# fr34za/multilinear

Hardware: AMD Instinct MI355X
Metric: NTT 2^24 field-elems/sec + FRI commit ms; % HBM roofline at 1/2/4/8 GPUs (higher is better)
Workload: dtype u128 mod M (F_M, M = 2^128 - 45*2^40 + 1)

## Files before the change

include/mlhip.h:

```cpp
#ifndef MLHIP_H
#define MLHIP_H

#include <stddef.h>
#include <stdint.h>

#ifdef __cplusplus
extern "C" {
#endif

typedef enum mlh_status {
  MLH_OK = 0,
  MLH_ERR_INVALID = 1,
  MLH_ERR_NOT_POW2 = 2,
  MLH_ERR_BAD_GENERATOR = 3,
  MLH_ERR_HIP = 4,
  MLH_ERR_OOM = 5,
  MLH_ERR_NOT_RS_CODE = 6,
  MLH_ERR_VERIFY = 7,
  MLH_ERR_VERIFY_INDEX = 8,
  MLH_ERR_COMM = 9,
  MLH_ERR_DEVICE = 10
} mlh_status;

typedef struct mlh_ctx mlh_ctx;
typedef struct mlh_transcript mlh_transcript;
typedef struct mlh_fri_prover mlh_fri_prover;

#define MLH_LOG_BLOWUP 1
#define MLH_NUM_QUERIES 128

const char* mlh_version(void);
mlh_status mlh_context_create(int device, void* hip_stream, mlh_ctx** out);
void mlh_context_destroy(mlh_ctx* ctx);
mlh_status mlh_set_table_cache_limit(mlh_ctx* ctx, uint64_t bytes);
uint64_t mlh_table_cache_bytes(const mlh_ctx* ctx);
mlh_status mlh_set_ntt_plan(mlh_ctx* ctx, const uint32_t* logr, uint32_t count);
mlh_status mlh_set_coop_spin_limit(mlh_ctx* ctx, uint32_t sleeps);
mlh_status mlh_set_pcs_fused_max(mlh_ctx* ctx, uint32_t max_vars);
mlh_status mlh_set_stream(mlh_ctx* ctx, void* hip_stream);
mlh_status mlh_synchronize(mlh_ctx* ctx);
const char* mlh_last_error(const mlh_ctx* ctx);
mlh_status mlh_malloc(mlh_ctx* ctx, size_t bytes, void** dev);
mlh_status mlh_free(mlh_ctx* ctx, void* dev);
mlh_status mlh_memcpy_h2d(mlh_ctx* ctx, void* dev, const void* host, size_t bytes);
mlh_status mlh_memcpy_d2h(mlh_ctx* ctx, void* host, const void* dev, size_t bytes);
mlh_status mlh_memcpy_d2d(mlh_ctx* ctx, void* dst, const void* src, size_t bytes);

mlh_status mlh_pow_2_generator(uint32_t log_size, uint8_t gen_out[16]);
mlh_status mlh_pow_2_generator_powers(mlh_ctx* ctx, uint32_t log_size, void* dev_out);

mlh_status mlh_field_add(mlh_ctx* ctx, const void* dev_a, const void* dev_b, void* dev_out, uint64_t n);
mlh_status mlh_field_sub(mlh_ctx* ctx, const void* dev_a, const void* dev_b, void* dev_out, uint64_t n);
mlh_status mlh_field_mul(mlh_ctx* ctx, const void* dev_a, const void* dev_b, void* dev_out, uint64_t n);
mlh_status mlh_field_neg(mlh_ctx* ctx, const void* dev_a, void* dev_out, uint64_t n);
mlh_status mlh_field_scale(mlh_ctx* ctx, const void* dev_a, const uint8_t c[16], void* dev_out,
                           uint64_t n);
mlh_status mlh_field_inv(mlh_ctx* ctx, const void* dev_a, void* dev_out, uint64_t n);

mlh_status mlh_ntt(mlh_ctx* ctx, const void* dev_coeffs, void* dev_evals, uint32_t log_n,
                   const uint8_t gen[16]);
mlh_status mlh_intt(mlh_ctx* ctx, const void* dev_evals, void* dev_coeffs, uint32_t log_n,
                    const uint8_t gen[16]);
mlh_status mlh_bit_reverse_permutation(mlh_ctx* ctx, const void* dev_in, void* dev_out,
                                       uint32_t log_n);
mlh_status mlh_ntt_host(mlh_ctx* ctx, const uint8_t* host_in, uint8_t* host_out, uint32_t log_n,
                        const uint8_t gen[16], int inverse);

mlh_status mlh_reed_solomon(mlh_ctx* ctx, const void* dev_coeffs, uint32_t log_n,
                            const uint8_t gen[16], void* dev_code);
mlh_status mlh_reed_solomon_brev(mlh_ctx* ctx, const void* dev_coeffs, uint32_t log_n,
                                 const uint8_t gen[16], void* dev_code);
uint64_t mlh_merkle_layers_bytes(uint64_t leaves);
mlh_status mlh_merkle_commit_pairs(mlh_ctx* ctx, const void* dev_code, uint32_t log_code,
                                   void* dev_layers, uint8_t root_out[32]);
mlh_status mlh_merkle_commit(mlh_ctx* ctx, const void* dev_items, uint64_t item_len,
                             uint64_t count, void* dev_layers, uint8_t root_out[32]);
mlh_status mlh_merkle_batch_commit(mlh_ctx* ctx, const void* dev_items, uint64_t item_len,
                                   uint32_t m, uint64_t count, void* dev_layers,
                                   uint8_t root_out[32]);
mlh_status mlh_fri_fold(mlh_ctx* ctx, const void* dev_layer, uint32_t log_layer, uint32_t k,
                        uint32_t log_domain, const uint8_t r[16], void* dev_next);

mlh_status mlh_gen_pows_params(const uint8_t* gen_pows, uint64_t len, uint8_t gen_out[16],
                               uint32_t* log_len_out);
mlh_status mlh_gen_pows_verify(mlh_ctx* ctx, const uint8_t* gen_pows, uint64_t len,
                               uint8_t gen_out[16], uint32_t* log_len_out);
mlh_status mlh_fri_prover_init(mlh_ctx* ctx, const void* dev_code, uint32_t log_code,
                               mlh_transcript* tr, mlh_fri_prover** out);
mlh_status mlh_fri_prover_init_gp(mlh_ctx* ctx, const void* dev_code, uint32_t log_code,
                                  const uint8_t gen_pows_1[16], uint32_t log_gen_pows,
                                  mlh_transcript* tr, mlh_fri_prover** out);
mlh_status mlh_fri_prover_fold_step(mlh_ctx* ctx, mlh_fri_prover* p, uint32_t k,
                                    const uint8_t r[16], mlh_transcript* tr);
mlh_status mlh_fri_prover_fold_step_gp(mlh_ctx* ctx, mlh_fri_prover* p, const uint8_t gen_pows_1[16],
                                       uint32_t log_gen_pows, uint32_t k, const uint8_t r[16],
                                       mlh_transcript* tr);
mlh_status mlh_fri_prover_fold(mlh_ctx* ctx, const void* dev_code, uint32_t log_code,
                               mlh_transcript* tr, mlh_fri_prover** out);
mlh_status mlh_fri_prover_fold_gp(mlh_ctx* ctx, const void* dev_code, uint32_t log_code,
                                  const uint8_t gen_pows_1[16], uint32_t log_gen_pows,
                                  mlh_transcript* tr, mlh_fri_prover** out);
uint32_t mlh_fri_prover_num_trees(const mlh_fri_prover* p);
mlh_status mlh_fri_prover_roots(const mlh_fri_prover* p, uint8_t* roots_out );
mlh_status mlh_fri_prover_last_element(const mlh_fri_prover* p, uint8_t out[16]);
mlh_status mlh_fri_prover_open_query(mlh_ctx* ctx, const mlh_fri_prover* p, uint64_t index,
                                     uint8_t* out);
void mlh_fri_prover_destroy(mlh_fri_prover* p);

typedef struct mlh_fri_proof {
  uint32_t log_code;
  uint32_t num_trees;
  uint32_t num_queries;
  uint8_t* commitments;
  uint8_t last_elem[16];
  uint8_t last_random[32];
  uint64_t* query_indices;
  uint8_t* queries;
} mlh_fri_proof;
uint64_t mlh_fri_query_bytes(uint32_t log_code);
mlh_status mlh_fri_prove(mlh_ctx* ctx, const void* dev_code, uint32_t log_code, mlh_transcript* tr,
                         mlh_fri_proof* proof);
mlh_status mlh_fri_prove_gp(mlh_ctx* ctx, const void* dev_code, uint32_t log_code,
                            const uint8_t gen_pows_1[16], uint32_t log_gen_pows, mlh_transcript* tr,
                            mlh_fri_proof* proof);
uint64_t mlh_fri_proof_encoded_size(const mlh_fri_proof* proof);
mlh_status mlh_fri_proof_encode(const mlh_fri_proof* proof, uint8_t* out, uint64_t cap);
mlh_status mlh_fri_proof_decode_header(const uint8_t* in, uint64_t len, uint32_t* log_code,
                                       uint32_t* num_queries);
mlh_status mlh_fri_proof_decode(const uint8_t* in, uint64_t len, mlh_fri_proof* proof);
mlh_status mlh_fri_verify(const mlh_fri_proof* proof);

mlh_status mlh_fri_prover_open_queries(mlh_ctx* ctx, const mlh_fri_prover* p,
                                       const uint64_t* idx, uint32_t nq, uint8_t* out);

mlh_status mlh_shard_ntt_cross(mlh_ctx* ctx, const void* dev_in, void* dev_out, uint32_t log_n,
                               uint32_t log_p, uint32_t rank, const uint8_t gen[16], int inverse);
mlh_status mlh_shard_fri_fold(mlh_ctx* ctx, const void* dev_layer, uint32_t log_local, uint32_t k,
                              uint32_t log_domain, const uint8_t r[16], void* dev_next,
                              uint32_t log_s, uint32_t log_p, uint32_t rank);
mlh_status mlh_shard_fri_fold_commit(mlh_ctx* ctx, const void* dev_layer, uint32_t log_local,
                                     uint32_t k, uint32_t log_domain, const uint8_t r[16],
                                     void* dev_next, void* dev_tree, uint32_t log_s,
                                     uint32_t log_p, uint32_t rank);
mlh_status mlh_merkle_open(mlh_ctx* ctx, const void* dev_layers, uint64_t leaves,
                           const uint64_t* host_idx, uint32_t nq, uint8_t* out);
mlh_status mlh_merkle_verify(const uint8_t* value, uint64_t value_len, const uint8_t* sibs,
                             uint32_t depth, uint64_t dirs, const uint8_t root[32], uint64_t index);
mlh_status mlh_merkle_open_pairs(mlh_ctx* ctx, const void* dev_values, uint32_t log_n,
                                 const void* dev_tree, uint32_t levels, const uint64_t* idx,
                                 uint32_t nq, uint8_t* out);

uint64_t mlh_device_transcript_bytes(void);
mlh_status mlh_transcript_to_device(mlh_ctx* ctx, const mlh_transcript* tr, void* dev_state);
mlh_status mlh_transcript_from_device(mlh_ctx* ctx, const void* dev_state, mlh_transcript* tr);
mlh_status mlh_device_transcript_absorb(mlh_ctx* ctx, void* dev_state, const void* dev_src,
                                        uint32_t n, void* dev_challenge);
mlh_status mlh_device_fri_last(mlh_ctx* ctx, const void* dev_vals2, void* dev_state,
                               void* dev_flag, void* dev_last);
mlh_status mlh_shard_fri_fold_dr(mlh_ctx* ctx, const void* dev_layer, uint32_t log_local,
                                 uint32_t k, uint32_t log_domain, const void* dev_r,
                                 void* dev_next, uint32_t log_s, uint32_t log_p, uint32_t rank);
mlh_status mlh_shard_fri_fold_commit_dr(mlh_ctx* ctx, const void* dev_layer, uint32_t log_local,
                                        uint32_t k, uint32_t log_domain, const void* dev_r,
                                        void* dev_next, void* dev_tree, uint32_t log_s,
                                        uint32_t log_p, uint32_t rank);
mlh_status mlh_merkle_top(mlh_ctx* ctx, const void* dev_gathered, uint32_t P, uint64_t per_rank,
                          void* dev_levels);

mlh_status mlh_sumcheck_sums_dev(mlh_ctx* ctx, const void* dev_matrix, const void* dev_delta,
                                 uint32_t log_height, void* dev_sums);
mlh_status mlh_sumcheck_fold_sums_dr(mlh_ctx* ctx, void* dev_matrix, void* dev_delta,
                                     uint32_t log_height, const void* dev_r, void* dev_sums);
mlh_status mlh_sumcheck_fold_dr(mlh_ctx* ctx, void* dev_matrix, void* dev_delta,
                                uint32_t log_height, const void* dev_r);
mlh_status mlh_device_sumcheck_round(mlh_ctx* ctx, const void* dev_sum_pairs, uint32_t npairs,
                                     void* dev_prev, void* dev_state, void* dev_poly_out,
                                     void* dev_r_out);

typedef struct mlh_batched_fri_proof {
  uint32_t log_code;
  uint32_t num_codes;
  uint32_t num_trees;
  uint32_t num_queries;
  uint8_t batch_commitment[32];
  uint8_t* commitments;
  uint8_t last_elem[16];
  uint8_t last_random[32];
  uint64_t* query_indices;
  uint8_t* queries;
} mlh_batched_fri_proof;
uint64_t mlh_batched_fri_query_bytes(uint32_t log_code, uint32_t num_codes);
mlh_status mlh_batched_fri_prove(mlh_ctx* ctx, const void* dev_codes, uint32_t num_codes,
                                 uint32_t log_code, mlh_transcript* tr,
                                 mlh_batched_fri_proof* proof);
mlh_status mlh_batched_fri_verify(const mlh_batched_fri_proof* proof);
typedef struct mlh_batched_fri_prover mlh_batched_fri_prover;
mlh_status mlh_batched_fri_prover_init(mlh_ctx* ctx, const void* dev_codes, uint32_t num_codes,
                                       uint32_t log_code, mlh_transcript* tr,
                                       mlh_batched_fri_prover** out);
mlh_status mlh_batched_fri_prover_fold_step_gp(mlh_ctx* ctx, mlh_batched_fri_prover* bp,
                                               const uint8_t gen_pows_1[16], uint32_t log_gen_pows,
                                               const uint8_t r[16], mlh_transcript* tr);
mlh_fri_prover* mlh_batched_fri_prover_inner(mlh_batched_fri_prover* bp);
mlh_status mlh_batched_fri_prover_batch_root(const mlh_batched_fri_prover* bp, uint8_t out[32]);
mlh_status mlh_batched_fri_prover_fingerprint_r(const mlh_batched_fri_prover* bp, uint8_t out[16]);
mlh_status mlh_batched_fri_prover_open_query(mlh_ctx* ctx, const mlh_batched_fri_prover* bp,
                                             uint64_t index, uint8_t* out);
void mlh_batched_fri_prover_destroy(mlh_batched_fri_prover* bp);
typedef struct mlh_batched_pcs_proof {
  mlh_batched_fri_proof fri;
  uint8_t* sumcheck_polys;
} mlh_batched_pcs_proof;
mlh_status mlh_batched_pcs_prove(mlh_ctx* ctx, const void* dev_evals, uint32_t num_polys,
                                 uint32_t n_vars, const uint8_t* inputs, const uint8_t* outputs,
                                 mlh_transcript* tr, mlh_batched_pcs_proof* proof);
mlh_status mlh_batched_pcs_verify(const mlh_batched_pcs_proof* proof, uint32_t n_vars,
                                  const uint8_t* inputs, const uint8_t* outputs,
                                  mlh_transcript* tr);

mlh_status mlh_transcript_create(mlh_transcript** out);
mlh_status mlh_transcript_clone(const mlh_transcript* t, mlh_transcript** out);
void mlh_transcript_destroy(mlh_transcript* t);
mlh_status mlh_transcript_absorb(mlh_transcript* t, const uint8_t* bytes, uint64_t len);
mlh_status mlh_transcript_random(const mlh_transcript* t, uint8_t out[32]);
mlh_status mlh_transcript_next_challenge(mlh_transcript* t, uint8_t out[16]);

mlh_status mlh_mle_to_coefficient(mlh_ctx* ctx, void* dev_evals, uint32_t log_n);
mlh_status mlh_mle_to_evaluation(mlh_ctx* ctx, void* dev_coeffs, uint32_t log_n);
mlh_status mlh_eq_table(mlh_ctx* ctx, const uint8_t* host_points, uint32_t n, void* dev_out);
mlh_status mlh_mle_evaluate(mlh_ctx* ctx, const void* dev_evals, uint32_t n,
                            const uint8_t* host_args, uint8_t out[16]);
mlh_status mlh_mle_coeffs_evaluate(mlh_ctx* ctx, const void* dev_coeffs, uint32_t n,
                                   const uint8_t* host_args, uint8_t out[16]);
mlh_status mlh_poly_evaluate(mlh_ctx* ctx, const void* dev_coeffs, uint64_t n, const uint8_t x[16],
                             uint8_t out[16]);
mlh_status mlh_trace_evaluate(mlh_ctx* ctx, const void* dev_matrix, uint32_t log_height,
                              uint32_t width, const uint8_t* host_points, uint8_t* out);
mlh_status mlh_sumcheck_partial_sums(mlh_ctx* ctx, const void* dev_matrix, const void* dev_delta,
                                     uint32_t log_height, uint8_t out[32]);
mlh_status mlh_sumcheck_fold(mlh_ctx* ctx, void* dev_matrix, void* dev_delta, uint32_t log_height,
                             const uint8_t r[16]);
mlh_status mlh_sumcheck_fold_and_sums(mlh_ctx* ctx, void* dev_matrix, void* dev_delta,
                                      uint32_t log_height, const uint8_t r[16], uint8_t out[32]);
mlh_status mlh_sumcheck_prove(mlh_ctx* ctx, void* dev_matrix, void* dev_delta, uint32_t log_height,
                              const uint8_t sum[16], mlh_transcript* tr, uint8_t* polys_out,
                              uint8_t* rs_out);
mlh_status mlh_sumcheck_prove_eq(mlh_ctx* ctx, const void* dev_evals, void* dev_work,
                                 uint32_t log_height, const uint8_t* host_points,
                                 const uint8_t sum[16], mlh_transcript* tr, uint8_t* polys_out,
                                 uint8_t* rs_out, uint8_t* delta_out);

typedef struct mlh_cs_program mlh_cs_program;
#define MLH_CS_MAX_LOG_HEIGHT 32
mlh_status mlh_cs_program_create(const uint8_t* bytes, uint64_t len, mlh_cs_program** out);
void mlh_cs_program_destroy(mlh_cs_program* prog);
uint32_t mlh_cs_program_width(const mlh_cs_program* prog);
uint32_t mlh_cs_program_degree(const mlh_cs_program* prog);
uint32_t mlh_cs_program_n_constraints(const mlh_cs_program* prog);
uint32_t mlh_cs_program_n_randoms(const mlh_cs_program* prog);
mlh_status mlh_cs_program_evaluate(const mlh_cs_program* prog, const uint8_t* host_values,
                                   const uint8_t* host_randoms, const uint8_t* host_mask,
                                   uint8_t out[16]);
mlh_status mlh_cs_launch_info(const mlh_cs_program* prog, uint32_t log_height, uint32_t* threads,
                              uint32_t* blocks);
mlh_status mlh_system_challenges(mlh_transcript* tr, uint32_t log_rows, uint32_t n_randoms,
                                 uint32_t n_constraints, uint8_t* row_out, uint8_t* trace_out,
                                 uint8_t* constraint_out, uint8_t* mask_out);
mlh_status mlh_cs_partial_sums(mlh_ctx* ctx, const mlh_cs_program* prog, uint32_t width,
                               const void* dev_matrix, const void* dev_delta, uint32_t log_height,
                               const uint8_t* host_randoms, const uint8_t* host_mask,
                               uint8_t* out);
mlh_status mlh_cs_fold(mlh_ctx* ctx, uint32_t width, void* dev_matrix, void* dev_delta,
                       uint32_t log_height, const uint8_t r[16]);
mlh_status mlh_cs_fold_and_sums(mlh_ctx* ctx, const mlh_cs_program* prog, uint32_t width,
                                void* dev_matrix, void* dev_delta, uint32_t log_height,
                                const uint8_t* host_randoms, const uint8_t* host_mask,
                                const uint8_t r[16], uint8_t* out);
mlh_status mlh_cs_sumcheck_prove(mlh_ctx* ctx, const mlh_cs_program* prog, uint32_t width,
                                 void* dev_matrix, void* dev_delta, uint32_t log_height,
                                 const uint8_t* host_randoms, const uint8_t* host_mask,
                                 const uint8_t sum[16], mlh_transcript* tr, uint8_t* polys_out,
                                 uint8_t* rs_out);
mlh_status mlh_cs_sumcheck_verify(const mlh_cs_program* prog, uint32_t log_height,
                                  const uint8_t* host_row_points, const uint8_t* host_randoms,
                                  const uint8_t* host_mask, const uint8_t sum[16],
                                  const uint8_t* polys, const uint8_t* host_output,
                                  mlh_transcript* tr);

mlh_status mlh_cs_sumcheck_prove_sums(mlh_ctx* ctx, const mlh_cs_program* prog, uint32_t width,
                                      void* dev_matrix, void* dev_delta, uint32_t log_height,
                                      const uint8_t* host_randoms, const uint8_t* host_mask,
                                      uint32_t sum_column_mask, const uint8_t* beta,
                                      const uint8_t claim[16], mlh_transcript* tr,
                                      uint8_t* polys_out, uint8_t* rs_out);
mlh_status mlh_cs_sumcheck_verify_sums(const mlh_cs_program* prog, uint32_t log_height,
                                       const uint8_t* host_row_points, const uint8_t* host_randoms,
                                       const uint8_t* host_mask, uint32_t sum_column_mask,
                                       const uint8_t* beta, const uint8_t claim[16],
                                       const uint8_t* polys, const uint8_t* host_output,
                                       mlh_transcript* tr);

mlh_status mlh_trace_columns(mlh_ctx* ctx, const void* dev_matrix, uint32_t log_height,
                             uint32_t width, void* dev_out);
mlh_status mlh_trace_columns_launch_info(uint32_t log_height, uint32_t width, uint32_t* tile_rows,
                                         uint32_t* blocks);
typedef struct mlh_trace_commitment mlh_trace_commitment;
mlh_status mlh_trace_commit(mlh_ctx* ctx, const void* dev_matrix, uint32_t log_height,
                            uint32_t width, mlh_trace_commitment** out);
mlh_status mlh_trace_columns_range(mlh_ctx* ctx, const void* dev_matrix, uint32_t log_height,
                                   uint32_t width, uint32_t col0, uint32_t ncols, void* dev_out);
mlh_status mlh_trace_columns_range_launch_info(uint32_t log_height, uint32_t width, uint32_t col0,
                                               uint32_t ncols, uint32_t* tile_rows,
                                               uint32_t* blocks);
mlh_status mlh_trace_commit_range(mlh_ctx* ctx, const void* dev_matrix, uint32_t log_height,
                                  uint32_t width, uint32_t col0, uint32_t ncols,
                                  mlh_trace_commitment** out);
mlh_status mlh_trace_commitment_root(const mlh_trace_commitment* c, uint8_t out[32]);
uint32_t mlh_trace_commitment_width(const mlh_trace_commitment* c);
uint32_t mlh_trace_commitment_log_height(const mlh_trace_commitment* c);
void mlh_trace_commitment_destroy(mlh_trace_commitment* c);
typedef struct mlh_system_proof {
  uint32_t log_height, width, degree;
  uint8_t* sumcheck_polys;
  uint8_t* output;
  mlh_batched_pcs_proof pcs;
} mlh_system_proof;
mlh_status mlh_system_prove(mlh_ctx* ctx, const mlh_cs_program* prog,
                            const mlh_trace_commitment* commitment, void* dev_matrix,
                            const uint8_t sum[16], mlh_transcript* tr, mlh_system_proof* proof);
mlh_status mlh_system_verify(const mlh_cs_program* prog, uint32_t log_height, const uint8_t sum[16],
                             const mlh_system_proof* proof, mlh_transcript* tr);

mlh_status mlh_system_trace_randoms(const mlh_transcript* tr, const uint8_t root1[32],
                                    uint32_t n_randoms, uint8_t* out);
typedef struct mlh_phased_proof {
  uint32_t log_height, width, degree;
  uint32_t pre_random_columns;
  uint32_t sum_column_mask;
  uint8_t* sumcheck_polys;
  uint8_t* output;
  mlh_batched_pcs_proof pcs[2];
} mlh_phased_proof;
mlh_status mlh_system_prove_phased(mlh_ctx* ctx, const mlh_cs_program* prog,
                                   const mlh_trace_commitment* commitment1,
                                   const mlh_trace_commitment* commitment2,
                                   uint32_t sum_column_mask, void* dev_matrix,
                                   const uint8_t sum[16], const uint8_t column_sum[16],
                                   mlh_transcript* tr, mlh_phased_proof* proof);
mlh_status mlh_system_verify_phased(const mlh_cs_program* prog, uint32_t log_height,
                                    uint32_t pre_random_columns, uint32_t sum_column_mask,
                                    const uint8_t sum[16], const uint8_t column_sum[16],
                                    const mlh_phased_proof* proof, mlh_transcript* tr);

typedef struct mlh_fill_program mlh_fill_program;
mlh_status mlh_fill_program_create(const uint8_t* bytes, uint64_t len, mlh_fill_program** out);
void mlh_fill_program_destroy(mlh_fill_program* prog);
uint32_t mlh_fill_program_width(const mlh_fill_program* prog);
uint32_t mlh_fill_program_n_randoms(const mlh_fill_program* prog);
uint32_t mlh_fill_program_n_outputs(const mlh_fill_program* prog);
uint32_t mlh_fill_program_n_inverses(const mlh_fill_program* prog);
uint32_t mlh_fill_program_output_mask(const mlh_fill_program* prog);
mlh_status mlh_fill_program_evaluate(const mlh_fill_program* prog, const uint8_t* host_row,
                                     const uint8_t* host_randoms, uint8_t* out_row);
mlh_status mlh_trace_fill(mlh_ctx* ctx, const mlh_fill_program* prog, void* dev_matrix,
                          uint32_t log_height, uint32_t width, const uint8_t* host_randoms);
mlh_status mlh_trace_fill_launch_info(const mlh_fill_program* prog, uint32_t log_height,
                                      uint32_t* threads, uint32_t* rows_per_thread,
                                      uint32_t* blocks);
mlh_status mlh_trace_fill_shaped(mlh_ctx* ctx, const mlh_fill_program* prog, void* dev_matrix,
                                 uint32_t log_height, uint32_t width, const uint8_t* host_randoms,
                                 uint32_t threads, uint32_t rows_per_thread);
mlh_status mlh_trace_column_sum(mlh_ctx* ctx, const void* dev_matrix, uint32_t log_height,
                                uint32_t width, uint32_t column_mask, uint8_t out[16]);

typedef struct mlh_pcs_proof {
  mlh_fri_proof fri;
  uint8_t* sumcheck_polys;
} mlh_pcs_proof;
mlh_status mlh_pcs_prove(mlh_ctx* ctx, const void* dev_evals, uint32_t n_vars,
                         const uint8_t* host_inputs, const uint8_t output[16], mlh_transcript* tr,
                         mlh_pcs_proof* proof);
mlh_status mlh_pcs_verify(const mlh_pcs_proof* proof, uint32_t n_vars, const uint8_t* host_inputs,
                          const uint8_t output[16], mlh_transcript* tr);

typedef int (*mlh_all_to_all_fn)(void* user, const void* dev_send, void* dev_recv,
                                 uint64_t bytes_per_rank, void* hip_stream);
typedef int (*mlh_all_gather_fn)(void* user, const void* dev_send, void* dev_recv, uint64_t bytes,
                                 void* hip_stream);
typedef struct mlh_transport {
  uint32_t world;
  uint32_t rank;
  uint32_t host_side;
  void* user;
  mlh_all_to_all_fn all_to_all;
  mlh_all_gather_fn all_gather;
} mlh_transport;
typedef struct mlh_comm mlh_comm;
mlh_status mlh_comm_unique_id(uint8_t out[128]);
mlh_status mlh_comm_create(mlh_ctx* ctx, uint32_t world, uint32_t rank, const uint8_t id[128],
                           mlh_comm** out);
void mlh_comm_destroy(mlh_comm* comm);
mlh_status mlh_comm_transport(mlh_comm* comm, mlh_transport* out);
mlh_status mlh_comm_info(mlh_comm* comm, uint32_t* count, uint32_t* rank, int* device);
mlh_status mlh_comm_preflight(mlh_ctx* ctx, const mlh_transport* tp, uint64_t bytes_per_rank,
                              uint64_t* mismatches, float* ms);
mlh_status mlh_sharded_ntt(mlh_ctx* ctx, const mlh_transport* tp, const void* dev_in, void* dev_out,
                           uint32_t log_n, const uint8_t gen[16], int inverse);
mlh_status mlh_sharded_ntt_batch(mlh_ctx* ctx, const mlh_transport* tp, const void* const* dev_in,
                                 void* const* dev_out, uint32_t count, uint32_t log_n,
                                 const uint8_t gen[16], int inverse);
mlh_status mlh_sharded_ntt_fused_batch(mlh_ctx* ctx, const mlh_transport* tp, const void* const* dev_in,
                                       void* const* dev_out, uint32_t count, uint32_t log_n,
                                       const uint8_t gen[16], uint32_t* log_s_out);
mlh_status mlh_sharded_reed_solomon(mlh_ctx* ctx, const mlh_transport* tp, const void* dev_coeffs,
                                    uint32_t log_n, const uint8_t gen[16], void* dev_code);
mlh_status mlh_sharded_commit_rs_code(mlh_ctx* ctx, const mlh_transport* tp, const void* dev_code,
                                      uint32_t log_code, uint8_t root_out[32]);
mlh_status mlh_sharded_fri_prove(mlh_ctx* ctx, const mlh_transport* tp, const void* dev_code,
                                 uint32_t log_code, uint32_t gather_log, mlh_transcript* tr,
                                 mlh_fri_proof* proof);
mlh_status mlh_sharded_eq_table(mlh_ctx* ctx, const mlh_transport* tp, const uint8_t* points,
                                uint32_t n, void* dev_out);
mlh_status mlh_sharded_sumcheck_prove(mlh_ctx* ctx, const mlh_transport* tp, void* dev_m, void* dev_d,
                                      uint32_t n, const uint8_t sum[16], mlh_transcript* tr,
                                      uint8_t* polys_out, uint8_t* rs_out);

mlh_status mlh_profile_enable(mlh_ctx* ctx, int on);
mlh_status mlh_profile_reset(mlh_ctx* ctx);
mlh_status mlh_profile_get(mlh_ctx* ctx, const char* label, uint64_t* count, double* total_ms);
mlh_status mlh_bench_ntt(mlh_ctx* ctx, void* dev_buf, uint32_t log_n, uint32_t iters,
                         float* ms_out);

#ifdef __cplusplus
}
#endif
#endif
```

multilinear_amd/_lib.py:

```python
import ctypes
import os

_HERE = os.path.dirname(os.path.abspath(__file__))
LIB_PATH = os.path.join(_HERE, "libmlhip.so")

MLH_OK = 0
STATUS_NAMES = {
    0: "MLH_OK",
    1: "MLH_ERR_INVALID",
    2: "MLH_ERR_NOT_POW2",
    3: "MLH_ERR_BAD_GENERATOR",
    4: "MLH_ERR_HIP",
    5: "MLH_ERR_OOM",
    6: "MLH_ERR_NOT_RS_CODE",
    7: "MLH_ERR_VERIFY",
    8: "MLH_ERR_VERIFY_INDEX",
    9: "MLH_ERR_COMM",
    10: "MLH_ERR_DEVICE",
}
STATUS_CODES = {v: k for k, v in STATUS_NAMES.items()}
globals().update(STATUS_CODES)
LOG_BLOWUP = 1
NUM_QUERIES = 128


class MlhError(RuntimeError):
    def __init__(self, status, msg=""):
        self.status = status
        super().__init__("%s: %s" % (STATUS_NAMES.get(status, status), msg))


class FriProofC(ctypes.Structure):
    _fields_ = [
        ("log_code", ctypes.c_uint32),
        ("num_trees", ctypes.c_uint32),
        ("num_queries", ctypes.c_uint32),
        ("commitments", ctypes.c_void_p),
        ("last_elem", ctypes.c_uint8 * 16),
        ("last_random", ctypes.c_uint8 * 32),
        ("query_indices", ctypes.c_void_p),
        ("queries", ctypes.c_void_p),
    ]


class PcsProofC(ctypes.Structure):
    _fields_ = [("fri", FriProofC), ("sumcheck_polys", ctypes.c_void_p)]


class BatchedFriProofC(ctypes.Structure):
    _fields_ = [
        ("log_code", ctypes.c_uint32),
        ("num_codes", ctypes.c_uint32),
        ("num_trees", ctypes.c_uint32),
        ("num_queries", ctypes.c_uint32),
        ("batch_commitment", ctypes.c_uint8 * 32),
        ("commitments", ctypes.c_void_p),
        ("last_elem", ctypes.c_uint8 * 16),
        ("last_random", ctypes.c_uint8 * 32),
        ("query_indices", ctypes.c_void_p),
        ("queries", ctypes.c_void_p),
    ]


class BatchedPcsProofC(ctypes.Structure):
    _fields_ = [("fri", BatchedFriProofC), ("sumcheck_polys", ctypes.c_void_p)]


class SystemProofC(ctypes.Structure):
    _fields_ = [
        ("log_height", ctypes.c_uint32),
        ("width", ctypes.c_uint32),
        ("degree", ctypes.c_uint32),
        ("sumcheck_polys", ctypes.c_void_p),
        ("output", ctypes.c_void_p),
        ("pcs", BatchedPcsProofC),
    ]


class PhasedProofC(ctypes.Structure):
    _fields_ = [
        ("log_height", ctypes.c_uint32),
        ("width", ctypes.c_uint32),
        ("degree", ctypes.c_uint32),
        ("pre_random_columns", ctypes.c_uint32),
        ("sum_column_mask", ctypes.c_uint32),
        ("sumcheck_polys", ctypes.c_void_p),
        ("output", ctypes.c_void_p),
        ("pcs", BatchedPcsProofC * 2),
    ]


ALL_TO_ALL_FN = ctypes.CFUNCTYPE(ctypes.c_int, ctypes.c_void_p, ctypes.c_void_p, ctypes.c_void_p,
                                 ctypes.c_uint64, ctypes.c_void_p)
ALL_GATHER_FN = ctypes.CFUNCTYPE(ctypes.c_int, ctypes.c_void_p, ctypes.c_void_p, ctypes.c_void_p,
                                 ctypes.c_uint64, ctypes.c_void_p)


class TransportC(ctypes.Structure):
    _fields_ = [
        ("world", ctypes.c_uint32),
        ("rank", ctypes.c_uint32),
        ("host_side", ctypes.c_uint32),
        ("user", ctypes.c_void_p),
        ("all_to_all", ALL_TO_ALL_FN),
        ("all_gather", ALL_GATHER_FN),
    ]


_P = ctypes.c_void_p
_U32 = ctypes.c_uint32
_U64 = ctypes.c_uint64
_I = ctypes.c_int
_S = ctypes.c_size_t

SIGNATURES = {
    "mlh_version": (ctypes.c_char_p, []),
    "mlh_context_create": (_I, [_I, _P, ctypes.POINTER(_P)]),
    "mlh_context_destroy": (None, [_P]),
    "mlh_set_stream": (_I, [_P, _P]),
    "mlh_set_ntt_plan": (_I, [_P, ctypes.POINTER(ctypes.c_uint32), _U32]),
    "mlh_set_coop_spin_limit": (_I, [_P, _U32]),
    "mlh_set_pcs_fused_max": (_I, [_P, _U32]),
    "mlh_set_table_cache_limit": (_I, [_P, ctypes.c_uint64]),
    "mlh_table_cache_bytes": (ctypes.c_uint64, [_P]),
    "mlh_synchronize": (_I, [_P]),
    "mlh_last_error": (ctypes.c_char_p, [_P]),
    "mlh_malloc": (_I, [_P, _S, ctypes.POINTER(_P)]),
    "mlh_free": (_I, [_P, _P]),
    "mlh_memcpy_h2d": (_I, [_P, _P, _P, _S]),
    "mlh_memcpy_d2h": (_I, [_P, _P, _P, _S]),
    "mlh_memcpy_d2d": (_I, [_P, _P, _P, _S]),
    "mlh_pow_2_generator": (_I, [_U32, _P]),
    "mlh_pow_2_generator_powers": (_I, [_P, _U32, _P]),
    "mlh_field_add": (_I, [_P, _P, _P, _P, _U64]),
    "mlh_field_sub": (_I, [_P, _P, _P, _P, _U64]),
    "mlh_field_mul": (_I, [_P, _P, _P, _P, _U64]),
    "mlh_field_neg": (_I, [_P, _P, _P, _U64]),
    "mlh_field_scale": (_I, [_P, _P, _P, _P, _U64]),
    "mlh_field_inv": (_I, [_P, _P, _P, _U64]),
    "mlh_ntt": (_I, [_P, _P, _P, _U32, _P]),
    "mlh_intt": (_I, [_P, _P, _P, _U32, _P]),
    "mlh_bit_reverse_permutation": (_I, [_P, _P, _P, _U32]),
    "mlh_ntt_host": (_I, [_P, _P, _P, _U32, _P, _I]),
    "mlh_reed_solomon": (_I, [_P, _P, _U32, _P, _P]),
    "mlh_reed_solomon_brev": (_I, [_P, _P, _U32, _P, _P]),
    "mlh_merkle_layers_bytes": (_U64, [_U64]),
    "mlh_merkle_commit_pairs": (_I, [_P, _P, _U32, _P, _P]),
    "mlh_merkle_commit": (_I, [_P, _P, _U64, _U64, _P, _P]),
    "mlh_merkle_batch_commit": (_I, [_P, _P, _U64, _U32, _U64, _P, _P]),
    "mlh_fri_fold": (_I, [_P, _P, _U32, _U32, _U32, _P, _P]),
    "mlh_fri_prover_init": (_I, [_P, _P, _U32, _P, ctypes.POINTER(_P)]),
    "mlh_fri_prover_fold_step": (_I, [_P, _P, _U32, _P, _P]),
    "mlh_fri_prover_fold_step_gp": (_I, [_P, _P, _P, _U32, _U32, _P, _P]),
    "mlh_fri_prover_fold": (_I, [_P, _P, _U32, _P, ctypes.POINTER(_P)]),
    "mlh_fri_prover_init_gp": (_I, [_P, _P, _U32, _P, _U32, _P, ctypes.POINTER(_P)]),
    "mlh_fri_prover_fold_gp": (_I, [_P, _P, _U32, _P, _U32, _P, ctypes.POINTER(_P)]),
    "mlh_fri_prover_num_trees": (_U32, [_P]),
    "mlh_fri_prover_roots": (_I, [_P, _P]),
    "mlh_fri_prover_last_element": (_I, [_P, _P]),
    "mlh_fri_prover_open_query": (_I, [_P, _P, _U64, _P]),
    "mlh_fri_prover_open_queries": (_I, [_P, _P, _P, _U32, _P]),
    "mlh_fri_prover_destroy": (None, [_P]),
    "mlh_fri_query_bytes": (_U64, [_U32]),
    "mlh_fri_prove": (_I, [_P, _P, _U32, _P, ctypes.POINTER(FriProofC)]),
    "mlh_fri_prove_gp": (_I, [_P, _P, _U32, _P, _U32, _P, ctypes.POINTER(FriProofC)]),
    "mlh_fri_verify": (_I, [ctypes.POINTER(FriProofC)]),
    "mlh_fri_proof_encoded_size": (_U64, [ctypes.POINTER(FriProofC)]),
    "mlh_fri_proof_encode": (_I, [ctypes.POINTER(FriProofC), _P, _U64]),
    "mlh_fri_proof_decode_header": (_I, [_P, _U64, ctypes.POINTER(_U32), ctypes.POINTER(_U32)]),
    "mlh_fri_proof_decode": (_I, [_P, _U64, ctypes.POINTER(FriProofC)]),
    "mlh_shard_ntt_cross": (_I, [_P, _P, _P, _U32, _U32, _U32, _P, _I]),
    "mlh_shard_fri_fold": (_I, [_P, _P, _U32, _U32, _U32, _P, _P, _U32, _U32, _U32]),
    "mlh_shard_fri_fold_commit": (_I, [_P, _P, _U32, _U32, _U32, _P, _P, _P, _U32, _U32, _U32]),
    "mlh_merkle_open_pairs": (_I, [_P, _P, _U32, _P, _U32, _P, _U32, _P]),
    "mlh_merkle_open": (_I, [_P, _P, _U64, _P, _U32, _P]),
    "mlh_merkle_verify": (_I, [_P, _U64, _P, _U32, _U64, _P, _U64]),
    "mlh_batched_fri_query_bytes": (_U64, [_U32, _U32]),
    "mlh_batched_fri_prove": (_I, [_P, _P, _U32, _U32, _P, ctypes.POINTER(BatchedFriProofC)]),
    "mlh_batched_fri_prover_init": (_I, [_P, _P, _U32, _U32, _P, ctypes.POINTER(_P)]),
    "mlh_batched_fri_prover_fold_step_gp": (_I, [_P, _P, _P, _U32, _P, _P]),
    "mlh_batched_fri_prover_inner": (_P, [_P]),
    "mlh_batched_fri_prover_batch_root": (_I, [_P, _P]),
    "mlh_batched_fri_prover_fingerprint_r": (_I, [_P, _P]),
    "mlh_batched_fri_prover_open_query": (_I, [_P, _P, ctypes.c_uint64, _P]),
    "mlh_batched_fri_prover_destroy": (None, [_P]),
    "mlh_batched_fri_verify": (_I, [ctypes.POINTER(BatchedFriProofC)]),
    "mlh_batched_pcs_prove": (_I, [_P, _P, _U32, _U32, _P, _P, _P,
                                   ctypes.POINTER(BatchedPcsProofC)]),
    "mlh_batched_pcs_verify": (_I, [ctypes.POINTER(BatchedPcsProofC), _U32, _P, _P, _P]),
    "mlh_device_transcript_bytes": (_U64, []),
    "mlh_transcript_to_device": (_I, [_P, _P, _P]),
    "mlh_transcript_from_device": (_I, [_P, _P, _P]),
    "mlh_device_transcript_absorb": (_I, [_P, _P, _P, _U32, _P]),
    "mlh_device_fri_last": (_I, [_P, _P, _P, _P, _P]),
    "mlh_shard_fri_fold_dr": (_I, [_P, _P, _U32, _U32, _U32, _P, _P, _U32, _U32, _U32]),
    "mlh_shard_fri_fold_commit_dr": (_I, [_P, _P, _U32, _U32, _U32, _P, _P, _P, _U32, _U32, _U32]),
    "mlh_merkle_top": (_I, [_P, _P, _U32, _U64, _P]),
    "mlh_sumcheck_sums_dev": (_I, [_P, _P, _P, _U32, _P]),
    "mlh_sumcheck_fold_sums_dr": (_I, [_P, _P, _P, _U32, _P, _P]),
    "mlh_sumcheck_fold_dr": (_I, [_P, _P, _P, _U32, _P]),
    "mlh_device_sumcheck_round": (_I, [_P, _P, _U32, _P, _P, _P, _P]),
    "mlh_transcript_create": (_I, [ctypes.POINTER(_P)]),
    "mlh_transcript_clone": (_I, [_P, ctypes.POINTER(_P)]),
    "mlh_transcript_destroy": (None, [_P]),
    "mlh_transcript_absorb": (_I, [_P, _P, _U64]),
    "mlh_transcript_random": (_I, [_P, _P]),
    "mlh_transcript_next_challenge": (_I, [_P, _P]),
    "mlh_mle_to_coefficient": (_I, [_P, _P, _U32]),
    "mlh_mle_to_evaluation": (_I, [_P, _P, _U32]),
    "mlh_eq_table": (_I, [_P, _P, _U32, _P]),
    "mlh_mle_coeffs_evaluate": (_I, [_P, _P, _U32, _P, _P]),
    "mlh_poly_evaluate": (_I, [_P, _P, _U64, _P, _P]),
    "mlh_trace_evaluate": (_I, [_P, _P, _U32, _U32, _P, _P]),
    "mlh_mle_evaluate": (_I, [_P, _P, _U32, _P, _P]),
    "mlh_sumcheck_partial_sums": (_I, [_P, _P, _P, _U32, _P]),
    "mlh_sumcheck_fold": (_I, [_P, _P, _P, _U32, _P]),
    "mlh_sumcheck_fold_and_sums": (_I, [_P, _P, _P, _U32, _P, _P]),
    "mlh_sumcheck_prove": (_I, [_P, _P, _P, _U32, _P, _P, _P, _P]),
    "mlh_sumcheck_prove_eq": (_I, [_P, _P, _P, _U32, _P, _P, _P, _P, _P, _P]),
    "mlh_cs_program_create": (_I, [_P, _U64, ctypes.POINTER(_P)]),
    "mlh_cs_program_destroy": (None, [_P]),
    "mlh_cs_program_width": (_U32, [_P]),
    "mlh_cs_program_degree": (_U32, [_P]),
    "mlh_cs_program_n_constraints": (_U32, [_P]),
    "mlh_cs_program_n_randoms": (_U32, [_P]),
    "mlh_cs_program_evaluate": (_I, [_P, _P, _P, _P, _P]),
    "mlh_cs_launch_info": (_I, [_P, _U32, ctypes.POINTER(_U32), ctypes.POINTER(_U32)]),
    "mlh_system_challenges": (_I, [_P, _U32, _U32, _U32, _P, _P, _P, _P]),
    "mlh_cs_partial_sums": (_I, [_P, _P, _U32, _P, _P, _U32, _P, _P, _P]),
    "mlh_cs_fold": (_I, [_P, _U32, _P, _P, _U32, _P]),
    "mlh_cs_fold_and_sums": (_I, [_P, _P, _U32, _P, _P, _U32, _P, _P, _P, _P]),
    "mlh_cs_sumcheck_prove": (_I, [_P, _P, _U32, _P, _P, _U32, _P, _P, _P, _P, _P, _P]),
    "mlh_cs_sumcheck_verify": (_I, [_P, _U32, _P, _P, _P, _P, _P, _P, _P]),
    "mlh_cs_sumcheck_prove_sums": (_I, [_P, _P, _U32, _P, _P, _U32, _P, _P, _U32, _P, _P, _P, _P, _P]),
    "mlh_cs_sumcheck_verify_sums": (_I, [_P, _U32, _P, _P, _P, _U32, _P, _P, _P, _P, _P]),
    "mlh_trace_columns": (_I, [_P, _P, _U32, _U32, _P]),
    "mlh_trace_columns_range": (_I, [_P, _P, _U32, _U32, _U32, _U32, _P]),
    "mlh_trace_columns_range_launch_info": (_I, [_U32, _U32, _U32, _U32, ctypes.POINTER(_U32),
                                                 ctypes.POINTER(_U32)]),
    "mlh_trace_commit_range": (_I, [_P, _P, _U32, _U32, _U32, _U32, ctypes.POINTER(_P)]),
    "mlh_system_trace_randoms": (_I, [_P, _P, _U32, _P]),
    "mlh_system_prove_phased": (_I, [_P, _P, _P, _P, _U32, _P, _P, _P, _P,
                                     ctypes.POINTER(PhasedProofC)]),
    "mlh_system_verify_phased": (_I, [_P, _U32, _U32, _U32, _P, _P, ctypes.POINTER(PhasedProofC), _P]),
    "mlh_fill_program_create": (_I, [_P, _U64, ctypes.POINTER(_P)]),
    "mlh_fill_program_destroy": (None, [_P]),
    "mlh_fill_program_width": (_U32, [_P]),
    "mlh_fill_program_n_randoms": (_U32, [_P]),
    "mlh_fill_program_n_outputs": (_U32, [_P]),
    "mlh_fill_program_n_inverses": (_U32, [_P]),
    "mlh_fill_program_output_mask": (_U32, [_P]),
    "mlh_fill_program_evaluate": (_I, [_P, _P, _P, _P]),
    "mlh_trace_fill": (_I, [_P, _P, _P, _U32, _U32, _P]),
    "mlh_trace_fill_launch_info": (_I, [_P, _U32, ctypes.POINTER(_U32), ctypes.POINTER(_U32),
                                        ctypes.POINTER(_U32)]),
    "mlh_trace_fill_shaped": (_I, [_P, _P, _P, _U32, _U32, _P, _U32, _U32]),
    "mlh_trace_column_sum": (_I, [_P, _P, _U32, _U32, _U32, _P]),
    "mlh_trace_columns_launch_info": (_I, [_U32, _U32, ctypes.POINTER(_U32), ctypes.POINTER(_U32)]),
    "mlh_trace_commit": (_I, [_P, _P, _U32, _U32, ctypes.POINTER(_P)]),
    "mlh_trace_commitment_root": (_I, [_P, _P]),
    "mlh_trace_commitment_width": (_U32, [_P]),
    "mlh_trace_commitment_log_height": (_U32, [_P]),
    "mlh_trace_commitment_destroy": (None, [_P]),
    "mlh_system_prove": (_I, [_P, _P, _P, _P, _P, _P, ctypes.POINTER(SystemProofC)]),
    "mlh_system_verify": (_I, [_P, _U32, _P, ctypes.POINTER(SystemProofC), _P]),
    "mlh_pcs_prove": (_I, [_P, _P, _U32, _P, _P, _P, ctypes.POINTER(PcsProofC)]),
    "mlh_pcs_verify": (_I, [ctypes.POINTER(PcsProofC), _U32, _P, _P, _P]),
    "mlh_bench_ntt": (_I, [_P, _P, _U32, _U32, ctypes.POINTER(ctypes.c_float)]),
    "mlh_profile_enable": (_I, [_P, _I]),
    "mlh_profile_reset": (_I, [_P]),
    "mlh_profile_get": (_I, [_P, ctypes.c_char_p, ctypes.POINTER(_U64), ctypes.POINTER(ctypes.c_double)]),
    "mlh_comm_unique_id": (_I, [_P]),
    "mlh_comm_create": (_I, [_P, _U32, _U32, _P, ctypes.POINTER(_P)]),
    "mlh_comm_destroy": (None, [_P]),
    "mlh_comm_transport": (_I, [_P, ctypes.POINTER(TransportC)]),
    "mlh_comm_info": (_I, [_P, ctypes.POINTER(_U32), ctypes.POINTER(_U32), ctypes.POINTER(ctypes.c_int)]),
    "mlh_comm_preflight": (_I, [_P, ctypes.POINTER(TransportC), ctypes.c_uint64,
                                ctypes.POINTER(ctypes.c_uint64), ctypes.POINTER(ctypes.c_float)]),
    "mlh_sharded_ntt": (_I, [_P, ctypes.POINTER(TransportC), _P, _P, _U32, _P, _I]),
    "mlh_gen_pows_params": (_I, [_P, _U64, _P, ctypes.POINTER(_U32)]),
    "mlh_gen_pows_verify": (_I, [_P, _P, _U64, _P, ctypes.POINTER(_U32)]),
    "mlh_sharded_ntt_batch": (_I, [_P, ctypes.POINTER(TransportC), ctypes.POINTER(_P),
                                   ctypes.POINTER(_P), _U32, _U32, _P, _I]),
    "mlh_sharded_ntt_fused_batch": (_I, [_P, ctypes.POINTER(TransportC), ctypes.POINTER(_P),
                                         ctypes.POINTER(_P), _U32, _U32, _P, ctypes.POINTER(_U32)]),
    "mlh_sharded_reed_solomon": (_I, [_P, ctypes.POINTER(TransportC), _P, _U32, _P, _P]),
    "mlh_sharded_commit_rs_code": (_I, [_P, ctypes.POINTER(TransportC), _P, _U32, _P]),
    "mlh_sharded_fri_prove": (_I, [_P, ctypes.POINTER(TransportC), _P, _U32, _U32, _P,
                                   ctypes.POINTER(FriProofC)]),
    "mlh_sharded_eq_table": (_I, [_P, ctypes.POINTER(TransportC), _P, _U32, _P]),
    "mlh_sharded_sumcheck_prove": (_I, [_P, ctypes.POINTER(TransportC), _P, _P, _U32, _P, _P, _P, _P]),
}

_lib = None


def load():
    global _lib
    if _lib is not None:
        return _lib
    if not os.path.exists(LIB_PATH):
        raise ImportError(
            "libmlhip.so not built at %s -- run `python -c 'import __graft_entry__ as g; g.build()'`"
            % LIB_PATH
        )
    import torch

    lib = ctypes.CDLL(LIB_PATH)
    for name, (res, args) in SIGNATURES.items():
        fn = getattr(lib, name)
        fn.restype = res
        fn.argtypes = args
    _lib = lib
    return lib
```

multilinear_amd/csrc/capi.hip:

```cpp
#include <hip/hip_runtime.h>
#include <stdint.h>
#include <stdio.h>
#include <string.h>

#include <algorithm>
#include <map>
#include <memory>
#include <string>
#include <tuple>
#include <vector>

#include "../../include/mlhip.h"
#include "field.hpp"
#include "dist.hpp"
#include "fieldops.hpp"
#include "host_field.hpp"
#include "host_sha256.hpp"
#include "host_transcript.hpp"
#include "context.hpp"
#include "cs_program.hpp"
#include "cs_sumcheck.hpp"
#include "fri_prover.hpp"
#include "fused_ntt.hpp"
#include "merkle.hpp"
#include "ntt.hpp"
#include "pcs_prover.hpp"
#include "sha256.hpp"
#include "sumcheck.hpp"
#include "system_head.hpp"
#include "tables.hpp"
#include "trace_commit.hpp"
#include "trace_fill.hpp"
#include "transcript_dev.hpp"

using namespace mlh;


constexpr uint64_t kTablePin = 24;

static bool ranges_overlap(const void* a, const void* b, uint64_t bytes) {
  const uintptr_t x = (uintptr_t)a, y = (uintptr_t)b;
  return x < y ? y - x < bytes : x - y < bytes;
}

static mlh_status table_make_room(mlh_ctx* ctx, size_t need) {
  if (ctx->table_bytes + need <= ctx->table_limit) return MLH_OK;
  std::vector<std::pair<uint64_t, TableKey>> order;
  for (auto& kv : ctx->tables)
    if (kv.second.stamp + kTablePin <= ctx->table_stamp) order.push_back({kv.second.stamp, kv.first});
  std::sort(order.begin(), order.end(),
            [](const std::pair<uint64_t, TableKey>& a, const std::pair<uint64_t, TableKey>& b) {
              return a.first < b.first;
            });
  bool synced = false;
  for (auto& o : order) {
    if (ctx->table_bytes + need <= ctx->table_limit) break;
    if (!synced) {
      HIP_TRY(ctx, hipStreamSynchronize(ctx->stream));
      synced = true;
    }
    auto it = ctx->tables.find(o.second);
    HIP_TRY(ctx, hipFree(it->second.d));
    ctx->table_bytes -= it->second.bytes;
    ctx->tables.erase(it);
  }
  return MLH_OK;
}

static bool table_hit(mlh_ctx* ctx, const TableKey& k, const fe** out) {
  auto it = ctx->tables.find(k);
  if (it == ctx->tables.end()) return false;
  it->second.stamp = ++ctx->table_stamp;
  *out = it->second.d;
  return true;
}

static mlh_status table_alloc(mlh_ctx* ctx, const TableKey& k, size_t bytes, fe** d) {
  MLH_TRY(table_make_room(ctx, bytes));
  HIP_TRY(ctx, hipMalloc(d, bytes));
  ctx->tables[k] = CachedTable{*d, bytes, ++ctx->table_stamp};
  ctx->table_bytes += bytes;
  return MLH_OK;
}

mlh_status mlh::get_table(mlh_ctx* ctx, u128 base, uint64_t count, u128 scale, const fe** out,
                          bool expand) {
  TableKey k{base, count, scale, expand ? 1 : 0};
  if (table_hit(ctx, k, out)) return MLH_OK;
  fe* d = nullptr;
  MLH_TRY(table_alloc(ctx, k, count * sizeof(fe) * (expand ? 4 : 1), &d));
  HIP_TRY(ctx, launch_pow_table(d, to_fe(base), to_fe(scale), count, ctx->stream, expand));
  *out = d;
  return MLH_OK;
}

static mlh_status get_table2d(mlh_ctx* ctx, u128 base, uint64_t rows, uint64_t cols,
                              uint64_t mult, u128 scale, const fe** out, bool expand = false) {
  TableKey k{base, rows, scale, expand ? 1 : 0, cols, mult};
  if (table_hit(ctx, k, out)) return MLH_OK;
  fe* d = nullptr;
  MLH_TRY(table_alloc(ctx, k, rows * cols * sizeof(fe) * (expand ? 4 : 1), &d));
  HIP_TRY(ctx, launch_pow_table2d(d, to_fe(base), to_fe(scale), rows, cols, mult, ctx->stream,
                                  expand));
  *out = d;
  return MLH_OK;
}

uint64_t mlh::hi_count(uint32_t log_n) {
  const uint64_t N = 1ull << log_n;
  return N <= 4096 ? 1 : N / 4096;
}

#ifndef MLH_P0_GEO
#define MLH_P0_GEO 1
#endif
#ifndef MLH_P0_GEO_MAXLOGW
#define MLH_P0_GEO_MAXLOGW 16
#endif
static mlh_status get_ntt_tables(mlh_ctx* ctx, u128 gen, uint32_t log_n, bool inverse,
                                 NttTables* tb, const uint32_t* plan = nullptr, uint32_t nplan = 0) {
  const uint64_t N = 1ull << log_n;
  const u128 w = inverse ? h_inv(gen) : gen;
  const u128 scale = inverse ? h_inv((u128)N) : (u128)1;
  tb->log_n = log_n;
  tb->inverse = inverse;
  tb->scale = to_fe(scale);
  if (log_n <= 10) {
    MLH_TRY(get_table(ctx, w, N / 2 ? N / 2 : 1, 1, &tb->tw_small));
    return MLH_OK;
  }
  tb->debug_sync = ctx->debug_sync;
  if (plan)
    ntt_plan_radices(log_n, &tb->nradix, tb->logr, plan, nplan);
  else
    ntt_plan_radices(log_n, &tb->nradix, tb->logr, ctx->forced_plan, ctx->forced_plan_len);
  for (uint32_t p = 0; p < tb->nradix; ++p) {
    const uint64_t R = 1ull << tb->logr[p];
    MLH_TRY(get_table(ctx, h_pow(w, N / R), R / 2, 1, &tb->tw[p], true));
  }
  uint64_t S = 1;
  for (uint32_t p = 0; p + 1 < tb->nradix; ++p) {
    const uint64_t R = 1ull << tb->logr[p];
    const uint32_t logw = log_n - (uint32_t)__builtin_ctzll(S) - tb->logr[p];
    const uint32_t loga =
        tb->logr[p] + logw <= kFullTwLog ? logw : (logw < kTwLogA ? logw : kTwLogA);
    const u128 ws = h_pow(w, S);
    tb->loga[p] = loga;
    MLH_TRY(get_table2d(ctx, ws, R, 1ull << loga, 1, p == 0 ? scale : (u128)1, &tb->ta[p]));
    tb->tb[p] = nullptr;
    if (logw > loga)
      MLH_TRY(get_table2d(ctx, ws, R, 1ull << (logw - loga), 1ull << loga, 1, &tb->tb[p], true));
    if (MLH_P0_GEO && p == 0 && logw > loga && (tb->logr[0] == 7 || tb->logr[0] == 8) &&
        logw <= MLH_P0_GEO_MAXLOGW) {
      MLH_TRY(get_table2d(ctx, ws, 64, 1ull << logw, 1, scale, &tb->gp[0]));
      MLH_TRY(get_table(ctx, h_pow(ws, 64), 1ull << logw, 1, &tb->gc[0], true));
    }
    S <<= tb->logr[p];
  }
  return MLH_OK;
}

bool mlh::check_generator(u128 gen, uint32_t log_n) {
  if (gen >= kModulus) return false;
  if (log_n == 0) return gen == 1;
  const u128 half = h_pow(gen, (u128)1 << (log_n - 1));
  return half == kModulus - 1;
}

mlh_status mlh::read_root(mlh_ctx* ctx, const uint8_t* layers, uint64_t leaves, uint8_t out[32]) {
  if (!out) return MLH_OK;
  HIP_TRY(ctx, hipMemcpyAsync(ctx->pinned, layers + (2 * leaves - 2) * 32, 32,
                              hipMemcpyDeviceToHost, ctx->stream));
  HIP_TRY(ctx, hipStreamSynchronize(ctx->stream));
  memcpy(out, ctx->pinned, 32);
  return MLH_OK;
}

mlh_status mlh::fold_tables_g(mlh_ctx* ctx, u128 g, uint32_t log_len, const fe** tlo,
                              const fe** thi) {
  const u128 ginv = h_inv(g);
  MLH_TRY(get_table(ctx, ginv, 4096, 1, tlo));
  MLH_TRY(get_table(ctx, h_pow(ginv, 4096), hi_count(log_len), 1, thi));
  return MLH_OK;
}
mlh_status mlh::fold_tables(mlh_ctx* ctx, uint32_t log_domain, const fe** tlo, const fe** thi) {
  return fold_tables_g(ctx, h_pow2_generator(log_domain), log_domain, tlo, thi);
}

#ifndef MLH_FOLD_TABLE_MAX_LOG
#define MLH_FOLD_TABLE_MAX_LOG 25
#endif
mlh_status mlh::fold_layer_table(mlh_ctx* ctx, u128 g, uint32_t L, const fe** out) {
  *out = nullptr;
  if (L < 2 || L > MLH_FOLD_TABLE_MAX_LOG) return MLH_OK;
  const TableKey key{h_inv(g), (1ull << L) - 1, 0, 2};
  if (table_hit(ctx, key, out)) return MLH_OK;
  fe* d = nullptr;
  MLH_TRY(table_alloc(ctx, key, ((1ull << L) - 1) * sizeof(fe), &d));
  const fe *tlo, *thi;
  MLH_TRY(fold_tables_g(ctx, g, L, &tlo, &thi));
  HIP_TRY(ctx, launch_fold_layer_table(d, tlo, thi, L, ctx->stream));
  *out = d;
  return MLH_OK;
}

static mlh_status ensure_ntt_scratch(mlh_ctx* ctx, uint32_t log_n) {
  const size_t need = (size_t)16 << log_n;
  if (ctx->ntt_scratch_bytes < need) {
    if (ctx->ntt_scratch) {
      HIP_TRY(ctx, hipStreamSynchronize(ctx->stream));
      HIP_TRY(ctx, hipFree(ctx->ntt_scratch));
      ctx->ntt_scratch = nullptr;
      ctx->ntt_scratch_bytes = 0;
    }
    HIP_TRY(ctx, hipMalloc(&ctx->ntt_scratch, need));
    ctx->ntt_scratch_bytes = need;
  }
  return MLH_OK;
}

static mlh_status ntt_network_core(mlh_ctx* ctx, const fe* in, fe* out, uint32_t log_n, u128 gen,
                                   bool inverse, int zero_top) {
  const u128 w = inverse ? h_inv(gen) : gen;
  const fe *tlo, *thi;
  MLH_TRY(get_table(ctx, w, 4096, 1, &tlo));
  MLH_TRY(get_table(ctx, h_pow(w, 4096), hi_count(log_n - 1), 1, &thi));
  fe* scratch = nullptr;
  if (in == out && log_n > 11) {
    MLH_TRY(ensure_ntt_scratch(ctx, log_n));
    scratch = ctx->ntt_scratch;
  }
  const u128 scale = inverse ? h_inv((u128)1 << log_n) : (u128)1;
  HIP_TRY(ctx, launch_ntt_network(in, out, scratch, tlo, thi, log_n, zero_top, to_fe(scale), inverse,
                                  ctx->stream));
  return MLH_OK;
}

FusedNtt::~FusedNtt() {
  for (void* q : scaled) pool_free(ctx, q);
}

mlh_status FusedNtt::prepare(mlh_ctx* c, u128 gen, uint32_t log_n, uint32_t log_p, uint32_t rank_) {
  ctx = c;
  L = log_n;
  p = log_p;
  rank = rank_;
  const uint32_t Lloc = L - p;
  const uint32_t cl = 9 - p;
  if (p < 1 || p > 4 || cl < 4 || Lloc < cl + 4 || Lloc > 40) return fail(ctx, MLH_ERR_INVALID, "fused plan");
  uint32_t npre = 0, pre[kMaxPasses];
  ntt_plan_radices(Lloc - cl, &npre, pre);
  if (npre + 1 > (uint32_t)kMaxPasses || pre[0] < p + 3) return fail(ctx, MLH_ERR_INVALID, "fused plan");
  uint32_t plan[kMaxPasses];
  for (uint32_t i = 0; i < npre; ++i) plan[i] = pre[i];
  plan[npre] = cl;
  for (uint32_t i = 0; i <= npre; ++i)
    if (plan[i] < 4 || plan[i] > 9) return fail(ctx, MLH_ERR_INVALID, "fused plan");
  const u128 gl = h_pow(gen, (u128)1 << p);
  MLH_TRY(get_ntt_tables(ctx, gl, Lloc, false, &loc, plan, npre + 1));
  if (loc.nradix != npre + 1) return fail(ctx, MLH_ERR_INVALID, "fused plan");
  nglob = npre + 1;
  for (uint32_t i = 0; i < npre; ++i) logr[i] = plan[i];
  logr[npre] = cl + p;
  uint64_t S = 1;
  for (uint32_t i = 0; i < npre; ++i) {
    const uint64_t R = 1ull << plan[i];
    void* q;
    MLH_TRY(pool_alloc(ctx, (R << loc.loga[i]) * sizeof(fe), &q));
    scaled.push_back(q);
    const u128 rb = h_pow(gen, (u128)S * rank);
    HIP_TRY(ctx, launch_scale_rows(loc.ta[i], reinterpret_cast<fe*>(q), R, loc.loga[i], to_fe(rb), ctx->stream));
    loc.ta[i] = reinterpret_cast<const fe*>(q);
    S <<= plan[i];
  }
  const uint64_t Rl = 1ull << logr[npre];
  MLH_TRY(get_table(ctx, h_pow(gen, (u128)(1ull << (L - logr[npre]))), Rl / 2, 1, &tw_last, true));
  return MLH_OK;
}

mlh_status FusedNtt::run_pre(const void* in, void* out) {
  ProfScope ps(ctx, "ntt_fused_pre");
  HIP_TRY(ctx, launch_ntt_passes_pre(reinterpret_cast<const fe*>(in), reinterpret_cast<fe*>(out), loc, L - p,
                                     nglob - 1, ctx->stream));
  ps.end();
  return MLH_OK;
}

mlh_status FusedNtt::run_last(const void* recv, void* out) {
  ProfScope ps(ctx, "ntt_fused_last");
  HIP_TRY(ctx, launch_ntt_shard_last(reinterpret_cast<const fe*>(recv), reinterpret_cast<fe*>(out), tw_last,
                                     logr, nglob, L, p, rank, ctx->stream));
  ps.end();
  return MLH_OK;
}

static mlh_status ntt_core(mlh_ctx* ctx, const fe* in, fe* out, uint32_t log_n, u128 gen,
                           bool inverse, int zero_top) {
  NttTables tb;
  MLH_TRY(get_ntt_tables(ctx, gen, log_n, inverse, &tb));
  if (log_n <= 10) {
    const uint64_t N = 1ull << log_n;
    HIP_TRY(ctx, launch_ntt_small(in, out, tb.tw_small, log_n, zero_top ? N / 2 : N, tb.scale,
                                  inverse, ctx->stream, 1, zero_top == 2));
    return MLH_OK;
  }
  MLH_TRY(ensure_ntt_scratch(ctx, log_n));
  char lab0[64];
  if (ctx->prof_on) ntt_pass_label(tb, 0, zero_top, lab0, sizeof lab0);
  if (ctx->prof_on && prof_sample(ctx, lab0)) {
    std::vector<hipEvent_t> ev(tb.nradix + 1);
    for (auto& e : ev) e = take_event(ctx);
    HIP_TRY(ctx, launch_ntt_passes(in, out, ctx->ntt_scratch, tb, log_n, zero_top, ctx->stream,
                                   ev.data()));
    for (uint32_t p = 0; p < tb.nradix; ++p) {
      char lab[64];
      ntt_pass_label(tb, p, zero_top, lab, sizeof lab);
      ctx->pending.push_back(mlh_ctx::Pending{lab, ev[p], ev[p + 1]});
    }
    return MLH_OK;
  }
  HIP_TRY(ctx, launch_ntt_passes(in, out, ctx->ntt_scratch, tb, log_n, zero_top, ctx->stream));
  return MLH_OK;
}

extern "C" {

const char* mlh_version(void) { return "mlhip 0.1 (gfx950)"; }

static thread_local char g_create_err[160] = "null context";

mlh_status mlh_context_create(int device, void* hip_stream, mlh_ctx** out) {
  if (!out) return MLH_ERR_INVALID;
  *out = nullptr;
  int n = 0;
  hipError_t e = hipGetDeviceCount(&n);
  if (e != hipSuccess || n <= device || device < 0) {
    snprintf(g_create_err, sizeof g_create_err, "mlh_context_create: hipGetDeviceCount -> %s, %d devices, device %d",
             hipGetErrorString(e), n, device);
    return MLH_ERR_HIP;
  }
  e = hipSetDevice(device);
  if (e != hipSuccess) {
    snprintf(g_create_err, sizeof g_create_err, "mlh_context_create: hipSetDevice(%d) -> %s", device,
             hipGetErrorString(e));
    return MLH_ERR_HIP;
  }
  std::unique_ptr<mlh_ctx> c(new mlh_ctx());
  c->device = device;
  c->stream = reinterpret_cast<hipStream_t>(hip_stream);
  const char* dbg = getenv("MLH_DEBUG_SYNC");
  c->debug_sync = dbg && *dbg && strcmp(dbg, "0") != 0;
  void* st = nullptr;
  const bool ok = hipMalloc(&c->partials, 2 * kMaxRedBlocks * sizeof(fe)) == hipSuccess &&
                  hipMalloc(&c->small, 64 * sizeof(fe)) == hipSuccess &&
                  hipHostMalloc(&c->pinned, kPinnedBytes, 0) == hipSuccess &&
                  hipHostMalloc(&st, 64, hipHostMallocCoherent) == hipSuccess;
  if (!ok) {
    snprintf(g_create_err, sizeof g_create_err, "mlh_context_create: allocation failed (%s)",
             hipGetErrorString(hipGetLastError()));
    (void)hipFree(c->partials);
    (void)hipFree(c->small);
    (void)hipHostFree(c->pinned);
    (void)hipHostFree(st);
    return MLH_ERR_OOM;
  }
  c->dev_status = reinterpret_cast<volatile uint32_t*>(st);
  *c->dev_status = 0;
  *out = c.release();
  return MLH_OK;
}

void mlh_context_destroy(mlh_ctx* ctx) {
  if (!ctx) return;
  (void)hipSetDevice(ctx->device);
  (void)hipStreamSynchronize(ctx->stream);
  if (ctx->side) (void)hipStreamSynchronize(ctx->side);
  if (ctx->side2) (void)hipStreamSynchronize(ctx->side2);
  resolve_profile(ctx);
  for (auto e : ctx->ev_free) (void)hipEventDestroy(e);
  for (auto& kv : ctx->tables) (void)hipFree(kv.second.d);
  for (auto& kv : ctx->pool) (void)hipFree(kv.second);
  for (auto& kv : ctx->live) (void)hipFree(kv.first);
  (void)hipFree(ctx->ntt_scratch);
  if (ctx->side) (void)hipStreamDestroy(ctx->side);
  if (ctx->side2) (void)hipStreamDestroy(ctx->side2);
  (void)hipFree(ctx->partials);
  (void)hipFree(ctx->small);
  (void)hipHostFree(ctx->pinned);
  (void)hipHostFree(const_cast<uint32_t*>(ctx->dev_status));
  if (ctx->qstage) (void)hipHostFree(ctx->qstage);
  delete ctx;
}

mlh_status mlh_set_table_cache_limit(mlh_ctx* ctx, uint64_t bytes) {
  if (!ctx) return MLH_ERR_INVALID;
  ctx->table_limit = (size_t)bytes;
  return table_make_room(ctx, 0);
}

uint64_t mlh_table_cache_bytes(const mlh_ctx* ctx) { return ctx ? ctx->table_bytes : 0; }

mlh_status mlh_set_ntt_plan(mlh_ctx* ctx, const uint32_t* logr, uint32_t count) {
  if (!ctx || (count && !logr) || count > (uint32_t)kMaxPasses)
    return fail(ctx, MLH_ERR_INVALID, "plan: at most kMaxPasses digits");
  for (uint32_t i = 0; i < count; ++i)
    if (logr[i] < 4 || logr[i] > 9) return fail(ctx, MLH_ERR_INVALID, "plan digits must be 4..9");
  ctx->forced_plan_len = count;
  for (uint32_t i = 0; i < count; ++i) ctx->forced_plan[i] = logr[i];
  return MLH_OK;
}

mlh_status mlh_set_coop_spin_limit(mlh_ctx* ctx, uint32_t sleeps) {
  if (!ctx) return MLH_ERR_INVALID;
  ctx->coop_spin = sleeps;
  return MLH_OK;
}

mlh_status mlh_set_pcs_fused_max(mlh_ctx* ctx, uint32_t max_vars) {
  if (!ctx) return MLH_ERR_INVALID;
  ctx->pcs_fused_max = max_vars < 24 ? max_vars : 24;
  return MLH_OK;
}

mlh_status mlh_set_stream(mlh_ctx* ctx, void* hip_stream) {
  if (!ctx) return MLH_ERR_INVALID;
  ctx->stream = reinterpret_cast<hipStream_t>(hip_stream);
  return MLH_OK;
}

mlh_status mlh_synchronize(mlh_ctx* ctx) {
  if (!ctx) return MLH_ERR_INVALID;
  HIP_TRY(ctx, hipStreamSynchronize(ctx->stream));
  return MLH_OK;
}

const char* mlh_last_error(const mlh_ctx* ctx) { return ctx ? ctx->err.c_str() : g_create_err; }

mlh_status mlh_malloc(mlh_ctx* ctx, size_t bytes, void** dev) {
  if (!ctx || !dev) return MLH_ERR_INVALID;
  HIP_TRY(ctx, hipMalloc(dev, bytes ? bytes : 16));
  return MLH_OK;
}
mlh_status mlh_free(mlh_ctx* ctx, void* dev) {
  if (!ctx) return MLH_ERR_INVALID;
  HIP_TRY(ctx, hipFree(dev));
  return MLH_OK;
}
mlh_status mlh_memcpy_h2d(mlh_ctx* ctx, void* dev, const void* host, size_t bytes) {
  if (!ctx) return MLH_ERR_INVALID;
  HIP_TRY(ctx, hipMemcpyAsync(dev, host, bytes, hipMemcpyHostToDevice, ctx->stream));
  HIP_TRY(ctx, hipStreamSynchronize(ctx->stream));
  return MLH_OK;
}
mlh_status mlh_memcpy_d2h(mlh_ctx* ctx, void* host, const void* dev, size_t bytes) {
  if (!ctx) return MLH_ERR_INVALID;
  HIP_TRY(ctx, hipMemcpyAsync(host, dev, bytes, hipMemcpyDeviceToHost, ctx->stream));
  HIP_TRY(ctx, hipStreamSynchronize(ctx->stream));
  return MLH_OK;
}
mlh_status mlh_memcpy_d2d(mlh_ctx* ctx, void* dst, const void* src, size_t bytes) {
  if (!ctx) return MLH_ERR_INVALID;
  HIP_TRY(ctx, hipMemcpyAsync(dst, src, bytes, hipMemcpyDeviceToDevice, ctx->stream));
  return MLH_OK;
}

mlh_status mlh_pow_2_generator(uint32_t log_size, uint8_t gen_out[16]) {
  if (!gen_out || log_size > 40) return MLH_ERR_INVALID;
  h_store(gen_out, h_pow2_generator(log_size));
  return MLH_OK;
}

mlh_status mlh_gen_pows_params(const uint8_t* gen_pows, uint64_t len, uint8_t gen_out[16],
                               uint32_t* log_len_out) {
  if (!gen_pows || !gen_out || !log_len_out) return MLH_ERR_INVALID;
  if (len < 2 || (len & (len - 1)) || len > (1ull << 40)) return MLH_ERR_INVALID;
  const uint32_t lg = 63 - __builtin_clzll(len);
  auto at = [&](uint64_t i) { return h_load(gen_pows + 16 * i); };
  const u128 g = at(1);
  if (at(0) != 1 || !check_generator(g, lg)) return MLH_ERR_INVALID;
  u128 p = g;
  for (uint32_t j = 0; j < lg; ++j, p = h_mul(p, p))
    if (at(1ull << j) != p) return MLH_ERR_INVALID;
  if (at(len / 2) != kModulus - 1 || h_mul(at(len - 1), g) != 1) return MLH_ERR_INVALID;
  p = 1;
  for (uint64_t i = 0; i < len && i < 4096; ++i, p = h_mul(p, g))
    if (at(i) != p) return MLH_ERR_INVALID;
  uint64_t x = len ^ 0x9E3779B97F4A7C15ull;
  for (int q = 0; q < 16; ++q) {
    x += 0x9E3779B97F4A7C15ull;
    uint64_t z = x;
    z = (z ^ (z >> 30)) * 0xBF58476D1CE4E5B9ull;
    z = (z ^ (z >> 27)) * 0x94D049BB133111EBull;
    z ^= z >> 31;
    const uint64_t i = z & (len - 1);
    if (at(i) != h_pow(g, (u128)i)) return MLH_ERR_INVALID;
  }
  h_store(gen_out, g);
  *log_len_out = lg;
  return MLH_OK;
}

mlh_status mlh_gen_pows_verify(mlh_ctx* ctx, const uint8_t* gen_pows, uint64_t len,
                               uint8_t gen_out[16], uint32_t* log_len_out) {
  if (!ctx || !gen_pows) return fail(ctx, MLH_ERR_INVALID, "null argument");
  uint8_t gb[16];
  uint32_t lg = 0;
  if (mlh_gen_pows_params(gen_pows, len, gb, &lg) != MLH_OK)
    return fail(ctx, MLH_ERR_INVALID, "gen_pows is not the power series of an element of order len");
  const u128 g = h_load(gb);
  const fe *tlo, *thi;
  MLH_TRY(get_table(ctx, g, 4096, 1, &tlo));
  MLH_TRY(get_table(ctx, h_pow(g, 4096), hi_count(lg), 1, &thi));
  const uint64_t chunk = len < (1ull << 20) ? len : (1ull << 20);
  PoolBuf buf(ctx), badb(ctx);
  MLH_TRY(buf.alloc(chunk * 16));
  MLH_TRY(badb.alloc(8));
  unsigned long long* bad = badb.as<unsigned long long>();
  HIP_TRY(ctx, hipMemsetAsync(bad, 0xFF, 8, ctx->stream));
  for (uint64_t base = 0; base < len; base += chunk) {
    const uint64_t cnt = len - base < chunk ? len - base : chunk;
    HIP_TRY(ctx, hipMemcpyAsync(buf.p, gen_pows + 16 * base, cnt * 16, hipMemcpyHostToDevice,
                                ctx->stream));
    HIP_TRY(ctx, launch_pow_series_check(buf.as<fe>(), base, cnt, tlo, thi, bad, ctx->stream));
  }
  HIP_TRY(ctx, hipMemcpyAsync(ctx->pinned + kPinSlotB, bad, 8, hipMemcpyDeviceToHost, ctx->stream));
  HIP_TRY(ctx, hipStreamSynchronize(ctx->stream));
  uint64_t first;
  memcpy(&first, ctx->pinned + kPinSlotB, 8);
  if (first != ~0ull)
    return fail(ctx, MLH_ERR_INVALID,
                "gen_pows[" + std::to_string(first) + "] is not gen_pows[1]^" + std::to_string(first));
  if (gen_out) memcpy(gen_out, gb, 16);
  if (log_len_out) *log_len_out = lg;
  return MLH_OK;
}

mlh_status mlh_pow_2_generator_powers(mlh_ctx* ctx, uint32_t log_size, void* dev_out) {
  if (!ctx || !dev_out || log_size > 40) return fail(ctx, MLH_ERR_INVALID, "bad argument");
  const u128 g = h_pow2_generator(log_size);
  const fe *tlo, *thi;
  MLH_TRY(get_table(ctx, g, 4096, 1, &tlo));
  MLH_TRY(get_table(ctx, h_pow(g, 4096), hi_count(log_size), 1, &thi));
  HIP_TRY(ctx, launch_pow_series(reinterpret_cast<fe*>(dev_out), tlo, thi, 1ull << log_size,
                                 ctx->stream));
  return MLH_OK;
}

static mlh_status ntt_entry(mlh_ctx* ctx, const void* in, void* out, uint32_t log_n,
                            const uint8_t gen[16], bool inverse) {
  if (!ctx || !in || !out || !gen) return fail(ctx, MLH_ERR_INVALID, "null argument");
  if (log_n < 1 || log_n > 32) return fail(ctx, MLH_ERR_NOT_POW2, "The number of coeffs must be a power of 2 (n >= 2)");
  const u128 g = h_load(gen);
  if (g >= kModulus) return fail(ctx, MLH_ERR_BAD_GENERATOR, "generator not canonical");
  if (!check_generator(g, log_n))
    return ntt_network_core(ctx, reinterpret_cast<const fe*>(in), reinterpret_cast<fe*>(out),
                            log_n, g, inverse, 0);
  return ntt_core(ctx, reinterpret_cast<const fe*>(in), reinterpret_cast<fe*>(out), log_n, g,
                  inverse, false);
}

mlh_status mlh_ntt(mlh_ctx* ctx, const void* dev_coeffs, void* dev_evals, uint32_t log_n,
                   const uint8_t gen[16]) {
  return ntt_entry(ctx, dev_coeffs, dev_evals, log_n, gen, false);
}

mlh_status mlh_intt(mlh_ctx* ctx, const void* dev_evals, void* dev_coeffs, uint32_t log_n,
                    const uint8_t gen[16]) {
  return ntt_entry(ctx, dev_evals, dev_coeffs, log_n, gen, true);
}

static mlh_status vec_op(mlh_ctx* ctx, int op, const void* a, const void* b, void* out, uint64_t n) {
  if (!ctx || !a || !out || (op < 3 && !b)) return fail(ctx, MLH_ERR_INVALID, "null argument");
  HIP_TRY(ctx, launch_vec_op(op, reinterpret_cast<const fe*>(a), reinterpret_cast<const fe*>(b),
                             reinterpret_cast<fe*>(out), n, ctx->stream));
  return MLH_OK;
}
mlh_status mlh_field_add(mlh_ctx* ctx, const void* a, const void* b, void* out, uint64_t n) {
  return vec_op(ctx, 0, a, b, out, n);
}
mlh_status mlh_field_sub(mlh_ctx* ctx, const void* a, const void* b, void* out, uint64_t n) {
  return vec_op(ctx, 1, a, b, out, n);
}
mlh_status mlh_field_mul(mlh_ctx* ctx, const void* a, const void* b, void* out, uint64_t n) {
  return vec_op(ctx, 2, a, b, out, n);
}
mlh_status mlh_field_neg(mlh_ctx* ctx, const void* a, void* out, uint64_t n) {
  return vec_op(ctx, 3, a, nullptr, out, n);
}
mlh_status mlh_field_scale(mlh_ctx* ctx, const void* a, const uint8_t c[16], void* out,
                           uint64_t n) {
  if (!ctx || !a || !out || !c) return fail(ctx, MLH_ERR_INVALID, "null argument");
  if (h_load(c) >= kModulus) return fail(ctx, MLH_ERR_INVALID, "scalar not canonical");
  HIP_TRY(ctx, launch_vec_op(4, reinterpret_cast<const fe*>(a), nullptr, reinterpret_cast<fe*>(out),
                             n, ctx->stream, to_fe(h_load(c))));
  return MLH_OK;
}
mlh_status mlh_field_inv(mlh_ctx* ctx, const void* a, void* out, uint64_t n) {
  if (!ctx) return fail(ctx, MLH_ERR_INVALID, "null argument");
  if (n == 0) return MLH_OK;
  if (!a || !out) return fail(ctx, MLH_ERR_INVALID, "null argument");
  if (a != out && ranges_overlap(a, out, n * 16))
    return fail(ctx, MLH_ERR_INVALID, "mlh_field_inv: in place or disjoint buffers only");
  ProfScope ps(ctx, "field_inv");
  HIP_TRY(ctx, launch_field_inv(reinterpret_cast<const fe*>(a), reinterpret_cast<fe*>(out), n,
                                ctx->stream));
  ps.end();
  return MLH_OK;
}

mlh_status mlh_bit_reverse_permutation(mlh_ctx* ctx, const void* dev_in, void* dev_out,
                                       uint32_t log_n) {
  if (!ctx || !dev_in || !dev_out || dev_in == dev_out)
    return fail(ctx, MLH_ERR_INVALID, "bit_reverse_permutation is out of place");
  if (log_n > 40) return fail(ctx, MLH_ERR_INVALID, "log_n too large");
  if (log_n == 0) return fail(ctx, MLH_ERR_NOT_POW2, "bit_reverse_permutation needs n >= 2");
  HIP_TRY(ctx, launch_bitrev(reinterpret_cast<const fe*>(dev_in), reinterpret_cast<fe*>(dev_out),
                             log_n, ctx->stream));
  return MLH_OK;
}

mlh_status mlh_ntt_host(mlh_ctx* ctx, const uint8_t* host_in, uint8_t* host_out, uint32_t log_n,
                        const uint8_t gen[16], int inverse) {
  if (!ctx || !host_in || !host_out) return fail(ctx, MLH_ERR_INVALID, "null argument");
  const size_t bytes = (size_t)16 << log_n;
  PoolBuf buf(ctx);
  MLH_TRY(buf.alloc(bytes));
  HIP_TRY(ctx, hipMemcpyAsync(buf.p, host_in, bytes, hipMemcpyHostToDevice, ctx->stream));
  MLH_TRY(ntt_entry(ctx, buf.p, buf.p, log_n, gen, inverse != 0));
  HIP_TRY(ctx, hipMemcpyAsync(host_out, buf.p, bytes, hipMemcpyDeviceToHost, ctx->stream));
  HIP_TRY(ctx, hipStreamSynchronize(ctx->stream));
  return MLH_OK;
}

mlh_status mlh_reed_solomon(mlh_ctx* ctx, const void* dev_coeffs, uint32_t log_n,
                            const uint8_t gen[16], void* dev_code) {
  if (!ctx || !dev_coeffs || !dev_code || !gen) return fail(ctx, MLH_ERR_INVALID, "null argument");
  if (log_n > 31) return fail(ctx, MLH_ERR_INVALID, "log_n too large");
  if (dev_coeffs == dev_code) return fail(ctx, MLH_ERR_INVALID, "reed_solomon is out of place");
  const uint32_t lc = log_n + MLH_LOG_BLOWUP;
  const u128 g = h_load(gen);
  if (g >= kModulus) return fail(ctx, MLH_ERR_BAD_GENERATOR, "generator not canonical");
  if (!check_generator(g, lc))
    return ntt_network_core(ctx, reinterpret_cast<const fe*>(dev_coeffs),
                            reinterpret_cast<fe*>(dev_code), lc, g, false, 1);
  return ntt_core(ctx, reinterpret_cast<const fe*>(dev_coeffs), reinterpret_cast<fe*>(dev_code),
                  lc, g, false, 1);
}

mlh_status mlh_reed_solomon_brev(mlh_ctx* ctx, const void* dev_coeffs, uint32_t log_n,
                                 const uint8_t gen[16], void* dev_code) {
  if (!ctx || !dev_coeffs || !dev_code || !gen) return fail(ctx, MLH_ERR_INVALID, "null argument");
  if (log_n > 31) return fail(ctx, MLH_ERR_INVALID, "log_n too large");
  if (dev_coeffs == dev_code) return fail(ctx, MLH_ERR_INVALID, "reed_solomon is out of place");
  const uint32_t lc = log_n + MLH_LOG_BLOWUP;
  const u128 g = h_load(gen);
  if (g >= kModulus) return fail(ctx, MLH_ERR_BAD_GENERATOR, "generator not canonical");
  if (!check_generator(g, lc))
    return ntt_network_core(ctx, reinterpret_cast<const fe*>(dev_coeffs),
                            reinterpret_cast<fe*>(dev_code), lc, g, false, 2);
  return ntt_core(ctx, reinterpret_cast<const fe*>(dev_coeffs), reinterpret_cast<fe*>(dev_code),
                  lc, g, false, 2);
}

uint64_t mlh_merkle_layers_bytes(uint64_t leaves) { return leaves ? (2 * leaves - 1) * 32 : 0; }

static bool is_pow2(uint64_t x) { return x && !(x & (x - 1)); }

mlh_status mlh_merkle_commit_pairs(mlh_ctx* ctx, const void* dev_code, uint32_t log_code,
                                   void* dev_layers, uint8_t root_out[32]) {
  if (!ctx || !dev_code || !dev_layers) return fail(ctx, MLH_ERR_INVALID, "null argument");
  if (log_code < 1 || log_code > 40)
    return fail(ctx, MLH_ERR_NOT_POW2, "Data length must be a power of two");
  const uint64_t L = 1ull << (log_code - 1);
  uint8_t* layers = reinterpret_cast<uint8_t*>(dev_layers);
  HIP_TRY(ctx, launch_commit_pairs(reinterpret_cast<const fe*>(dev_code), L, layers, ctx->stream));
  return read_root(ctx, layers, L, root_out);
}

mlh_status mlh_merkle_commit(mlh_ctx* ctx, const void* dev_items, uint64_t item_len,
                             uint64_t count, void* dev_layers, uint8_t root_out[32]) {
  if (!ctx || !dev_items || !dev_layers) return fail(ctx, MLH_ERR_INVALID, "null argument");
  if (!is_pow2(count)) return fail(ctx, MLH_ERR_NOT_POW2, "Data length must be a power of two");
  uint8_t* layers = reinterpret_cast<uint8_t*>(dev_layers);
  HIP_TRY(ctx, launch_leaf_bytes(reinterpret_cast<const uint8_t*>(dev_items), item_len, count,
                                 layers, ctx->stream));
  HIP_TRY(ctx, launch_merkle_levels(layers, count, ctx->stream));
  return read_root(ctx, layers, count, root_out);
}

mlh_status mlh_merkle_batch_commit(mlh_ctx* ctx, const void* dev_items, uint64_t item_len,
                                   uint32_t m, uint64_t count, void* dev_layers,
                                   uint8_t root_out[32]) {
  if (!ctx || !dev_items || !dev_layers) return fail(ctx, MLH_ERR_INVALID, "null argument");
  if (m == 0) return fail(ctx, MLH_ERR_INVALID, "Data must not be empty");
  if (!is_pow2(count))
    return fail(ctx, MLH_ERR_NOT_POW2, "Each batch length must be a power of two");
  uint8_t* layers = reinterpret_cast<uint8_t*>(dev_layers);
  HIP_TRY(ctx, launch_leaf_batch(reinterpret_cast<const uint8_t*>(dev_items), item_len,
                                 item_len * count, m, count, layers, ctx->stream));
  HIP_TRY(ctx, launch_merkle_levels(layers, count, ctx->stream));
  return read_root(ctx, layers, count, root_out);
}

mlh_status mlh_fri_fold(mlh_ctx* ctx, const void* dev_layer, uint32_t log_layer, uint32_t k,
                        uint32_t log_domain, const uint8_t r[16], void* dev_next) {
  if (!ctx || !dev_layer || !dev_next || !r) return fail(ctx, MLH_ERR_INVALID, "null argument");
  if (log_layer < 1 || log_domain > 40 || log_layer + k != log_domain)
    return fail(ctx, MLH_ERR_INVALID, "layer size must be 2^(log_domain - k)");
  const fe *tlo, *thi;
  MLH_TRY(fold_tables(ctx, log_domain, &tlo, &thi));
  HIP_TRY(ctx, launch_fri_fold(reinterpret_cast<const fe*>(dev_layer), 1ull << log_layer,
                               reinterpret_cast<fe*>(dev_next), to_fe(h_load(r)), tlo, thi, k,
                               1ull << log_domain, ctx->stream));
  return MLH_OK;
}

mlh_status mlh_mle_to_coefficient(mlh_ctx* ctx, void* dev_evals, uint32_t log_n) {
  if (!ctx || !dev_evals || log_n > 40) return fail(ctx, MLH_ERR_INVALID, "bad argument");
  HIP_TRY(ctx, launch_mobius(reinterpret_cast<fe*>(dev_evals), log_n, false, ctx->stream));
  return MLH_OK;
}

mlh_status mlh_mle_to_evaluation(mlh_ctx* ctx, void* dev_coeffs, uint32_t log_n) {
  if (!ctx || !dev_coeffs || log_n > 40) return fail(ctx, MLH_ERR_INVALID, "bad argument");
  HIP_TRY(ctx, launch_mobius(reinterpret_cast<fe*>(dev_coeffs), log_n, true, ctx->stream));
  return MLH_OK;
}

static mlh_status eq_table_impl(mlh_ctx* ctx, const uint8_t* host_points, uint32_t n,
                                void* dev_out, bool mono);

mlh_status mlh_eq_table(mlh_ctx* ctx, const uint8_t* host_points, uint32_t n, void* dev_out) {
  return eq_table_impl(ctx, host_points, n, dev_out, false);
}

static mlh_status eq_table_impl(mlh_ctx* ctx, const uint8_t* host_points, uint32_t n,
                                void* dev_out, bool mono) {
  if (!ctx || !dev_out || (n && !host_points) || n > 40)
    return fail(ctx, MLH_ERR_INVALID, "bad argument");
  PoolBuf pts(ctx), scratch(ctx);
  MLH_TRY(pts.alloc((n ? n : 1) * sizeof(fe)));
  const uint32_t a = n / 2, b = n - a;
  MLH_TRY(scratch.alloc(((1ull << a) + (1ull << b)) * sizeof(fe)));
  if (n) HIP_TRY(ctx, hipMemcpyAsync(pts.p, host_points, n * 16ull, hipMemcpyHostToDevice, ctx->stream));
  HIP_TRY(ctx, launch_eq_table(pts.as<fe>(), n, scratch.as<fe>(), reinterpret_cast<fe*>(dev_out),
                               ctx->stream, mono));
  return MLH_OK;
}

static mlh_status read_pair(mlh_ctx* ctx, const fe* dev2, uint8_t out[32]) {
  HIP_TRY(ctx, hipMemcpyAsync(ctx->pinned, dev2, 32, hipMemcpyDeviceToHost, ctx->stream));
  HIP_TRY(ctx, hipStreamSynchronize(ctx->stream));
  memcpy(out, ctx->pinned, 32);
  return MLH_OK;
}

mlh_status mlh_mle_evaluate(mlh_ctx* ctx, const void* dev_evals, uint32_t n,
                            const uint8_t* host_args, uint8_t out[16]) {
  if (!ctx || !dev_evals || !out || n > 40) return fail(ctx, MLH_ERR_INVALID, "bad argument");
  PoolBuf eq(ctx);
  MLH_TRY(eq.alloc((16ull << n)));
  MLH_TRY(mlh_eq_table(ctx, host_args, n, eq.p));
  HIP_TRY(ctx, launch_dot(reinterpret_cast<const fe*>(dev_evals), eq.as<fe>(), 1ull << n,
                          ctx->partials, ctx->small, ctx->stream));
  uint8_t pair[32];
  MLH_TRY(read_pair(ctx, ctx->small, pair));
  memcpy(out, pair, 16);
  return MLH_OK;
}

mlh_status mlh_mle_coeffs_evaluate(mlh_ctx* ctx, const void* dev_coeffs, uint32_t n,
                                   const uint8_t* host_args, uint8_t out[16]) {
  if (!ctx || !dev_coeffs || !out || n > 40) return fail(ctx, MLH_ERR_INVALID, "bad argument");
  PoolBuf mono(ctx);
  MLH_TRY(mono.alloc((16ull << n)));
  MLH_TRY(eq_table_impl(ctx, host_args, n, mono.p, true));
  HIP_TRY(ctx, launch_dot(reinterpret_cast<const fe*>(dev_coeffs), mono.as<fe>(), 1ull << n,
                          ctx->partials, ctx->small, ctx->stream));
  uint8_t pair[32];
  MLH_TRY(read_pair(ctx, ctx->small, pair));
  memcpy(out, pair, 16);
  return MLH_OK;
}

mlh_status mlh_poly_evaluate(mlh_ctx* ctx, const void* dev_coeffs, uint64_t n, const uint8_t x[16],
                             uint8_t out[16]) {
  if (!ctx || (n && !dev_coeffs) || !x || !out || n > (1ull << 40))
    return fail(ctx, MLH_ERR_INVALID, "bad argument");
  if (n == 0) {
    memset(out, 0, 16);
    return MLH_OK;
  }
  const u128 xv = h_load(x);
  if (xv >= kModulus) return fail(ctx, MLH_ERR_INVALID, "x not canonical");
  const uint64_t nlo = n < 4096 ? n : 4096, nhi = (n + 4095) / 4096;
  PoolBuf tlo(ctx), thi(ctx);
  MLH_TRY(tlo.alloc(16 * nlo));
  MLH_TRY(thi.alloc(16 * nhi));
  HIP_TRY(ctx, launch_pow_table(tlo.as<fe>(), to_fe(xv), to_fe(1), nlo, ctx->stream));
  HIP_TRY(ctx, launch_pow_table(thi.as<fe>(), to_fe(h_pow(xv, 4096)), to_fe(1), nhi, ctx->stream));
  HIP_TRY(ctx, launch_poly_eval(reinterpret_cast<const fe*>(dev_coeffs), n, tlo.as<fe>(),
                                thi.as<fe>(), ctx->partials, ctx->small, ctx->stream));
  uint8_t pair[32];
  MLH_TRY(read_pair(ctx, ctx->small, pair));
  memcpy(out, pair, 16);
  return MLH_OK;
}

mlh_status mlh_trace_evaluate(mlh_ctx* ctx, const void* dev_matrix, uint32_t log_height,
                             uint32_t width, const uint8_t* host_points, uint8_t* out) {
  if (!ctx || !dev_matrix || !out || log_height > 40 || width == 0 || width > (1u << 20) ||
      (log_height && !host_points))
    return fail(ctx, MLH_ERR_INVALID, "bad argument");
  const uint64_t height = 1ull << log_height;
  const uint32_t nc = width < 256 ? width : 256;
  PoolBuf eq(ctx), partials(ctx), res(ctx);
  MLH_TRY(eq.alloc(16ull << log_height));
  MLH_TRY(partials.alloc(16ull * trace_eval_blocks(height, nc) * nc));
  MLH_TRY(res.alloc(16ull * width));
  MLH_TRY(mlh_eq_table(ctx, host_points, log_height, eq.p));
  HIP_TRY(ctx, launch_trace_eval(reinterpret_cast<const fe*>(dev_matrix), eq.as<fe>(), height, width,
                                 partials.as<fe>(), res.as<fe>(), ctx->stream));
  HIP_TRY(ctx, hipMemcpyAsync(out, res.p, 16ull * width, hipMemcpyDeviceToHost, ctx->stream));
  HIP_TRY(ctx, hipStreamSynchronize(ctx->stream));
  return MLH_OK;
}

mlh_status mlh_sumcheck_partial_sums(mlh_ctx* ctx, const void* dev_matrix, const void* dev_delta,
                                     uint32_t log_height, uint8_t out[32]) {
  if (!ctx || !dev_matrix || !dev_delta || !out || log_height < 1 || log_height > 40)
    return fail(ctx, MLH_ERR_INVALID, "bad argument");
  HIP_TRY(ctx, launch_sums(reinterpret_cast<const fe*>(dev_matrix),
                           reinterpret_cast<const fe*>(dev_delta), 1ull << (log_height - 1),
                           ctx->partials, ctx->small, ctx->stream));
  return read_pair(ctx, ctx->small, out);
}

mlh_status mlh_sumcheck_fold(mlh_ctx* ctx, void* dev_matrix, void* dev_delta, uint32_t log_height,
                             const uint8_t r[16]) {
  if (!ctx || !dev_matrix || !dev_delta || !r || log_height < 1 || log_height > 40)
    return fail(ctx, MLH_ERR_INVALID, "bad argument");
  HIP_TRY(ctx, launch_fold(reinterpret_cast<fe*>(dev_matrix), reinterpret_cast<fe*>(dev_delta),
                           1ull << log_height, to_fe(h_load(r)), ctx->stream));
  return MLH_OK;
}

mlh_status mlh_sumcheck_fold_and_sums(mlh_ctx* ctx, void* dev_matrix, void* dev_delta,
                                      uint32_t log_height, const uint8_t r[16], uint8_t out[32]) {
  if (!ctx || !dev_matrix || !dev_delta || !r || !out || log_height < 2 || log_height > 40)
    return fail(ctx, MLH_ERR_INVALID, "bad argument");
  HIP_TRY(ctx, launch_fold_sums(reinterpret_cast<fe*>(dev_matrix), reinterpret_cast<fe*>(dev_delta),
                                1ull << log_height, to_fe(h_load(r)), ctx->partials, ctx->small,
                                ctx->stream));
  return read_pair(ctx, ctx->small, out);
}

}

extern "C" {

mlh_status mlh_merkle_open(mlh_ctx* ctx, const void* dev_layers, uint64_t leaves,
                           const uint64_t* host_idx, uint32_t nq, uint8_t* out) {
  if (!ctx || !dev_layers || (nq && (!host_idx || !out)))
    return fail(ctx, MLH_ERR_INVALID, "null argument");
  if (!is_pow2(leaves)) return fail(ctx, MLH_ERR_NOT_POW2, "Data length must be a power of two");
  for (uint32_t q = 0; q < nq; ++q)
    if (host_idx[q] >= leaves) return fail(ctx, MLH_ERR_INVALID, "index out of bounds");
  const uint32_t depth = 63 - __builtin_clzll(leaves);
  if (nq == 0 || depth == 0) return MLH_OK;
  const uint64_t rec = 32ull * depth;
  PoolBuf didx(ctx), dout(ctx);
  MLH_TRY(didx.alloc(nq * sizeof(uint64_t)));
  MLH_TRY(dout.alloc(nq * rec));
  HIP_TRY(ctx, hipMemcpyAsync(didx.p, host_idx, nq * sizeof(uint64_t), hipMemcpyHostToDevice,
                              ctx->stream));
  HIP_TRY(ctx, launch_merkle_paths(reinterpret_cast<const uint8_t*>(dev_layers), leaves,
                                   didx.as<uint64_t>(), nq, dout.as<uint8_t>(), ctx->stream));
  HIP_TRY(ctx, hipMemcpyAsync(out, dout.p, nq * rec, hipMemcpyDeviceToHost, ctx->stream));
  HIP_TRY(ctx, hipStreamSynchronize(ctx->stream));
  return MLH_OK;
}

}

extern "C" {

mlh_status mlh_profile_enable(mlh_ctx* ctx, int on) {
  if (!ctx || on < 0) return MLH_ERR_INVALID;
  ctx->prof_on = on != 0;
  ctx->prof_every = on > 1 ? (uint32_t)on : 1u;
  ctx->prof_ticks.clear();
  return MLH_OK;
}

mlh_status mlh_profile_reset(mlh_ctx* ctx) {
  if (!ctx) return MLH_ERR_INVALID;
  resolve_profile(ctx);
  ctx->prof.clear();
  return MLH_OK;
}

mlh_status mlh_profile_get(mlh_ctx* ctx, const char* label, uint64_t* count, double* total_ms) {
  if (!ctx || !label || !count || !total_ms) return MLH_ERR_INVALID;
  resolve_profile(ctx);
  auto it = ctx->prof.find(label);
  *count = it == ctx->prof.end() ? 0 : it->second.first;
  *total_ms = it == ctx->prof.end() ? 0.0 : it->second.second;
  return MLH_OK;
}

mlh_status mlh_bench_ntt(mlh_ctx* ctx, void* dev_buf, uint32_t log_n, uint32_t iters,
                         float* ms_out) {
  if (!ctx || !dev_buf || !ms_out || iters == 0) return fail(ctx, MLH_ERR_INVALID, "bad argument");
  uint8_t gen[16];
  h_store(gen, h_pow2_generator(log_n));
  MLH_TRY(mlh_ntt(ctx, dev_buf, dev_buf, log_n, gen));
  hipEvent_t a, b;
  HIP_TRY(ctx, hipEventCreate(&a));
  HIP_TRY(ctx, hipEventCreate(&b));
  HIP_TRY(ctx, hipEventRecord(a, ctx->stream));
  for (uint32_t i = 0; i < iters; ++i) MLH_TRY(mlh_ntt(ctx, dev_buf, dev_buf, log_n, gen));
  HIP_TRY(ctx, hipEventRecord(b, ctx->stream));
  HIP_TRY(ctx, hipEventSynchronize(b));
  float ms = 0;
  HIP_TRY(ctx, hipEventElapsedTime(&ms, a, b));
  (void)hipEventDestroy(a);
  (void)hipEventDestroy(b);
  *ms_out = ms / iters;
  return MLH_OK;
}

}

struct mlh_trace_commitment {
  mlh_ctx* ctx;
  uint32_t log_height = 0, width = 0;
  void* evals = nullptr;
  void* codes = nullptr;
  void* tree = nullptr;
  uint8_t root[32];
  ~mlh_trace_commitment() {
    pool_free(ctx, evals);
    pool_free(ctx, codes);
    pool_free(ctx, tree);
  }
};

static bool trace_range_ok(uint32_t log_height, uint32_t width, uint32_t col0, uint32_t ncols) {
  return width >= 1 && width <= kCsMaxWidth && log_height <= kCsMaxLogHeight && ncols >= 1 &&
         col0 < width && ncols <= width - col0;
}

static mlh_status trace_columns_impl(mlh_ctx* ctx, const void* dev_matrix, uint32_t log_height,
                                     uint32_t width, uint32_t col0, uint32_t ncols, void* dev_out) {
  if (!ctx || !dev_matrix || !dev_out) return fail(ctx, MLH_ERR_INVALID, "null argument");
  if (!trace_range_ok(log_height, width, col0, ncols))
    return fail(ctx, MLH_ERR_INVALID,
                "width 1..32, log_height 0..32, a column range inside the trace");
  const uint64_t tb = ((uint64_t)width << log_height) * 16, ob = ((uint64_t)ncols << log_height) * 16;
  const uintptr_t x = (uintptr_t)dev_matrix, y = (uintptr_t)dev_out;
  if (x < y ? y - x < tb : x - y < ob)
    return fail(ctx, MLH_ERR_INVALID, "the trace transpose is out of place: the buffers overlap");
  ProfScope ps(ctx, ncols == width ? "trace_columns" : "trace_columns_range");
  HIP_TRY(ctx, launch_trace_columns(reinterpret_cast<const fe*>(dev_matrix),
                                    reinterpret_cast<fe*>(dev_out), log_height, width, col0, ncols,
                                    ctx->stream));
  ps.end();
  return MLH_OK;
}

static mlh_status trace_launch_info(uint32_t log_height, uint32_t width, uint32_t col0,
                                    uint32_t ncols, uint32_t* tile_rows, uint32_t* blocks) {
  if (!tile_rows || !blocks || !trace_range_ok(log_height, width, col0, ncols))
    return MLH_ERR_INVALID;
  *tile_rows = tc_tile_rows(ncols);
  *blocks = tc_blocks(1ull << log_height, ncols);
  return MLH_OK;
}

static mlh_status trace_commit_impl(mlh_ctx* ctx, const void* dev_matrix, uint32_t log_height,
                                    uint32_t width, uint32_t col0, uint32_t ncols,
                                    mlh_trace_commitment** out) {
  if (!ctx || !dev_matrix || !out) return fail(ctx, MLH_ERR_INVALID, "null argument");
  if (log_height < 1 || !trace_range_ok(log_height, width, col0, ncols))
    return fail(ctx, MLH_ERR_INVALID,
                "width 1..32, log_height 1..32, a column range inside the trace");
  std::unique_ptr<mlh_trace_commitment> c(new mlh_trace_commitment());
  c->ctx = ctx;
  c->log_height = log_height;
  c->width = ncols;
  const uint64_t n = 1ull << log_height;
  MLH_TRY(pool_alloc(ctx, ncols * n * 16, &c->evals));
  MLH_TRY(pool_alloc(ctx, ncols * n * 32, &c->codes));
  MLH_TRY(pool_alloc(ctx, mlh_merkle_layers_bytes(n), &c->tree));
  MLH_TRY(trace_columns_impl(ctx, dev_matrix, log_height, width, col0, ncols, c->evals));
  fe* codes = reinterpret_cast<fe*>(c->codes);
  MLH_TRY(batched_pcs_codes(ctx, c->evals, ncols, log_height, codes));
  uint8_t* bt = reinterpret_cast<uint8_t*>(c->tree);
  MLH_TRY(batch_layer_commit(ctx, codes, ncols, 2 * n, bt));
  MLH_TRY(read_root(ctx, bt, n, c->root));
  *out = c.release();
  return MLH_OK;
}

extern "C" {

mlh_status mlh_trace_columns(mlh_ctx* ctx, const void* dev_matrix, uint32_t log_height,
                             uint32_t width, void* dev_out) {
  return trace_columns_impl(ctx, dev_matrix, log_height, width, 0, width, dev_out);
}

mlh_status mlh_trace_columns_launch_info(uint32_t log_height, uint32_t width, uint32_t* tile_rows,
                                         uint32_t* blocks) {
  return trace_launch_info(log_height, width, 0, width, tile_rows, blocks);
}

mlh_status mlh_trace_columns_range(mlh_ctx* ctx, const void* dev_matrix, uint32_t log_height,
                                   uint32_t width, uint32_t col0, uint32_t ncols, void* dev_out) {
  return trace_columns_impl(ctx, dev_matrix, log_height, width, col0, ncols, dev_out);
}

mlh_status mlh_trace_columns_range_launch_info(uint32_t log_height, uint32_t width, uint32_t col0,
                                               uint32_t ncols, uint32_t* tile_rows,
                                               uint32_t* blocks) {
  return trace_launch_info(log_height, width, col0, ncols, tile_rows, blocks);
}

mlh_status mlh_trace_commit(mlh_ctx* ctx, const void* dev_matrix, uint32_t log_height,
                            uint32_t width, mlh_trace_commitment** out) {
  return trace_commit_impl(ctx, dev_matrix, log_height, width, 0, width, out);
}

mlh_status mlh_trace_commit_range(mlh_ctx* ctx, const void* dev_matrix, uint32_t log_height,
                                  uint32_t width, uint32_t col0, uint32_t ncols,
                                  mlh_trace_commitment** out) {
  return trace_commit_impl(ctx, dev_matrix, log_height, width, col0, ncols, out);
}

mlh_status mlh_trace_commitment_root(const mlh_trace_commitment* c, uint8_t out[32]) {
  if (!c || !out) return MLH_ERR_INVALID;
  memcpy(out, c->root, 32);
  return MLH_OK;
}

uint32_t mlh_trace_commitment_width(const mlh_trace_commitment* c) { return c ? c->width : 0; }

uint32_t mlh_trace_commitment_log_height(const mlh_trace_commitment* c) {
  return c ? c->log_height : 0;
}

void mlh_trace_commitment_destroy(mlh_trace_commitment* c) {
  if (c) {
    (void)hipStreamSynchronize(c->ctx->stream);
    delete c;
  }
}


mlh_status mlh_trace_fill_shaped(mlh_ctx* ctx, const mlh_fill_program* prog, void* dev_matrix,
                                 uint32_t log_height, uint32_t width, const uint8_t* host_randoms,
                                 uint32_t threads, uint32_t rows_per_thread) {
  if (!ctx || !prog || !dev_matrix || width != prog->p.width || log_height > kCsMaxLogHeight ||
      (prog->p.n_randoms && !host_randoms) || !fill_shape_ok(prog->p, threads, rows_per_thread))
    return fail(ctx, MLH_ERR_INVALID, "mlh_trace_fill: bad argument");
  const FillProgram& p = prog->p;
  std::vector<u128> rnd(p.n_randoms);
  for (uint32_t i = 0; i < p.n_randoms; ++i)
    if ((rnd[i] = h_load(host_randoms + 16ull * i)) >= kModulus)
      return fail(ctx, MLH_ERR_INVALID, "non-canonical random");
  const FillImageLayout l = fill_image_layout(p);
  const std::vector<uint8_t> img = fill_build_image(p, rnd.data());
  PoolBuf buf(ctx);
  MLH_TRY(buf.alloc(img.size()));
  HIP_TRY(ctx, hipMemcpyAsync(buf.p, img.data(), img.size(), hipMemcpyHostToDevice, ctx->stream));
  const uint8_t* b = buf.as<uint8_t>();
  FillDev dev{};
  dev.uni = reinterpret_cast<const fe*>(b);
  dev.code = reinterpret_cast<const uint32_t*>(b + l.code_off);
  dev.outs = reinterpret_cast<const uint32_t*>(b + l.outs_off);
  dev.width = p.width;
  dev.n_temps = p.n_temps;
  dev.n_instr = p.n_instr;
  dev.n_pre = p.n_pre;
  dev.n_inv = p.n_inv;
  dev.n_outputs = p.n_outputs;
  dev.K = rows_per_thread;
  const uint64_t height = 1ull << log_height;
  const uint32_t blocks = fill_blocks(p, fill_chunks(height, threads, dev.K), threads, dev.K);
  PoolBuf prefix(ctx);
  if (const uint64_t elems = blocks * fill_prefix_elems(p, threads, dev.K)) {
    MLH_TRY(prefix.alloc(16 * elems));
    dev.prefix = prefix.as<fe>();
  }
  ProfScope ps(ctx, "trace_fill");
  HIP_TRY(ctx, launch_trace_fill(dev, threads, blocks, reinterpret_cast<fe*>(dev_matrix), height,
                                 ctx->stream));
  ps.end();
  return MLH_OK;
}

mlh_status mlh_trace_fill(mlh_ctx* ctx, const mlh_fill_program* prog, void* dev_matrix,
                          uint32_t log_height, uint32_t width, const uint8_t* host_randoms) {
  uint32_t B = 0, K = 0;
  if (prog && log_height <= kCsMaxLogHeight) fill_shape(prog->p, 1ull << log_height, &B, &K);
  return mlh_trace_fill_shaped(ctx, prog, dev_matrix, log_height, width, host_randoms, B, K);
}

mlh_status mlh_trace_column_sum(mlh_ctx* ctx, const void* dev_matrix, uint32_t log_height,
                                uint32_t width, uint32_t column_mask, uint8_t out[16]) {
  if (!ctx || !dev_matrix || !out || width < 1 || width > kCsMaxWidth ||
      log_height > kCsMaxLogHeight || (width < 32 && (column_mask >> width)))
    return fail(ctx, MLH_ERR_INVALID, "mlh_trace_column_sum: bad argument");
  ProfScope ps(ctx, "trace_column_sum");
  HIP_TRY(ctx, launch_trace_column_sum(reinterpret_cast<const fe*>(dev_matrix), 1ull << log_height,
                                       width, column_mask, ctx->partials, ctx->small, ctx->stream));
  ps.end();
  HIP_TRY(ctx, hipMemcpyAsync(ctx->pinned, ctx->small, 16, hipMemcpyDeviceToHost, ctx->stream));
  HIP_TRY(ctx, hipStreamSynchronize(ctx->stream));
  memcpy(out, ctx->pinned, 16);
  return MLH_OK;
}

}

struct CsCall {
  PoolBuf buf;
  std::vector<uint8_t> img;
  CsDev dev{};
  const fe* vinv = nullptr;
  uint32_t threads = 0;
  explicit CsCall(mlh_ctx* c) : buf(c) {}
  mlh_status init(mlh_ctx* ctx, const mlh_cs_program* prog, const uint8_t* host_randoms,
                  const uint8_t* host_mask) {
    const CsProgram& p = prog->p;
    std::vector<u128> rnd(p.n_randoms), mask(p.n_constraints);
    for (uint32_t i = 0; i < p.n_randoms; ++i)
      if ((rnd[i] = h_load(host_randoms + 16ull * i)) >= kModulus)
        return fail(ctx, MLH_ERR_INVALID, "non-canonical random");
    for (uint32_t i = 0; i < p.n_constraints; ++i)
      if ((mask[i] = h_load(host_mask + 16ull * i)) >= kModulus)
        return fail(ctx, MLH_ERR_INVALID, "non-canonical mask");
    const CsImageLayout l = cs_image_layout(p);
    img = cs_build_image(p, rnd.data(), mask.data());
    MLH_TRY(buf.alloc(l.bytes));
    HIP_TRY(ctx, hipMemcpyAsync(buf.p, img.data(), l.bytes, hipMemcpyHostToDevice, ctx->stream));
    const uint8_t* b = buf.as<uint8_t>();
    dev.uni = reinterpret_cast<const fe*>(b);
    dev.code = reinterpret_cast<const uint32_t*>(b + l.code_off);
    dev.outs = reinterpret_cast<const uint32_t*>(b + l.outs_off);
    dev.width = p.width;
    dev.n_temps = p.n_temps;
    dev.n_instr = p.n_instr;
    dev.n_constraints = p.n_constraints;
    dev.D = p.points();
    vinv = dev.uni + l.vinv_off;
    threads = cs_threads(cs_slots(p));
    return MLH_OK;
  }
};

static bool cs_args_ok(const mlh_cs_program* prog, uint32_t width, const void* m, const void* d,
                       const uint8_t* randoms, const uint8_t* mask) {
  return prog && m && d && mask && width == prog->p.width && (!prog->p.n_randoms || randoms);
}

static mlh_status cs_read_sums(mlh_ctx* ctx, const CsCall& cc, uint32_t nb, uint8_t* out) {
  HIP_TRY(ctx, launch_cs_reduce(ctx->partials, nb, cc.dev.D, ctx->small, ctx->stream));
  HIP_TRY(ctx, hipMemcpyAsync(ctx->pinned, ctx->small, 16ull * cc.dev.D, hipMemcpyDeviceToHost,
                              ctx->stream));
  HIP_TRY(ctx, hipStreamSynchronize(ctx->stream));
  memcpy(out, ctx->pinned, 16ull * cc.dev.D);
  return MLH_OK;
}

extern "C" {

mlh_status mlh_cs_partial_sums(mlh_ctx* ctx, const mlh_cs_program* prog, uint32_t width,
                               const void* dev_matrix, const void* dev_delta, uint32_t log_height,
                               const uint8_t* host_randoms, const uint8_t* host_mask,
                               uint8_t* out) {
  if (!ctx || !out || !cs_args_ok(prog, width, dev_matrix, dev_delta, host_randoms, host_mask) ||
      log_height < 1 || log_height > kCsMaxLogHeight)
    return fail(ctx, MLH_ERR_INVALID, "bad argument");
  CsCall cc(ctx);
  MLH_TRY(cc.init(ctx, prog, host_randoms, host_mask));
  uint32_t nb = 0;
  HIP_TRY(ctx, launch_cs_sums(cc.dev, cc.threads, reinterpret_cast<const fe*>(dev_matrix),
                              reinterpret_cast<const fe*>(dev_delta), 1ull << (log_height - 1),
                              ctx->partials, ctx->stream, &nb));
  return cs_read_sums(ctx, cc, nb, out);
}

mlh_status mlh_cs_fold(mlh_ctx* ctx, uint32_t width, void* dev_matrix, void* dev_delta,
                       uint32_t log_height, const uint8_t r[16]) {
  if (!ctx || !dev_matrix || !dev_delta || !r || width < 1 || width > kCsMaxWidth ||
      log_height < 1 || log_height > kCsMaxLogHeight || h_load(r) >= kModulus)
    return fail(ctx, MLH_ERR_INVALID, "bad argument");
  HIP_TRY(ctx, launch_cs_fold(width, reinterpret_cast<fe*>(dev_matrix),
                              reinterpret_cast<fe*>(dev_delta), 1ull << log_height,
                              to_fe(h_load(r)), nullptr, ctx->stream));
  return MLH_OK;
}

mlh_status mlh_cs_fold_and_sums(mlh_ctx* ctx, const mlh_cs_program* prog, uint32_t width,
                                void* dev_matrix, void* dev_delta, uint32_t log_height,
                                const uint8_t* host_randoms, const uint8_t* host_mask,
                                const uint8_t r[16], uint8_t* out) {
  if (!ctx || !out || !r || !cs_args_ok(prog, width, dev_matrix, dev_delta, host_randoms, host_mask) ||
      log_height < 2 || log_height > kCsMaxLogHeight || h_load(r) >= kModulus)
    return fail(ctx, MLH_ERR_INVALID, "bad argument");
  CsCall cc(ctx);
  MLH_TRY(cc.init(ctx, prog, host_randoms, host_mask));
  uint32_t nb = 0;
  HIP_TRY(ctx, launch_cs_fold_sums(cc.dev, cc.threads, reinterpret_cast<fe*>(dev_matrix),
                                   reinterpret_cast<fe*>(dev_delta), 1ull << log_height,
                                   to_fe(h_load(r)), nullptr, ctx->partials, ctx->stream, &nb));
  return cs_read_sums(ctx, cc, nb, out);
}

mlh_status mlh_cs_sumcheck_prove(mlh_ctx* ctx, const mlh_cs_program* prog, uint32_t width,
                                 void* dev_matrix, void* dev_delta, uint32_t log_height,
                                 const uint8_t* host_randoms, const uint8_t* host_mask,
                                 const uint8_t sum[16], mlh_transcript* tr, uint8_t* polys_out,
                                 uint8_t* rs_out) {
  return mlh_cs_sumcheck_prove_sums(ctx, prog, width, dev_matrix, dev_delta, log_height, host_randoms,
                                    host_mask, 0, nullptr, sum, tr, polys_out, rs_out);
}

mlh_status mlh_cs_sumcheck_prove_sums(mlh_ctx* ctx, const mlh_cs_program* prog, uint32_t width,
                                      void* dev_matrix, void* dev_delta, uint32_t log_height,
                                      const uint8_t* host_randoms, const uint8_t* host_mask,
                                      uint32_t sum_column_mask, const uint8_t* beta,
                                      const uint8_t claim[16], mlh_transcript* tr,
                                      uint8_t* polys_out, uint8_t* rs_out) {
  if (!ctx || !claim || !tr || !cs_args_ok(prog, width, dev_matrix, dev_delta, host_randoms, host_mask) ||
      log_height > kCsMaxLogHeight || h_load(claim) >= kModulus)
    return fail(ctx, MLH_ERR_INVALID, "bad argument");
  const uint32_t smask = sum_column_mask;
  if (smask && (!beta || h_load(beta) >= kModulus || (width < 32 && (smask >> width))))
    return fail(ctx, MLH_ERR_INVALID, "sum columns: beta missing or a mask bit at or above the width");
  const uint32_t L = log_height;
  if (L == 0) return MLH_OK;
  CsCall cc(ctx);
  MLH_TRY(cc.init(ctx, prog, host_randoms, host_mask));
  const uint32_t D = cc.dev.D;
  RoundBuf rb(ctx, D, L);
  MLH_TRY(rb.alloc(smask ? 32ull * kCsMaxBlocks : 0));
  fe* lin = smask ? rb.extra() : nullptr;
  const fe fbeta = smask ? to_fe(h_load(beta)) : fe{};
  MLH_TRY(rb.seed(tr, claim));
  fe* m = reinterpret_cast<fe*>(dev_matrix);
  fe* d = reinterpret_cast<fe*>(dev_delta);
  uint32_t nb = 0;
  {
    ProfScope ps(ctx, "cs_sums");
    HIP_TRY(ctx, launch_cs_sums(cc.dev, cc.threads, m, d, 1ull << (L - 1), ctx->partials,
                                ctx->stream, &nb, smask, lin));
    ps.end();
  }
  for (uint32_t k = 0; k < L; ++k) {
    {
      ProfScope ps(ctx, "cs_round");
      HIP_TRY(ctx, launch_cs_round(ctx->partials, nb, D, cc.vinv, rb.prev(), rb.dt(), rb.poly(k),
                                   rb.r(k), ctx->stream, lin, fbeta));
      ps.end();
    }
    const uint64_t S = 1ull << (L - k);
    if (S >= 4) {
      ProfScope ps(ctx, "cs_fold_sums");
      HIP_TRY(ctx, launch_cs_fold_sums(cc.dev, cc.threads, m, d, S, fe{}, rb.r(k), ctx->partials,
                                       ctx->stream, &nb, smask, lin));
      ps.end();
    } else {
      ProfScope ps(ctx, "cs_fold");
      HIP_TRY(ctx, launch_cs_fold(width, m, d, S, fe{}, rb.r(k), ctx->stream));
      ps.end();
    }
  }
  static_assert(16ull * (kCsMaxDegree + 2) * kCsMaxLogHeight <= kPinStage, "prove staging");
  MLH_TRY(rb.read_back());
  MLH_TRY(rb.replay(tr));
  rb.copy_out(polys_out, rs_out);
  return MLH_OK;
}

}

static mlh_status system_prove_core(mlh_ctx* ctx, const mlh_cs_program* prog,
                                    const mlh_trace_commitment* com1,
                                    const mlh_trace_commitment* com2, uint32_t sum_column_mask,
                                    void* dev_matrix, const uint8_t sum[16],
                                    const uint8_t* column_sum, mlh_transcript* tr,
                                    uint8_t* polys_out, uint8_t* output_out,
                                    mlh_batched_pcs_proof* pcs1, mlh_batched_pcs_proof* pcs2) {
  const uint32_t L = com1->log_height, W = prog->p.width;
  TranscriptGuard guard(tr);
  SystemHead h(prog->p, L);
  if (system_head(tr, prog->p, L, com1->root, com2 ? com2->root : nullptr, sum_column_mask, sum,
                  column_sum, &h) != MLH_OK)
    return fail(ctx, MLH_ERR_INVALID, "challenge set");
  PoolBuf delta(ctx);
  MLH_TRY(delta.alloc(16ull << L));
  MLH_TRY(mlh_eq_table(ctx, h.row.data(), L, delta.p));
  std::vector<uint8_t> rs(16ull * L);
  {
    ProfScope ps(ctx, "system_sumcheck");
    MLH_TRY(mlh_cs_sumcheck_prove_sums(ctx, prog, W, dev_matrix, delta.p, L, h.randoms.data(),
                                       h.mask.data(), sum_column_mask, h.beta, h.claim, tr,
                                       polys_out, rs.data()));
    ps.end();
  }
  HIP_TRY(ctx, hipMemcpyAsync(ctx->pinned, dev_matrix, 16ull * W, hipMemcpyDeviceToHost, ctx->stream));
  HIP_TRY(ctx, hipStreamSynchronize(ctx->stream));
  std::vector<uint8_t> output(ctx->pinned, ctx->pinned + 16ull * W);
  {
    ProfScope ps(ctx, "system_open");
    MLH_TRY(batched_pcs_open(ctx, reinterpret_cast<const fe*>(com1->codes), com1->evals,
                             reinterpret_cast<const uint8_t*>(com1->tree), com1->width, L, rs.data(),
                             output.data(), tr, pcs1));
    ps.end();
  }
  if (com2) {
    ProfScope ps(ctx, "system_open2");
    MLH_TRY(batched_pcs_open(ctx, reinterpret_cast<const fe*>(com2->codes), com2->evals,
                             reinterpret_cast<const uint8_t*>(com2->tree), com2->width, L, rs.data(),
                             output.data() + 16ull * com1->width, tr, pcs2));
    ps.end();
  }
  memcpy(output_out, output.data(), output.size());
  guard.keep();
  return MLH_OK;
}

extern "C" {

mlh_status mlh_system_prove(mlh_ctx* ctx, const mlh_cs_program* prog,
                            const mlh_trace_commitment* com, void* dev_matrix,
                            const uint8_t sum[16], mlh_transcript* tr, mlh_system_proof* proof) {
  if (!ctx || !prog || !com || !dev_matrix || !sum || !tr || !proof || !proof->sumcheck_polys ||
      !proof->output)
    return fail(ctx, MLH_ERR_INVALID, "null argument");
  if (com->ctx != ctx) return fail(ctx, MLH_ERR_INVALID, "commitment of another context");
  if (prog->p.width != com->width)
    return fail(ctx, MLH_ERR_INVALID, "program width differs from the commitment's");
  if (h_load(sum) >= kModulus) return fail(ctx, MLH_ERR_INVALID, "non-canonical sum");
  MLH_TRY(system_prove_core(ctx, prog, com, nullptr, 0, dev_matrix, sum, nullptr, tr,
                            proof->sumcheck_polys, proof->output, &proof->pcs, nullptr));
  proof->log_height = com->log_height;
  proof->width = com->width;
  proof->degree = prog->p.degree;
  return MLH_OK;
}

mlh_status mlh_system_prove_phased(mlh_ctx* ctx, const mlh_cs_program* prog,
                                   const mlh_trace_commitment* com1,
                                   const mlh_trace_commitment* com2, uint32_t sum_column_mask,
                                   void* dev_matrix, const uint8_t sum[16],
                                   const uint8_t column_sum[16], mlh_transcript* tr,
                                   mlh_phased_proof* proof) {
  if (!ctx || !prog || !com1 || !dev_matrix || !sum || !column_sum || !tr || !proof ||
      !proof->sumcheck_polys || !proof->output)
    return fail(ctx, MLH_ERR_INVALID, "null argument");
  if (com1->ctx != ctx || (com2 && com2->ctx != ctx))
    return fail(ctx, MLH_ERR_INVALID, "commitment of another context");
  const uint32_t W = prog->p.width, P1 = com1->width, P2 = com2 ? com2->width : 0;
  if (P1 < 1 || P1 + P2 != W || (com2 && com2->log_height != com1->log_height))
    return fail(ctx, MLH_ERR_INVALID,
                "the commitments' widths must add up to the program's (com2 null iff all columns "
                "are pre-random), over the same rows");
  if (W < 32 && (sum_column_mask >> W))
    return fail(ctx, MLH_ERR_INVALID, "sum column at or above the width");
  if (h_load(sum) >= kModulus || h_load(column_sum) >= kModulus)
    return fail(ctx, MLH_ERR_INVALID, "non-canonical sum");
  MLH_TRY(system_prove_core(ctx, prog, com1, com2, sum_column_mask, dev_matrix, sum, column_sum, tr,
                            proof->sumcheck_polys, proof->output, &proof->pcs[0], &proof->pcs[1]));
  proof->log_height = com1->log_height;
  proof->width = W;
  proof->degree = prog->p.degree;
  proof->pre_random_columns = P1;
  proof->sum_column_mask = sum_column_mask;
  return MLH_OK;
}

}
```

multilinear_amd/csrc/context.hpp:

```cpp
#pragma once
#include <hip/hip_runtime.h>
#include <stdint.h>
#include <string.h>

#include <algorithm>
#include <map>
#include <memory>
#include <string>
#include <unordered_map>
#include <tuple>
#include <vector>

#include "../../include/mlhip.h"
#include "host_transcript.hpp"
#include "field.hpp"
#include "host_field.hpp"
#include "ntt.hpp"

using mlh::fe;
using mlh::kMaxPasses;
using mlh::u128;

constexpr size_t kPinnedBytes = 16384, kPinStage = 12288, kPinSlotA = 12288, kPinSlotB = 12800;

struct TableKey {
  u128 base;
  uint64_t count;
  u128 scale;
  int expand;
  uint64_t cols = 0;
  uint64_t mult = 0;
  bool operator<(const TableKey& o) const {
    return std::tie(base, count, scale, expand, cols, mult) <
           std::tie(o.base, o.count, o.scale, o.expand, o.cols, o.mult);
  }
};

struct CachedTable {
  fe* d = nullptr;
  size_t bytes = 0;
  uint64_t stamp = 0;
};

struct mlh_ctx {
  int device = 0;
  hipStream_t stream = nullptr;
  std::string err;
  std::map<TableKey, CachedTable> tables;
  size_t table_bytes = 0;
  size_t table_limit = (size_t)1 << 30;
  uint64_t table_stamp = 0;
  std::multimap<size_t, void*> pool;
  std::map<void*, size_t> live;
  fe* partials = nullptr;
  fe* small = nullptr;
  uint8_t* pinned = nullptr;
  volatile uint32_t* dev_status = nullptr;
  uint32_t coop_spin = 0;
  uint32_t pcs_fused_max = 24;
  uint8_t* qstage = nullptr;
  size_t qstage_bytes = 0;
  fe* ntt_scratch = nullptr;
  size_t ntt_scratch_bytes = 0;
  hipStream_t side = nullptr;
  hipStream_t side2 = nullptr;
  bool debug_sync = false;
  uint32_t forced_plan[kMaxPasses] = {0};
  uint32_t forced_plan_len = 0;
  bool prof_on = false;
  uint32_t prof_every = 1;
  std::unordered_map<std::string, uint64_t> prof_ticks;
  std::vector<hipEvent_t> ev_free;
  struct Pending {
    std::string label;
    hipEvent_t a, b;
  };
  std::vector<Pending> pending;
  std::map<std::string, std::pair<uint64_t, double>> prof;
};

inline hipEvent_t take_event(mlh_ctx* ctx) {
  if (!ctx->ev_free.empty()) {
    hipEvent_t e = ctx->ev_free.back();
    ctx->ev_free.pop_back();
    return e;
  }
  hipEvent_t e = nullptr;
  (void)hipEventCreate(&e);
  return e;
}

inline void resolve_profile(mlh_ctx* ctx) {
  for (auto& p : ctx->pending) {
    (void)hipEventSynchronize(p.b);
    float ms = 0;
    (void)hipEventElapsedTime(&ms, p.a, p.b);
    auto& slot = ctx->prof[p.label];
    slot.first += 1;
    slot.second += ms;
  }
  std::vector<hipEvent_t> evs;
  for (auto& p : ctx->pending) {
    evs.push_back(p.a);
    evs.push_back(p.b);
  }
  std::sort(evs.begin(), evs.end());
  evs.erase(std::unique(evs.begin(), evs.end()), evs.end());
  for (auto e : evs) ctx->ev_free.push_back(e);
  ctx->pending.clear();
}

inline bool prof_sample(mlh_ctx* ctx, const char* label) {
  if (!ctx->prof_on) return false;
  if (ctx->prof_every <= 1) return true;
  return ctx->prof_ticks[label]++ % ctx->prof_every == 0;
}

struct ProfScope {
  mlh_ctx* ctx;
  const char* label;
  hipEvent_t a = nullptr;
  ProfScope(mlh_ctx* c, const char* lab) : ctx(c), label(lab) {
    if (prof_sample(ctx, label)) {
      a = take_event(ctx);
      (void)hipEventRecord(a, ctx->stream);
    }
  }
  void end() {
    if (!a) return;
    hipEvent_t b = take_event(ctx);
    (void)hipEventRecord(b, ctx->stream);
    ctx->pending.push_back(mlh_ctx::Pending{label, a, b});
    a = nullptr;
  }
  ~ProfScope() {
    if (a) ctx->ev_free.push_back(a);
  }
};


inline mlh_status fail(mlh_ctx* ctx, mlh_status st, const std::string& msg) {
  if (ctx) ctx->err = msg;
  return st;
}

#ifndef MLH_SYNC_SPIN
#define MLH_SYNC_SPIN 0
#endif
inline hipError_t prove_wait(mlh_ctx* ctx) {
  if (!MLH_SYNC_SPIN) return hipStreamSynchronize(ctx->stream);
  hipError_t e;
  while ((e = hipStreamQuery(ctx->stream)) == hipErrorNotReady) {
  }
  return e;
}

inline void device_arm(mlh_ctx* ctx) {
  (void)hipMemsetAsync(const_cast<uint32_t*>(ctx->dev_status), 0, sizeof(uint32_t), ctx->stream);
}
inline mlh_status device_check(mlh_ctx* ctx) {
  const uint32_t s = *ctx->dev_status;
  if (!s) return MLH_OK;
  *ctx->dev_status = 0;
  return fail(ctx, MLH_ERR_DEVICE,
              "a cooperative sumcheck kernel gave up waiting (spin limit): its outputs are invalid");
}

struct ReplayCheck {
  mlh_ctx* ctx;
  mlh_transcript* tr;
  mlh::HostSha256 saved;
  bool committed = false;
  uint32_t bad = 0, first_bad = ~0u, n = 0;
  ReplayCheck(mlh_ctx* c, mlh_transcript* t) : ctx(c), tr(t), saved(t->sha) {}
  ReplayCheck(const ReplayCheck&) = delete;
  ReplayCheck& operator=(const ReplayCheck&) = delete;
  ~ReplayCheck() {
    if (!committed) tr->sha = saved;
  }
  void absorb(const uint8_t* p, uint64_t len) { mlh_transcript_absorb(tr, p, len); }
  void expect(const uint8_t* dev_r) {
    uint8_t h[16];
    mlh_transcript_next_challenge(tr, h);
    if (memcmp(h, dev_r, 16) != 0) {
      if (!bad) first_bad = n;
      ++bad;
    }
    ++n;
  }
  mlh_status status() {
    if (!bad) {
      committed = true;
      return MLH_OK;
    }
    return fail(ctx, MLH_ERR_DEVICE,
                "device transcript diverged from the host replay at challenge " +
                    std::to_string(first_bad) + " (" + std::to_string(bad) + " of " +
                    std::to_string(n) + " differ)");
  }
};

struct StreamSwap {
  mlh_ctx* ctx;
  hipStream_t saved;
  StreamSwap(mlh_ctx* c, hipStream_t s) : ctx(c), saved(c->stream) { c->stream = s; }
  ~StreamSwap() { ctx->stream = saved; }
};

#define HIP_TRY(ctx, expr)                                                                \
  do {                                                                                    \
    hipError_t e_ = (expr);                                                               \
    if (e_ != hipSuccess)                                                                 \
      return fail((ctx), MLH_ERR_HIP, std::string(#expr ": ") + hipGetErrorString(e_));  \
  } while (0)

#define MLH_TRY(expr)              \
  do {                             \
    mlh_status s_ = (expr);        \
    if (s_ != MLH_OK) return s_;   \
  } while (0)

inline mlh::fe to_fe(u128 v) {
  fe r;
  memcpy(r.w, &v, 16);
  return r;
}
inline mlh::u128 from_fe(const mlh::fe& x) {
  u128 v;
  memcpy(&v, x.w, 16);
  return v;
}

inline mlh_status pool_alloc(mlh_ctx* ctx, size_t bytes, void** out) {
  bytes = (bytes + 255) & ~(size_t)255;
  auto it = ctx->pool.lower_bound(bytes);
  if (it != ctx->pool.end() && it->first <= bytes + bytes / 4) {
    *out = it->second;
    ctx->live[it->second] = it->first;
    ctx->pool.erase(it);
    return MLH_OK;
  }
  void* p = nullptr;
  hipError_t e = hipMalloc(&p, bytes);
  if (e != hipSuccess) {
    for (auto& kv : ctx->pool) (void)hipFree(kv.second);
    ctx->pool.clear();
    e = hipMalloc(&p, bytes);
    if (e != hipSuccess) return fail(ctx, MLH_ERR_OOM, "hipMalloc failed");
  }
  ctx->live[p] = bytes;
  *out = p;
  return MLH_OK;
}
inline void pool_free(mlh_ctx* ctx, void* p) {
  if (!p) return;
  auto it = ctx->live.find(p);
  if (it == ctx->live.end()) return;
  ctx->pool.emplace(it->second, p);
  ctx->live.erase(it);
}

struct PoolBuf {
  mlh_ctx* ctx;
  void* p = nullptr;
  explicit PoolBuf(mlh_ctx* c) : ctx(c) {}
  ~PoolBuf() { pool_free(ctx, p); }
  mlh_status alloc(size_t bytes) { return pool_alloc(ctx, bytes, &p); }
  void* release() {
    void* q = p;
    p = nullptr;
    return q;
  }
  template <class T>
  T* as() const {
    return reinterpret_cast<T*>(p);
  }
};
```

multilinear_amd/csrc/ntt.hip:

```cpp
#include <stdio.h>
#include <stdlib.h>

#include <type_traits>

#include "bfly_asm.hpp"
#include "field.hpp"
#include "ntt.hpp"

namespace mlh {

constexpr int kCols = 8;
constexpr int kLogCols = 3;
constexpr int kEPT = 8;

__device__ __forceinline__ uint32_t bitrev(uint32_t x, int bits) {
  return __builtin_bitreverse32(x) >> (32 - bits);
}

struct PassGeom {
  uint32_t log_n;
  uint32_t nradix;
  uint32_t p;
  uint32_t logr[kMaxPasses];
  uint32_t lstride;
  uint32_t loga;
  uint32_t ltpv;
  uint32_t lin_v;
  uint32_t lout_v;
  uint32_t sh_p = 0, sh_rank = 0, sh_lchunk = 0;
};

__device__ __forceinline__ uint64_t reverse_mid_digits(const PassGeom& g, uint64_t mid) {
  uint64_t rev = 0;
  for (int q = (int)g.nradix - 2; q >= 1; --q) {
    uint32_t shift = 0;
    for (int i = 1; i < q; ++i) shift += g.logr[i];
    rev += (mid & ((1ull << g.logr[q]) - 1)) << shift;
    mid >>= g.logr[q];
  }
  return rev;
}

#ifndef MLH_WPS8
#define MLH_WPS8 4
#endif
#ifndef MLH_LAST_STAGED
#define MLH_LAST_STAGED 1
#endif
#ifndef MLH_LAST_DIRECT
#define MLH_LAST_DIRECT 1
#endif
#ifndef MLH_LDS_PAD
#define MLH_LDS_PAD 0
#endif
#ifndef MLH_DIAG_TW
#define MLH_DIAG_TW 0
#endif
#ifndef MLH_LDS_TW
#define MLH_LDS_TW 1
#endif
constexpr int pass_waves_per_simd(int logr, int ept) {
  return ept == 16 ? 2 : (logr == 8 ? MLH_WPS8 : (logr == 9 ? 4 : (logr == 7 ? 4 : 2)));
}

template <int LOGR, int TW, int ZT, int EPT = kEPT>
__global__ void __launch_bounds__(kCols * (1 << LOGR) / EPT,
                                  (TW == 2 || TW == 4) ? 1 : pass_waves_per_simd(LOGR, EPT))
ntt_pass_kernel(const fe* in, fe* out, const fe* __restrict__ tw,
                const fe* __restrict__ ta, const fe* __restrict__ tb, PassGeom g) {
  constexpr int R = 1 << LOGR;
  constexpr int LQ = EPT == 16 ? 4 : 3;
  constexpr int TPC = R / EPT;
  constexpr bool LAST = TW == 2 || TW == 4;
  constexpr bool SH = TW == 4;
  auto phys = [&](uint64_t v) -> uint64_t {
    if constexpr (SH)
      return ((v & ((1ull << g.sh_p) - 1)) << g.sh_lchunk) |
             ((v >> g.sh_p) & ((1ull << g.sh_lchunk) - 1));
    else
      return v;
  };
  __shared__ fe lds[R * kCols];
#if MLH_LDS_TW
  __shared__ fe lds_tw[LOGR > LQ ? 2 * R : 1];
  if constexpr (LOGR > LQ) {
    constexpr int NT = kCols * R / EPT;
    static_assert((2 * R) % NT == 0, "twiddle copy: whole rounds");
#pragma unroll
    for (int e = 0; e < 2 * R / NT; ++e)
      lds_tw[e * NT + threadIdx.x] = fe_load(tw + e * NT + threadIdx.x);
  }
#endif

  const int tid = threadIdx.x;
  constexpr bool kDirect = MLH_LAST_DIRECT && LAST && !SH && ZT == 0 && EPT == 8 && LOGR >= 6;
  constexpr int kLTPC = LOGR - 3;
  const int cB = tid % kCols;
  int c = cB;
  int t = tid / kCols;
  if constexpr (kDirect) {
    c = tid >> kLTPC;
    t = (int)bitrev((uint32_t)tid & ((1u << kLTPC) - 1), kLTPC);
  }
  const uint64_t vec = (uint64_t)blockIdx.x >> g.ltpv;
  uint64_t tile = blockIdx.x & ((1ull << g.ltpv) - 1);
  if constexpr (SH) {
    const uint32_t lmid = g.log_n - g.logr[0] - LOGR;
    const uint32_t ld1 = g.logr[0] - kLogCols - g.sh_p;
    tile = ((((uint64_t)g.sh_rank << ld1) | (tile >> lmid)) << lmid) | (tile & ((1ull << lmid) - 1));
  }
  in += vec << g.lin_v;
  out += vec << g.lout_v;

  uint64_t base, jrest = 0, k1 = 0, mid = 0;
  uint32_t rshift;
  uint32_t cshift;
  if (!LAST) {
    const uint32_t lw = g.lstride;
    const uint64_t hi = tile >> (lw - kLogCols), lo = tile & ((1ull << (lw - kLogCols)) - 1);
    base = (hi << (LOGR + lw)) + (lo << kLogCols);
    jrest = (lo << kLogCols) + cB;
    rshift = lw;
    cshift = 0;
  } else {
    const uint32_t lw1 = g.log_n - g.logr[0];
    const uint32_t lmid = lw1 - LOGR;
    const uint64_t d1hi = tile >> lmid;
    mid = tile & ((1ull << lmid) - 1);
    base = (d1hi << (kLogCols + lw1)) + (mid << LOGR);
    k1 = (d1hi << kLogCols) + cB;
    rshift = 0;
    cshift = lw1;
  }
  const fe* src = in + base + ((uint64_t)c << cshift);
  fe* dst = out + base + ((uint64_t)cB << cshift);


  fe x[EPT];
#if MLH_LAST_STAGED
  if constexpr (LAST && ZT == 0 && !kDirect) {
    constexpr int NT = kCols * R / EPT;
    auto swz = [&](uint32_t row) -> uint32_t {
      if constexpr (SH) return (row ^ (row >> g.sh_p)) & (kCols - 1);
      else return row & (kCols - 1);
    };
#pragma unroll
    for (int e = 0; e < EPT; ++e) {
      const uint32_t idx = (uint32_t)(e * NT + tid);
      const uint32_t l = idx & 63, grp = idx >> 6;
      uint32_t row = grp * 8 + (l & 7);
      if constexpr (SH) {
        const uint32_t lq = LOGR - g.sh_p - 3;
        const uint32_t src = grp >> lq, q0 = grp & ((1u << lq) - 1);
        row = ((((q0 << 3) + (l & 7)) << g.sh_p)) | src;
      }
      const uint32_t col = l >> 3;
      lds[row * kCols + (col ^ swz(row))] = fe_load(in + phys(base + ((uint64_t)col << cshift) + row));
    }
    __syncthreads();
#pragma unroll
    for (int e = 0; e < EPT; ++e) {
      const uint32_t row = bitrev((uint32_t)(t * EPT + e), LOGR);
      x[e] = lds[row * kCols + (c ^ swz(row))];
    }
  } else
#endif
#pragma unroll
  for (int e = 0; e < EPT; ++e) {
    const uint32_t row = bitrev((uint32_t)(t * EPT + e), LOGR);
    if (ZT != 0 && (e & 1)) {
      x[e] = fe_zero();
    } else if (ZT == 2) {
      const uint32_t logw = g.log_n - LOGR;
      const uint64_t colr = __builtin_bitreverse64(jrest) >> (64 - logw);
      x[e] = fe_load(in + (colr << (LOGR - 1)) + ((uint32_t)(t * EPT + e) >> 1));
    } else if constexpr (SH) {
      x[e] = fe_load(in + phys(base + ((uint64_t)c << cshift) + ((uint64_t)row << rshift)));
    } else {
      x[e] = fe_load(src + ((uint64_t)row << rshift));
    }
  }

  auto run_phase = [&](auto S0_, auto Q_) {
    constexpr int s0 = decltype(S0_)::value;
    constexpr int q = decltype(Q_)::value;
    constexpr int G = EPT >> q;
    constexpr int NB = EPT / 2;
    constexpr int BPG = 1 << (q - 1);
#pragma unroll
    for (int s = s0; s < s0 + q; ++s) {
      const int d = 1 << (s - s0);
      int be0[NB], be1[NB];
      uint32_t bj[NB];
      bool btriv[NB];
#pragma unroll
      for (int b = 0; b < NB; ++b) {
        const int gi = b / BPG, m = b % BPG;
        const int i = ((m >> (s - s0)) << (s - s0 + 1)) | (m & (d - 1));
        be0[b] = gi * (1 << q) + i;
        be1[b] = be0[b] + d;
        const uint32_t gamma = (uint32_t)(t * G + gi);
        const uint32_t bpos = (gamma & ((1u << s0) - 1u)) | ((gamma >> s0) << (s0 + q));
        const uint32_t pos = bpos + ((uint32_t)i << s0);
        bj[b] = pos & ((1u << s) - 1u);
        btriv[b] = s0 == 0 && (s == 0 || (i & ((1 << s) - 1)) == 0);
      }
      if (ZT != 0 && s0 == 0 && s == 0) {
#pragma unroll
        for (int b = 0; b < NB; ++b) x[be1[b]] = x[be0[b]];
        continue;
      }
      uint64_t rare;
#pragma unroll
      for (int b = 0; b < NB; b += 2) {
        fe& u0 = x[be0[b]];
        fe& v0 = x[be1[b]];
        fe& u1 = x[be0[b + 1]];
        fe& v1 = x[be1[b + 1]];
        if (s0 == 0) {
          const fe* w0 = tw + 4 * (bj[b] << (LOGR - 1 - s));
          const fe* w1 = tw + 4 * (bj[b + 1] << (LOGR - 1 - s));
          if (!btriv[b] && !btriv[b + 1])
            bfly_mm_s(u0, v0, w0[0], w0[1], w0[2], w0[3], u1, v1, w1[0], w1[1], w1[2], w1[3], rare);
          else if (!btriv[b])
            bfly_mt_s(u0, v0, w0[0], w0[1], w0[2], w0[3], u1, v1, rare);
          else if (!btriv[b + 1])
            bfly_mt_s(u1, v1, w1[0], w1[1], w1[2], w1[3], u0, v0, rare);
          else
            bfly_tt_v(u0, v0, u1, v1, rare);
        } else {
#if MLH_LDS_TW
          const fe* w0 = lds_tw + 4 * (bj[b] << (LOGR - 1 - s));
          const fe* w1 = lds_tw + 4 * (bj[b + 1] << (LOGR - 1 - s));
#else
          const fe* w0 = tw + 4 * (bj[b] << (LOGR - 1 - s));
          const fe* w1 = tw + 4 * (bj[b + 1] << (LOGR - 1 - s));
#endif
          bfly_mm_v(u0, v0, w0[0], w0[1], w0[2], w0[3], u1, v1, w1[0], w1[1], w1[2], w1[3], rare);
        }
      }
    }
  };
  auto positions = [&](auto S0_, auto Q_, uint32_t (&pos)[EPT]) {
    constexpr int s0 = decltype(S0_)::value;
    constexpr int q = decltype(Q_)::value;
    constexpr int G = EPT >> q;
#pragma unroll
    for (int gi = 0; gi < G; ++gi) {
      const uint32_t gamma = (uint32_t)(t * G + gi);
      const uint32_t bpos = (gamma & ((1u << s0) - 1u)) | ((gamma >> s0) << (s0 + q));
#pragma unroll
      for (int i = 0; i < (1 << q); ++i) pos[gi * (1 << q) + i] = bpos + ((uint32_t)i << s0);
    }
  };

  using I0 = std::integral_constant<int, 0>;
  constexpr int Q1 = LOGR < LQ ? LOGR : LQ;
  run_phase(I0{}, std::integral_constant<int, Q1>{});
  uint32_t pos[EPT];
  positions(I0{}, std::integral_constant<int, Q1>{}, pos);

  auto exchange_and_run = [&](auto S0_, auto Q_) {
    __syncthreads();
#pragma unroll
    for (int e = 0; e < EPT; ++e) fe_store(&lds[pos[e] * kCols + c], x[e]);
    __syncthreads();
    positions(S0_, Q_, pos);
#pragma unroll
    for (int e = 0; e < EPT; ++e) x[e] = fe_load(&lds[pos[e] * kCols + c]);
    run_phase(S0_, Q_);
  };
  constexpr int NTt = kCols * R / EPT;
  constexpr int kTbPerThread = TW == 0 ? R / NTt : 1;
  fe tbv[kTbPerThread][4];
  const uint64_t jl = jrest & ((1ull << g.loga) - 1);
  fe ta_c0, ta_c1;
#ifndef MLH_TB_COALESCED
#define MLH_TB_COALESCED 1
#endif
  auto load_tb = [&]() {
    if constexpr (TW == 0 && MLH_DIAG_TW == 0) {
      const uint64_t jh = jrest >> g.loga;
      const uint32_t ltcols = g.lstride - g.loga;
#pragma unroll
      for (int e = 0; e < kTbPerThread; ++e) {
#if MLH_TB_COALESCED
#pragma unroll
        for (int k = 0; k < 4; ++k) {
          const uint32_t i = (uint32_t)((e * 4 + k) * NTt + tid);
          tbv[e][k] = fe_load(tb + ((((uint64_t)(i >> 2) << ltcols) + jh) << 2) + (i & 3));
        }
#else
        const fe* q = tb + ((((uint64_t)(e * NTt + tid) << ltcols) + jh) << 2);
#pragma unroll
        for (int k = 0; k < 4; ++k) tbv[e][k] = fe_load(q + k);
#endif
      }
    }
  };
  auto load_ta0 = [&](const uint32_t (&pf)[EPT]) {
    if constexpr (TW == 5) {
      (void)pf;
    } else if constexpr (!LAST && MLH_DIAG_TW == 2) {
      ta_c0 = fe{{(uint32_t)jl | 1u, 7u, 9u, 3u}};
      ta_c1 = fe{{(uint32_t)pf[1] | 1u, 5u, 9u, 3u}};
    } else if constexpr (!LAST) {
      ta_c0 = fe_load(ta + ((uint64_t)pf[0] << g.loga) + jl);
      ta_c1 = fe_load(ta + ((uint64_t)pf[1] << g.loga) + jl);
    }
  };
#ifndef MLH_P0_EARLY_TB
#define MLH_P0_EARLY_TB 0
#endif

  constexpr bool kEarly = MLH_P0_EARLY_TB && TW == 0 && LOGR > 2 * LQ;
  if constexpr (LOGR > LQ) {
    constexpr int Q2 = (LOGR - LQ) < LQ ? (LOGR - LQ) : LQ;
    if constexpr (kDirect) {
      auto slot = [&](uint32_t row, int col) -> uint32_t {
        return row * kCols + ((uint32_t)col ^ ((row >> (LOGR - 3)) & (kCols - 1)));
      };
      __syncthreads();
#pragma unroll
      for (int e = 0; e < EPT; ++e) fe_store(&lds[slot(pos[e], c)], x[e]);
      __syncthreads();
      c = cB;
      t = tid / kCols;
      positions(std::integral_constant<int, LQ>{}, std::integral_constant<int, Q2>{}, pos);
#pragma unroll
      for (int e = 0; e < EPT; ++e) x[e] = fe_load(&lds[slot(pos[e], c)]);
      run_phase(std::integral_constant<int, LQ>{}, std::integral_constant<int, Q2>{});
    } else {
      exchange_and_run(std::integral_constant<int, LQ>{}, std::integral_constant<int, Q2>{});
    }
    if constexpr (LOGR > 2 * LQ) {
      constexpr int Q3 = LOGR - 2 * LQ;
      static_assert(Q3 <= LQ, "LOGR <= 3 * LQ");
      if constexpr (kEarly) {
        uint32_t pf[EPT];
        positions(std::integral_constant<int, 2 * LQ>{}, std::integral_constant<int, Q3>{}, pf);
        load_tb();
        if (MLH_P0_EARLY_TB == 1) load_ta0(pf);
      }
      exchange_and_run(std::integral_constant<int, 2 * LQ>{}, std::integral_constant<int, Q3>{});
    }
  }

  if constexpr (!kEarly) {
    load_ta0(pos);
    load_tb();
  } else if (MLH_P0_EARLY_TB == 2) {
    load_ta0(pos);
  }
  if constexpr (TW == 0) {
    static_assert(4 * R <= R * kCols, "the expanded TB column fits the exchange tile");
    constexpr int NT = NTt;
    __syncthreads();
#pragma unroll
    for (int e = 0; e < kTbPerThread; ++e)
#pragma unroll
      for (int k = 0; k < 4; ++k)
        lds[MLH_TB_COALESCED ? (e * 4 + k) * NT + tid : 4 * (e * NT + tid) + k] = tbv[e][k];
    __syncthreads();
  }
  uint64_t kbase = 0;
  uint32_t kshift = 0;
  if (LAST) {
    kbase = k1 + (reverse_mid_digits(g, mid) << g.logr[0]);
    kshift = g.log_n - LOGR;
  }
  if constexpr (TW == 5) {
    constexpr int Q3 = LOGR - 2 * LQ, NI = 1 << Q3, G = EPT / NI;
    static_assert(LOGR > 2 * LQ && G % 2 == 0, "progression twiddle: groups in pairs");
    fe tv[G];
#pragma unroll
    for (int gq = 0; gq < G; ++gq) tv[gq] = fe_load(ta + ((uint64_t)pos[gq * NI] << g.lstride) + jrest);
    const fe* cp = tb + 4 * jrest;
    const fe c0 = fe_load(cp), c1 = fe_load(cp + 1), c2 = fe_load(cp + 2), c3 = fe_load(cp + 3);
#pragma unroll
    for (int i = 0; i < NI; ++i) {
      uint64_t rare;
#pragma unroll
      for (int gq = 0; gq < G; gq += 2) {
        const int e0 = gq * NI + i, e1 = (gq + 1) * NI + i;
        bfly_ff_v(x[e0], tv[gq], x[e1], tv[gq + 1], rare);
        fe_store(dst + ((uint64_t)pos[e0] << rshift), x[e0]);
        fe_store(dst + ((uint64_t)pos[e1] << rshift), x[e1]);
      }
      if (i + 1 < NI) {
#pragma unroll
        for (int gq = 0; gq < G; gq += 2) bfly_pp_v(tv[gq], c0, c1, c2, c3, tv[gq + 1], c0, c1, c2, c3, rare);
      }
    }
  } else if constexpr (!LAST) {
#pragma unroll
    for (int e = 0; e < EPT; e += 2) {
      uint64_t rare;
      const fe a0 = ta_c0, a1 = ta_c1;
      if (e + 2 < EPT && MLH_DIAG_TW < 2) {
        ta_c0 = fe_load(ta + ((uint64_t)pos[e + 2] << g.loga) + jl);
        ta_c1 = fe_load(ta + ((uint64_t)pos[e + 3] << g.loga) + jl);
      }
      bfly_ff_v(x[e], a0, x[e + 1], a1, rare);
      if constexpr (TW == 0 && MLH_DIAG_TW == 0) {
        const fe* b0 = lds + 4 * pos[e];
        const fe* b1 = lds + 4 * pos[e + 1];
        bfly_pp_v(x[e], b0[0], b0[1], b0[2], b0[3], x[e + 1], b1[0], b1[1], b1[2], b1[3], rare);
      }
      fe_store(dst + ((uint64_t)pos[e] << rshift), x[e]);
      fe_store(dst + ((uint64_t)pos[e + 1] << rshift), x[e + 1]);
    }
  } else {
    static_assert(EPT % 4 == 0, "canonicalisation in fours");
#pragma unroll
    for (int e = 0; e < EPT; e += 4) bfly_cccc_v(x[e], x[e + 1], x[e + 2], x[e + 3]);
#pragma unroll
    for (int e = 0; e < EPT; ++e) {
      uint64_t K = kbase + ((uint64_t)pos[e] << kshift);
      if constexpr (SH) {
        const uint32_t lo = g.logr[0] - g.sh_p;
        K = ((K >> g.logr[0]) << lo) | (K & ((1ull << lo) - 1));
      }
      fe_store(out + K, x[e]);
    }
  }
  (void)TPC;
}

__global__ void __launch_bounds__(512)
ntt_small_kernel(const fe* __restrict__ in, fe* __restrict__ out, const fe* __restrict__ tw,
                 uint32_t log_n, uint32_t in_len, fe scale, int apply_scale, int brev_in) {
  __shared__ fe lds[1024];
  const uint32_t N = 1u << log_n;
  in += (uint64_t)blockIdx.x * in_len;
  out += (uint64_t)blockIdx.x * N;
  for (uint32_t i = threadIdx.x; i < N; i += blockDim.x) {
    const uint32_t src = bitrev(i, (int)log_n);
    const uint32_t at = (brev_in && in_len > 1) ? bitrev(src, 31 - __builtin_clz(in_len)) : src;
    lds[i] = src < in_len ? fe_load(in + at) : fe_zero();
  }
  __syncthreads();
  for (uint32_t s = 0; s < log_n; ++s) {
    const uint32_t h = 1u << s;
    for (uint32_t b = threadIdx.x; b < N / 2; b += blockDim.x) {
      const uint32_t j = b & (h - 1);
      const uint32_t p0 = j + ((b >> s) << (s + 1));
      const fe u = lds[p0];
      fe v = lds[p0 + h];
      if (j) v = fe_mul(v, tw[j << (log_n - 1 - s)]);
      lds[p0] = fe_add(u, v);
      lds[p0 + h] = fe_sub(u, v);
    }
    __syncthreads();
  }
  for (uint32_t i = threadIdx.x; i < N; i += blockDim.x) {
    fe v = lds[i];
    if (apply_scale) v = fe_mul(v, scale);
    fe_store(out + i, v);
  }
}

__global__ void pow_table_kernel(fe* __restrict__ out, fe base, fe scale, uint64_t count,
                                 int expand) {
  const uint64_t t = (uint64_t)blockIdx.x * blockDim.x + threadIdx.x;
  if (t >= count) return;
  fe v = fe_pow(base, t);
  v = fe_mul(v, scale);
  if (!expand) {
    fe_store(out + t, v);
    return;
  }
#pragma unroll
  for (int k = 0; k < 4; ++k) {
    fe_store(out + 4 * t + k, v);
    v = fe_mul(v, fe{{0u, 1u, 0u, 0u}});
  }
}

__global__ void pow_table2d_kernel(fe* __restrict__ out, fe base, fe scale, uint64_t rows,
                                   uint64_t cols, uint64_t mult, int expand) {
  const uint64_t t = (uint64_t)blockIdx.x * blockDim.x + threadIdx.x;
  if (t >= rows * cols) return;
  const uint64_t k = t / cols, j = t % cols;
  fe v = fe_mul(fe_pow(base, k * j * mult), scale);
  if (!expand) {
    fe_store(out + t, v);
    return;
  }
#pragma unroll
  for (int q = 0; q < 4; ++q) {
    fe_store(out + 4 * t + q, v);
    v = fe_mul(v, fe{{0u, 1u, 0u, 0u}});
  }
}

hipError_t launch_pow_table2d(fe* out, fe base, fe scale, uint64_t rows, uint64_t cols,
                              uint64_t mult, hipStream_t st, bool expand) {
  const uint64_t n = rows * cols;
  hipLaunchKernelGGL(pow_table2d_kernel, dim3((unsigned)((n + 255) / 256)), dim3(256), 0, st, out,
                     base, scale, rows, cols, mult, expand ? 1 : 0);
  return hipGetLastError();
}

__global__ void pow_series_kernel(fe* __restrict__ out, const fe* __restrict__ tlo,
                                  const fe* __restrict__ thi, uint64_t count) {
  const uint64_t t = (uint64_t)blockIdx.x * blockDim.x + threadIdx.x;
  if (t >= count) return;
  fe_store(out + t, fe_mul(tlo[t & 4095], thi[t >> 12]));
}

__global__ void pow_series_check_kernel(const fe* __restrict__ gp, uint64_t base, uint64_t count,
                                        const fe* __restrict__ tlo, const fe* __restrict__ thi,
                                        unsigned long long* bad) {
  const uint64_t t = (uint64_t)blockIdx.x * blockDim.x + threadIdx.x;
  if (t >= count) return;
  const uint64_t i = base + t;
  const fe want = fe_mul(tlo[i & 4095], thi[i >> 12]);
  const fe got = fe_load(gp + t);
  if ((want.w[0] ^ got.w[0]) | (want.w[1] ^ got.w[1]) | (want.w[2] ^ got.w[2]) | (want.w[3] ^ got.w[3]))
    atomicMin(bad, (unsigned long long)i);
}

constexpr uint32_t kNetLB = 11;

__device__ __forceinline__ fe net_tw(const fe* __restrict__ tlo, const fe* __restrict__ thi,
                                     uint64_t t) {
  const uint64_t lo = t & 4095, hi = t >> 12;
  if (!hi) return fe_load(tlo + lo);
  if (!lo) return fe_load(thi + hi);
  return fe_mul(fe_load(tlo + lo), fe_load(thi + hi));
}

__device__ __forceinline__ uint64_t bitrev64(uint64_t x, uint32_t bits) {
  return bits ? __builtin_bitreverse64(x) >> (64 - bits) : 0;
}

__global__ void __launch_bounds__(1024)
ntt_net_block_kernel(const fe* __restrict__ in, fe* __restrict__ out, const fe* __restrict__ tlo,
                     const fe* __restrict__ thi, uint32_t log_n, uint32_t lb, int zero_top, fe scale, int apply_scale) {
  __shared__ fe lds[1u << kNetLB];
  const uint32_t B = 1u << lb;
  const uint64_t N = 1ull << log_n, base = (uint64_t)blockIdx.x << lb;
  for (uint32_t i = threadIdx.x; i < B; i += blockDim.x) {
    const uint64_t src = bitrev64(base + i, log_n);
    fe v;
    if (zero_top == 0) v = fe_load(in + src);
    else if (src >= N / 2) v = fe_zero();
    else v = fe_load(in + (zero_top == 2 ? bitrev64(src, log_n - 1) : src));
    lds[i] = v;
  }
  __syncthreads();
  for (uint32_t s = 0; s < lb; ++s) {
    const uint32_t h = 1u << s;
    for (uint32_t b = threadIdx.x; b < B / 2; b += blockDim.x) {
      const uint32_t j = b & (h - 1);
      const uint32_t p0 = j + ((b >> s) << (s + 1));
      const fe u = lds[p0];
      fe v = lds[p0 + h];
      if (j) v = fe_mul(v, net_tw(tlo, thi, (uint64_t)j << (log_n - 1 - s)));
      lds[p0] = fe_add(u, v);
      lds[p0 + h] = fe_sub(u, v);
    }
    __syncthreads();
  }
  for (uint32_t i = threadIdx.x; i < B; i += blockDim.x) {
    fe v = lds[i];
    if (apply_scale) v = fe_mul(v, scale);
    fe_store(out + base + i, v);
  }
}

template <int Q>
__global__ void __launch_bounds__(256)
ntt_net_stage_kernel(const fe* in, fe* out, const fe* __restrict__ tlo, const fe* __restrict__ thi,
                     uint32_t log_n,
                     uint32_t s0, fe scale, int apply_scale) {
  const uint64_t g = (uint64_t)blockIdx.x * blockDim.x + threadIdx.x;
  if (g >= (1ull << (log_n - Q))) return;
  const uint64_t low = g & ((1ull << s0) - 1);
  const uint64_t base = ((g >> s0) << (s0 + Q)) | low;
  fe x[1 << Q];
#pragma unroll
  for (int m = 0; m < (1 << Q); ++m) x[m] = fe_load(in + base + ((uint64_t)m << s0));
#pragma unroll
  for (int q = 0; q < Q; ++q) {
    const uint32_t s = s0 + q;
    const int d = 1 << q;
#pragma unroll
    for (int b = 0; b < (1 << (Q - 1)); ++b) {
      const int m = ((b >> q) << (q + 1)) | (b & (d - 1));
      const uint64_t j = (base + ((uint64_t)m << s0)) & ((1ull << s) - 1);
      const fe v = j ? fe_mul(x[m + d], net_tw(tlo, thi, j << (log_n - 1 - s))) : x[m + d];
      const fe u = x[m];
      x[m] = fe_add(u, v);
      x[m + d] = fe_sub(u, v);
    }
  }
#pragma unroll
  for (int m = 0; m < (1 << Q); ++m) {
    fe v = x[m];
    if (apply_scale) v = fe_mul(v, scale);
    fe_store(out + base + ((uint64_t)m << s0), v);
  }
}

hipError_t launch_ntt_network(const fe* in, fe* out, fe* scratch, const fe* tlo, const fe* thi,
                              uint32_t log_n,
                              int zero_top, fe scale, bool apply_scale, hipStream_t st) {
  if (log_n < 1 || log_n > 40 || (zero_top && in == out)) return hipErrorInvalidValue;
  const uint32_t lb = log_n < kNetLB ? log_n : kNetLB;
  const uint64_t blocks = 1ull << (log_n - lb);
  fe* first = (in == out && blocks > 1) ? scratch : out;
  const bool only = lb == log_n;
  const uint32_t threads = lb >= 11 ? 1024 : (1u << lb) / 2 < 64 ? 64 : (1u << lb) / 2;
  hipLaunchKernelGGL(ntt_net_block_kernel, dim3((unsigned)blocks), dim3(threads), 0, st, in, first,
                     tlo, thi, log_n, lb, zero_top, scale, (only && apply_scale) ? 1 : 0);
  hipError_t e = hipGetLastError();
  for (uint32_t s0 = lb; e == hipSuccess && s0 < log_n;) {
    const uint32_t q = log_n - s0 < 4 ? log_n - s0 : 4;
    const bool last = s0 + q == log_n;
    fe* dst = last ? out : first;
    const int sc = (last && apply_scale) ? 1 : 0;
    const dim3 grid((unsigned)(((1ull << (log_n - q)) + 255) / 256)), blk(256);
    switch (q) {
      case 1: hipLaunchKernelGGL(ntt_net_stage_kernel<1>, grid, blk, 0, st, first, dst, tlo, thi, log_n, s0, scale, sc); break;
      case 2: hipLaunchKernelGGL(ntt_net_stage_kernel<2>, grid, blk, 0, st, first, dst, tlo, thi, log_n, s0, scale, sc); break;
      case 3: hipLaunchKernelGGL(ntt_net_stage_kernel<3>, grid, blk, 0, st, first, dst, tlo, thi, log_n, s0, scale, sc); break;
      default: hipLaunchKernelGGL(ntt_net_stage_kernel<4>, grid, blk, 0, st, first, dst, tlo, thi, log_n, s0, scale, sc); break;
    }
    e = hipGetLastError();
    s0 += q;
  }
  return e;
}


template <int LOGR, int EPT>
static hipError_t launch_pass_ept(bool last, int zero_top, const fe* in, fe* out, const fe* tw,
                                  const fe* ta, const fe* tb, const PassGeom& g, uint64_t tiles,
                                  hipStream_t st, bool geo = false) {
  constexpr int threads = kCols * (1 << LOGR) / EPT;
  const dim3 grid((unsigned)tiles), blk(threads);
#define MLH_PASS(TWV, ZTV)                                                                  \
  hipLaunchKernelGGL((ntt_pass_kernel<LOGR, TWV, ZTV, EPT>), grid, blk, MLH_LDS_PAD, st, in, out, \
                     tw, ta, tb, g)
  if (last) {
    if (zero_top) return hipErrorInvalidValue;
    MLH_PASS(2, 0);
  } else if (geo) {
    if constexpr ((LOGR == 7 || LOGR == 8) && EPT == 8) {
      if (zero_top == 2) MLH_PASS(5, 2);
      else if (zero_top == 1) MLH_PASS(5, 1);
      else MLH_PASS(5, 0);
    } else {
      return hipErrorInvalidValue;
    }
  } else if (!tb && g.p == 0) {
    if (zero_top == 2) MLH_PASS(3, 2);
    else if (zero_top == 1) MLH_PASS(3, 1);
    else MLH_PASS(3, 0);
  } else if (!tb) {
    if (zero_top) return hipErrorInvalidValue;
    MLH_PASS(1, 0);
  } else {
    if (zero_top == 2) MLH_PASS(0, 2);
    else if (zero_top == 1) MLH_PASS(0, 1);
    else MLH_PASS(0, 0);
  }
#undef MLH_PASS
  return hipGetLastError();
}

template <int LOGR>
static hipError_t launch_pass(bool last, int zero_top, const fe* in, fe* out, const fe* tw,
                              const fe* ta, const fe* tb, const PassGeom& g, uint64_t tiles,
                              hipStream_t st, bool geo = false) {
  return launch_pass_ept<LOGR, kEPT>(last, zero_top, in, out, tw, ta, tb, g, tiles, st, geo);
}

void ntt_plan_radices(uint32_t log_n, uint32_t* nradix, uint32_t* logr, const uint32_t* forced,
                      uint32_t nforced) {
  if (forced && nforced >= 2 && nforced <= (uint32_t)kMaxPasses) {
    uint32_t sum = 0;
    bool ok = true;
    for (uint32_t i = 0; i < nforced; ++i) {
      ok = ok && forced[i] >= 4 && forced[i] <= 9;
      sum += forced[i];
    }
    if (ok && sum == log_n) {
      *nradix = nforced;
      for (uint32_t i = 0; i < nforced; ++i) logr[i] = forced[i];
      return;
    }
  }
  const uint32_t P = (log_n + 8) / 9;
  *nradix = P;
  uint32_t rem = log_n;
  for (uint32_t p = 0; p < P; ++p) {
    const uint32_t left = P - p;
    const uint32_t r = (rem + left - 1) / left;
    logr[p] = r;
    rem -= r;
  }
}

hipError_t launch_ntt_small(const fe* in, fe* out, const fe* tw, uint32_t log_n, uint64_t in_len,
                            fe scale, bool apply_scale, hipStream_t st, uint64_t batch,
                            bool brev_in) {
  const uint32_t N = 1u << log_n;
  const uint32_t threads = N / 2 < 64 ? 64 : (N / 2 > 512 ? 512 : N / 2);
  hipLaunchKernelGGL(ntt_small_kernel, dim3((unsigned)batch), dim3(threads), 0, st, in, out, tw, log_n,
                     (uint32_t)in_len, scale, apply_scale ? 1 : 0, brev_in ? 1 : 0);
  return hipGetLastError();
}

void ntt_pass_label(const NttTables& tb, uint32_t p, int zero_top, char* buf, size_t n) {
  const bool last = p + 1 == tb.nradix;
  const int tw = last ? 2 : (tb.gp[p] ? 5 : (tb.tb[p] ? 0 : (p == 0 ? 3 : 1)));
  snprintf(buf, n, "ntt_pass<%u,%d,%d>", tb.logr[p], tw, p == 0 ? zero_top : 0);
}

hipError_t launch_ntt_passes(const fe* in, fe* out, fe* scratch, const NttTables& tb,
                             uint32_t log_n, int zero_top, hipStream_t st, hipEvent_t* ev,
                             uint64_t batch) {
  PassGeom g;
  g.log_n = log_n;
  g.nradix = tb.nradix;
  for (uint32_t p = 0; p < tb.nradix; ++p) g.logr[p] = tb.logr[p];
  const uint64_t N = 1ull << log_n;
  uint64_t W = N;
  for (uint32_t p = 0; p < tb.nradix; ++p) {
    const uint32_t lr = tb.logr[p];
    W >>= lr;
    g.p = p;
    g.lstride = (uint32_t)__builtin_ctzll(W);
    g.loga = tb.loga[p];
    const bool last = (p + 1 == tb.nradix);
    g.ltpv = log_n - kLogCols - lr;
    const uint64_t tiles = (N >> (kLogCols + lr)) * batch;
    g.lin_v = (p == 0 && zero_top) ? log_n - 1 : log_n;
    g.lout_v = log_n;
    const fe* src = (p == 0) ? in : scratch;
    fe* dst = last ? out : scratch;
    const int zt = p == 0 ? zero_top : 0;
    if (ev) (void)hipEventRecord(ev[p], st);
    hipError_t e;
    const bool geo = tb.gp[p] != nullptr;
    const fe* ta = geo ? tb.gp[p] : tb.ta[p];
    const fe* tbb = geo ? tb.gc[p] : tb.tb[p];
    switch (lr) {
      case 4: e = launch_pass<4>(last, zt, src, dst, tb.tw[p], ta, tbb, g, tiles, st, geo); break;
      case 5: e = launch_pass<5>(last, zt, src, dst, tb.tw[p], ta, tbb, g, tiles, st, geo); break;
      case 6: e = launch_pass<6>(last, zt, src, dst, tb.tw[p], ta, tbb, g, tiles, st, geo); break;
      case 7: e = launch_pass<7>(last, zt, src, dst, tb.tw[p], ta, tbb, g, tiles, st, geo); break;
      case 8: e = launch_pass<8>(last, zt, src, dst, tb.tw[p], ta, tbb, g, tiles, st, geo); break;
      case 9: e = launch_pass<9>(last, zt, src, dst, tb.tw[p], ta, tbb, g, tiles, st, geo); break;
      default: return hipErrorInvalidValue;
    }
    if (e != hipSuccess) return e;
    if (tb.debug_sync) {
      e = hipStreamSynchronize(st);
      if (e != hipSuccess) return e;
    }
  }
  if (ev) (void)hipEventRecord(ev[tb.nradix], st);
  return hipSuccess;
}

__global__ void __launch_bounds__(256)
scale_rows_kernel(const fe* __restrict__ in, fe* __restrict__ out, uint64_t n, uint32_t lcols, fe rowbase) {
  const uint64_t i = (uint64_t)blockIdx.x * blockDim.x + threadIdx.x;
  if (i >= n) return;
  uint64_t k = i >> lcols;
  fe f = fe_one(), b = rowbase;
  while (k) {
    if (k & 1) f = fe_mul(f, b);
    b = fe_mul(b, b);
    k >>= 1;
  }
  fe_store(out + i, fe_mul(fe_load(in + i), f));
}

hipError_t launch_scale_rows(const fe* in, fe* out, uint64_t rows, uint32_t lcols, fe rowbase,
                             hipStream_t st) {
  const uint64_t n = rows << lcols;
  hipLaunchKernelGGL(scale_rows_kernel, dim3((unsigned)((n + 255) / 256)), dim3(256), 0, st, in, out, n,
                     lcols, rowbase);
  return hipGetLastError();
}

hipError_t launch_ntt_passes_pre(const fe* in, fe* out, const NttTables& tb, uint32_t log_n,
                                 uint32_t npasses, hipStream_t st) {
  if (npasses == 0 || npasses >= tb.nradix) return hipErrorInvalidValue;
  PassGeom g;
  g.log_n = log_n;
  g.nradix = tb.nradix;
  for (uint32_t p = 0; p < tb.nradix; ++p) g.logr[p] = tb.logr[p];
  const uint64_t N = 1ull << log_n;
  uint64_t W = N;
  for (uint32_t p = 0; p < npasses; ++p) {
    const uint32_t lr = tb.logr[p];
    W >>= lr;
    g.p = p;
    g.lstride = (uint32_t)__builtin_ctzll(W);
    g.loga = tb.loga[p];
    g.ltpv = log_n - kLogCols - lr;
    g.lin_v = g.lout_v = log_n;
    const uint64_t tiles = N >> (kLogCols + lr);
    const fe* src = p == 0 ? in : out;
    hipError_t e;
    switch (lr) {
      case 4: e = launch_pass<4>(false, 0, src, out, tb.tw[p], tb.ta[p], tb.tb[p], g, tiles, st); break;
      case 5: e = launch_pass<5>(false, 0, src, out, tb.tw[p], tb.ta[p], tb.tb[p], g, tiles, st); break;
      case 6: e = launch_pass<6>(false, 0, src, out, tb.tw[p], tb.ta[p], tb.tb[p], g, tiles, st); break;
      case 7: e = launch_pass<7>(false, 0, src, out, tb.tw[p], tb.ta[p], tb.tb[p], g, tiles, st); break;
      case 8: e = launch_pass<8>(false, 0, src, out, tb.tw[p], tb.ta[p], tb.tb[p], g, tiles, st); break;
      case 9: e = launch_pass<9>(false, 0, src, out, tb.tw[p], tb.ta[p], tb.tb[p], g, tiles, st); break;
      default: return hipErrorInvalidValue;
    }
    if (e != hipSuccess) return e;
  }
  return hipSuccess;
}

hipError_t launch_ntt_shard_last(const fe* recv, fe* out, const fe* tw, const uint32_t* logr,
                                 uint32_t nradix, uint32_t log_n, uint32_t log_p, uint32_t rank,
                                 hipStream_t st) {
  if (nradix < 2 || nradix > (uint32_t)kMaxPasses) return hipErrorInvalidValue;
  const uint32_t lr = logr[nradix - 1];
  if (lr < log_p + 3 || logr[0] < kLogCols + log_p) return hipErrorInvalidValue;
  PassGeom g;
  g.log_n = log_n;
  g.nradix = nradix;
  for (uint32_t p = 0; p < nradix; ++p) g.logr[p] = logr[p];
  g.p = nradix - 1;
  g.lstride = 0;
  g.loga = 0;
  g.ltpv = log_n - kLogCols - lr - log_p;
  g.lin_v = g.lout_v = log_n;
  g.sh_p = log_p;
  g.sh_rank = rank;
  g.sh_lchunk = log_n - 2 * log_p;
  const dim3 grid((unsigned)(1ull << g.ltpv));
#define MLH_SHL(LR)                                                                                 \
  hipLaunchKernelGGL((ntt_pass_kernel<LR, 4, 0, kEPT>), grid, dim3(kCols * (1 << LR) / kEPT), MLH_LDS_PAD, \
                     st, recv, out, tw, nullptr, nullptr, g)
  switch (lr) {
    case 6: MLH_SHL(6); break;
    case 7: MLH_SHL(7); break;
    case 8: MLH_SHL(8); break;
    case 9: MLH_SHL(9); break;
    default: return hipErrorInvalidValue;
  }
#undef MLH_SHL
  return hipGetLastError();
}

hipError_t launch_pow_table(fe* out, fe base, fe scale, uint64_t count, hipStream_t st,
                            bool expand) {
  const unsigned blocks = (unsigned)((count + 255) / 256);
  hipLaunchKernelGGL(pow_table_kernel, dim3(blocks), dim3(256), 0, st, out, base, scale, count,
                     expand ? 1 : 0);
  return hipGetLastError();
}

hipError_t launch_pow_series(fe* out, const fe* tlo, const fe* thi, uint64_t count,
                             hipStream_t st) {
  const unsigned blocks = (unsigned)((count + 255) / 256);
  hipLaunchKernelGGL(pow_series_kernel, dim3(blocks), dim3(256), 0, st, out, tlo, thi, count);
  return hipGetLastError();
}

hipError_t launch_pow_series_check(const fe* gp, uint64_t base, uint64_t count, const fe* tlo,
                                   const fe* thi, unsigned long long* bad, hipStream_t st) {
  if (count == 0) return hipSuccess;
  const unsigned blocks = (unsigned)((count + 255) / 256);
  hipLaunchKernelGGL(pow_series_check_kernel, dim3(blocks), dim3(256), 0, st, gp, base, count, tlo,
                     thi, bad);
  return hipGetLastError();
}

}
```

multilinear_amd/csrc/ntt.hpp:

```cpp
#pragma once
#include <hip/hip_runtime.h>
#include <stdint.h>

#include "field.hpp"

namespace mlh {

constexpr int kMaxPasses = 6;
constexpr uint32_t kTwLogA = 8;
#ifndef MLH_FULL_TW_LOG
#define MLH_FULL_TW_LOG 22
#endif
constexpr uint32_t kFullTwLog = MLH_FULL_TW_LOG;

struct NttTables {
  uint32_t log_n = 0;
  uint32_t nradix = 0;
  uint32_t logr[kMaxPasses] = {0};
  const fe* tw[kMaxPasses] = {nullptr};
  const fe* ta[kMaxPasses] = {nullptr};
  const fe* tb[kMaxPasses] = {nullptr};
  uint32_t loga[kMaxPasses] = {0};
  const fe* gp[kMaxPasses] = {nullptr};
  const fe* gc[kMaxPasses] = {nullptr};
  const fe* tw_small = nullptr;
  fe scale;
  bool inverse = false;
  bool debug_sync = false;
};

void ntt_plan_radices(uint32_t log_n, uint32_t* nradix, uint32_t* logr,
                      const uint32_t* forced = nullptr, uint32_t nforced = 0);

hipError_t launch_ntt_small(const fe* in, fe* out, const fe* tw, uint32_t log_n, uint64_t in_len,
                            fe scale, bool apply_scale, hipStream_t st, uint64_t batch = 1,
                            bool brev_in = false);
hipError_t launch_ntt_passes(const fe* in, fe* out, fe* scratch, const NttTables& tb,
                             uint32_t log_n, int zero_top, hipStream_t st,
                             hipEvent_t* ev = nullptr, uint64_t batch = 1);
hipError_t launch_scale_rows(const fe* in, fe* out, uint64_t rows, uint32_t lcols, fe rowbase,
                             hipStream_t st);
hipError_t launch_ntt_passes_pre(const fe* in, fe* out, const NttTables& tb, uint32_t log_n,
                                 uint32_t npasses, hipStream_t st);
hipError_t launch_ntt_shard_last(const fe* recv, fe* out, const fe* tw, const uint32_t* logr,
                                 uint32_t nradix, uint32_t log_n, uint32_t log_p, uint32_t rank,
                                 hipStream_t st);
void ntt_pass_label(const NttTables& tb, uint32_t p, int zero_top, char* buf, size_t n);
hipError_t launch_ntt_network(const fe* in, fe* out, fe* scratch, const fe* tlo, const fe* thi,
                              uint32_t log_n,
                              int zero_top, fe scale, bool apply_scale, hipStream_t st);
hipError_t launch_pow_table(fe* out, fe base, fe scale, uint64_t count, hipStream_t st,
                            bool expand = false);
hipError_t launch_pow_table2d(fe* out, fe base, fe scale, uint64_t rows, uint64_t cols,
                              uint64_t mult, hipStream_t st, bool expand = false);
hipError_t launch_pow_series(fe* out, const fe* tlo, const fe* thi, uint64_t count,
                             hipStream_t st);
hipError_t launch_pow_series_check(const fe* gp, uint64_t base, uint64_t count, const fe* tlo,
                                   const fe* thi, unsigned long long* bad, hipStream_t st);

}
```

Before: 38.83 billion.

## Use uniform base plus 32-bit lane offsets for NTT pass global and LDS addressing

Rewrites the NTT pass kernel address math so each access becomes a wave-uniform 64-bit tile base (read via readfirstlane) plus a per-lane 32-bit byte offset. Compile-time position constants replace the per-element pos arrays. The aim is to cut VGPR use and 64-bit address arithmetic per load and store. A wide-offset 64-bit variant is kept for passes whose extent exceeds 32 bits, and an env var can force it. A batched NTT API entry point is also added.

```diff
diff --git a/include/mlhip.h b/include/mlhip.h
--- a/include/mlhip.h
+++ b/include/mlhip.h
@@ -61,6 +61,8 @@
                    const uint8_t gen[16]);
 mlh_status mlh_intt(mlh_ctx* ctx, const void* dev_evals, void* dev_coeffs, uint32_t log_n,
                     const uint8_t gen[16]);
+mlh_status mlh_ntt_batch(mlh_ctx* ctx, const void* dev_coeffs, void* dev_evals, uint32_t log_n,
+                         const uint8_t gen[16], uint32_t log_batch);
 mlh_status mlh_bit_reverse_permutation(mlh_ctx* ctx, const void* dev_in, void* dev_out,
                                        uint32_t log_n);
 mlh_status mlh_ntt_host(mlh_ctx* ctx, const uint8_t* host_in, uint8_t* host_out, uint32_t log_n,
diff --git a/multilinear_amd/_lib.py b/multilinear_amd/_lib.py
--- a/multilinear_amd/_lib.py
+++ b/multilinear_amd/_lib.py
@@ -140,6 +140,7 @@
     "mlh_field_inv": (_I, [_P, _P, _P, _U64]),
     "mlh_ntt": (_I, [_P, _P, _P, _U32, _P]),
     "mlh_intt": (_I, [_P, _P, _P, _U32, _P]),
+    "mlh_ntt_batch": (_I, [_P, _P, _P, _U32, _P, _U32]),
     "mlh_bit_reverse_permutation": (_I, [_P, _P, _P, _U32]),
     "mlh_ntt_host": (_I, [_P, _P, _P, _U32, _P, _I]),
     "mlh_reed_solomon": (_I, [_P, _P, _U32, _P, _P]),
diff --git a/multilinear_amd/csrc/capi.hip b/multilinear_amd/csrc/capi.hip
--- a/multilinear_amd/csrc/capi.hip
+++ b/multilinear_amd/csrc/capi.hip
@@ -130,6 +130,7 @@
     return MLH_OK;
   }
   tb->debug_sync = ctx->debug_sync;
+  tb->wide_offsets = ctx->ntt_wide_offsets;
   if (plan)
     ntt_plan_radices(log_n, &tb->nradix, tb->logr, plan, nplan);
   else
@@ -350,6 +351,8 @@
   c->stream = reinterpret_cast<hipStream_t>(hip_stream);
   const char* dbg = getenv("MLH_DEBUG_SYNC");
   c->debug_sync = dbg && *dbg && strcmp(dbg, "0") != 0;
+  const char* wide = getenv("MLH_NTT_WIDE_OFFSETS");
+  c->ntt_wide_offsets = wide && *wide && strcmp(wide, "0") != 0;
   void* st = nullptr;
   const bool ok = hipMalloc(&c->partials, 2 * kMaxRedBlocks * sizeof(fe)) == hipSuccess &&
                   hipMalloc(&c->small, 64 * sizeof(fe)) == hipSuccess &&
@@ -567,6 +570,29 @@
 mlh_status mlh_intt(mlh_ctx* ctx, const void* dev_evals, void* dev_coeffs, uint32_t log_n,
                     const uint8_t gen[16]) {
   return ntt_entry(ctx, dev_evals, dev_coeffs, log_n, gen, true);
+}
+
+mlh_status mlh_ntt_batch(mlh_ctx* ctx, const void* dev_coeffs, void* dev_evals, uint32_t log_n,
+                         const uint8_t gen[16], uint32_t log_batch) {
+  if (!ctx || !dev_coeffs || !dev_evals || !gen) return fail(ctx, MLH_ERR_INVALID, "null argument");
+  if (log_n < 1 || log_n > 32 || log_n + log_batch > 32)
+    return fail(ctx, MLH_ERR_NOT_POW2, "The number of coeffs must be a power of 2 (n >= 2)");
+  const u128 g = h_load(gen);
+  if (g >= kModulus || !check_generator(g, log_n))
+    return fail(ctx, MLH_ERR_BAD_GENERATOR, "generator not of order 2^log_n");
+  const fe* in = reinterpret_cast<const fe*>(dev_coeffs);
+  fe* out = reinterpret_cast<fe*>(dev_evals);
+  NttTables tb;
+  MLH_TRY(get_ntt_tables(ctx, g, log_n, false, &tb));
+  const uint64_t batch = 1ull << log_batch;
+  if (log_n <= 10) {
+    HIP_TRY(ctx, launch_ntt_small(in, out, tb.tw_small, log_n, 1ull << log_n, tb.scale, false,
+                                  ctx->stream, batch));
+    return MLH_OK;
+  }
+  MLH_TRY(ensure_ntt_scratch(ctx, log_n + log_batch));
+  HIP_TRY(ctx, launch_ntt_passes(in, out, ctx->ntt_scratch, tb, log_n, 0, ctx->stream, nullptr, batch));
+  return MLH_OK;
 }
 
 static mlh_status vec_op(mlh_ctx* ctx, int op, const void* a, const void* b, void* out, uint64_t n) {
diff --git a/multilinear_amd/csrc/context.hpp b/multilinear_amd/csrc/context.hpp
--- a/multilinear_amd/csrc/context.hpp
+++ b/multilinear_amd/csrc/context.hpp
@@ -65,6 +65,7 @@
   hipStream_t side = nullptr;
   hipStream_t side2 = nullptr;
   bool debug_sync = false;
+  bool ntt_wide_offsets = false;
   uint32_t forced_plan[kMaxPasses] = {0};
   uint32_t forced_plan_len = 0;
   bool prof_on = false;
diff --git a/multilinear_amd/csrc/ntt.hip b/multilinear_amd/csrc/ntt.hip
--- a/multilinear_amd/csrc/ntt.hip
+++ b/multilinear_amd/csrc/ntt.hip
@@ -15,6 +15,41 @@
 
 __device__ __forceinline__ uint32_t bitrev(uint32_t x, int bits) {
   return __builtin_bitreverse32(x) >> (32 - bits);
+}
+
+typedef uint32_t u32x4 __attribute__((ext_vector_type(4)));
+typedef __attribute__((address_space(1))) u32x4 global_u32x4;
+template <typename Off>
+__device__ __forceinline__ global_u32x4* pass_addr(const void* ubase, Off lane_bytes) {
+  uint64_t v = reinterpret_cast<uint64_t>(ubase);
+  if constexpr (sizeof(Off) == 4) {
+    const uint32_t lo = __builtin_amdgcn_readfirstlane((uint32_t)v);
+    const uint32_t hi = __builtin_amdgcn_readfirstlane((uint32_t)(v >> 32));
+    v = ((uint64_t)hi << 32) | lo;
+  }
+  return (global_u32x4*)(v + lane_bytes);
+}
+template <typename Off>
+__device__ __forceinline__ fe fe_load_at(const fe* ubase, Off lane_bytes) {
+  const u32x4 v = *pass_addr<Off>(ubase, lane_bytes);
+  return fe{{v.x, v.y, v.z, v.w}};
+}
+template <typename Off>
+__device__ __forceinline__ void fe_store_at(fe* ubase, Off lane_bytes, const fe& x) {
+  *pass_addr<Off>(ubase, lane_bytes) = u32x4{x.w[0], x.w[1], x.w[2], x.w[3]};
+}
+__device__ __forceinline__ void pin_lane_offset(uint32_t& v) { asm("" : "+v"(v)); }
+__device__ __forceinline__ void pin_lane_offset(uint64_t&) {}
+constexpr uint32_t bitrev_c(uint32_t x, int bits) {
+  uint32_t r = 0;
+  for (int i = 0; i < bits; ++i) r |= ((x >> i) & 1u) << (bits - 1 - i);
+  return r;
+}
+constexpr uint32_t phase_bpos(uint32_t gamma, int s0, int q) {
+  return (gamma & ((1u << s0) - 1u)) | ((gamma >> s0) << (s0 + q));
+}
+constexpr uint32_t phase_pos_c(int s0, int q, int e) {
+  return phase_bpos((uint32_t)(e >> q), s0, q) + ((uint32_t)(e & ((1 << q) - 1)) << s0);
 }
 
 struct PassGeom {
@@ -63,16 +98,16 @@
   return ept == 16 ? 2 : (logr == 8 ? MLH_WPS8 : (logr == 9 ? 4 : (logr == 7 ? 4 : 2)));
 }
 
-template <int LOGR, int TW, int ZT, int EPT = kEPT>
-__global__ void __launch_bounds__(kCols * (1 << LOGR) / EPT,
-                                  (TW == 2 || TW == 4) ? 1 : pass_waves_per_simd(LOGR, EPT))
-ntt_pass_kernel(const fe* in, fe* out, const fe* __restrict__ tw,
-                const fe* __restrict__ ta, const fe* __restrict__ tb, PassGeom g) {
+template <int LOGR, int TW, int ZT, int EPT, bool WIDE>
+__device__ __forceinline__ void ntt_pass_body(const fe* in, fe* out, const fe* __restrict__ tw,
+                                              const fe* __restrict__ ta, const fe* __restrict__ tb,
+                                              const PassGeom& g) {
   constexpr int R = 1 << LOGR;
   constexpr int LQ = EPT == 16 ? 4 : 3;
   constexpr int TPC = R / EPT;
   constexpr bool LAST = TW == 2 || TW == 4;
   constexpr bool SH = TW == 4;
+  using Off = std::conditional_t<WIDE, uint64_t, uint32_t>;
   auto phys = [&](uint64_t v) -> uint64_t {
     if constexpr (SH)
       return ((v & ((1ull << g.sh_p) - 1)) << g.sh_lchunk) |
@@ -112,14 +147,15 @@
   in += vec << g.lin_v;
   out += vec << g.lout_v;
 
-  uint64_t base, jrest = 0, k1 = 0, mid = 0;
+  uint64_t base, jcol0 = 0, jrest = 0, k1u = 0, mid = 0;
   uint32_t rshift;
   uint32_t cshift;
   if (!LAST) {
     const uint32_t lw = g.lstride;
     const uint64_t hi = tile >> (lw - kLogCols), lo = tile & ((1ull << (lw - kLogCols)) - 1);
     base = (hi << (LOGR + lw)) + (lo << kLogCols);
-    jrest = (lo << kLogCols) + cB;
+    jcol0 = lo << kLogCols;
+    jrest = jcol0 + cB;
     rshift = lw;
     cshift = 0;
   } else {
@@ -128,12 +164,13 @@
     const uint64_t d1hi = tile >> lmid;
     mid = tile & ((1ull << lmid) - 1);
     base = (d1hi << (kLogCols + lw1)) + (mid << LOGR);
-    k1 = (d1hi << kLogCols) + cB;
+    k1u = d1hi << kLogCols;
     rshift = 0;
     cshift = lw1;
   }
-  const fe* src = in + base + ((uint64_t)c << cshift);
-  fe* dst = out + base + ((uint64_t)cB << cshift);
+  const fe* tile_in = in + base;
+  fe* tile_out = out + base;
+  const Off ld_lane = ((((Off)bitrev((uint32_t)t * EPT, LOGR)) << rshift) + ((Off)c << cshift)) << 4;
 
 
   fe x[EPT];
@@ -155,7 +192,15 @@
         row = ((((q0 << 3) + (l & 7)) << g.sh_p)) | src;
       }
       const uint32_t col = l >> 3;
-      lds[row * kCols + (col ^ swz(row))] = fe_load(in + phys(base + ((uint64_t)col << cshift) + row));
+      if constexpr (SH) {
+        lds[row * kCols + (col ^ swz(row))] = fe_load(in + phys(base + ((uint64_t)col << cshift) + row));
+      } else {
+        auto tile_at = [&](uint32_t i) -> Off {
+          return ((Off)((i & 63) >> 3) << cshift) + (Off)((i >> 6) * 8 + (i & 7));
+        };
+        lds[row * kCols + (col ^ swz(row))] =
+            fe_load_at<Off>(tile_in + (uint64_t)tile_at((uint32_t)(e * NT)), tile_at((uint32_t)tid) << 4);
+      }
     }
     __syncthreads();
 #pragma unroll
@@ -172,12 +217,14 @@
       x[e] = fe_zero();
     } else if (ZT == 2) {
       const uint32_t logw = g.log_n - LOGR;
-      const uint64_t colr = __builtin_bitreverse64(jrest) >> (64 - logw);
-      x[e] = fe_load(in + (colr << (LOGR - 1)) + ((uint32_t)(t * EPT + e) >> 1));
+      const uint64_t colr_u = __builtin_bitreverse64(jcol0) >> (64 - logw);
+      const Off colr_l = (Off)bitrev((uint32_t)cB, kLogCols) << (logw - kLogCols);
+      x[e] = fe_load_at<Off>(in + (colr_u << (LOGR - 1)) + (e >> 1),
+                             ((colr_l << (LOGR - 1)) + (Off)(t * (EPT / 2))) << 4);
     } else if constexpr (SH) {
       x[e] = fe_load(in + phys(base + ((uint64_t)c << cshift) + ((uint64_t)row << rshift)));
     } else {
-      x[e] = fe_load(src + ((uint64_t)row << rshift));
+      x[e] = fe_load_at<Off>(tile_in + ((uint64_t)bitrev_c((uint32_t)e, LOGR) << rshift), ld_lane);
     }
   }
 
@@ -199,10 +246,8 @@
         const int i = ((m >> (s - s0)) << (s - s0 + 1)) | (m & (d - 1));
         be0[b] = gi * (1 << q) + i;
         be1[b] = be0[b] + d;
-        const uint32_t gamma = (uint32_t)(t * G + gi);
-        const uint32_t bpos = (gamma & ((1u << s0) - 1u)) | ((gamma >> s0) << (s0 + q));
-        const uint32_t pos = bpos + ((uint32_t)i << s0);
-        bj[b] = pos & ((1u << s) - 1u);
+        bj[b] = (phase_bpos((uint32_t)(t * G), s0, q) & ((1u << s) - 1u)) +
+                (phase_pos_c(s0, q, gi * (1 << q) + i) & ((1u << s) - 1u));
         btriv[b] = s0 == 0 && (s == 0 || (i & ((1 << s) - 1)) == 0);
       }
       if (ZT != 0 && s0 == 0 && s == 0) {
@@ -241,72 +286,81 @@
       }
     }
   };
-  auto positions = [&](auto S0_, auto Q_, uint32_t (&pos)[EPT]) {
+  auto pos_lane = [&](auto S0_, auto Q_) -> uint32_t {
     constexpr int s0 = decltype(S0_)::value;
     constexpr int q = decltype(Q_)::value;
-    constexpr int G = EPT >> q;
-#pragma unroll
-    for (int gi = 0; gi < G; ++gi) {
-      const uint32_t gamma = (uint32_t)(t * G + gi);
-      const uint32_t bpos = (gamma & ((1u << s0) - 1u)) | ((gamma >> s0) << (s0 + q));
-#pragma unroll
-      for (int i = 0; i < (1 << q); ++i) pos[gi * (1 << q) + i] = bpos + ((uint32_t)i << s0);
-    }
+    return phase_bpos((uint32_t)(t * (EPT >> q)), s0, q);
   };
 
   using I0 = std::integral_constant<int, 0>;
   constexpr int Q1 = LOGR < LQ ? LOGR : LQ;
   run_phase(I0{}, std::integral_constant<int, Q1>{});
-  uint32_t pos[EPT];
-  positions(I0{}, std::integral_constant<int, Q1>{}, pos);
-
-  auto exchange_and_run = [&](auto S0_, auto Q_) {
+  uint32_t pos0 = pos_lane(I0{}, std::integral_constant<int, Q1>{});
+  constexpr int kS0F = LOGR > 2 * LQ ? 2 * LQ : (LOGR > LQ ? LQ : 0);
+  constexpr int kQF = LOGR - kS0F;
+  auto pos_c = [](int e) -> uint32_t { return phase_pos_c(kS0F, kQF, e); };
+
+  auto exchange_and_run = [&](auto PS0_, auto PQ_, auto S0_, auto Q_) {
+    constexpr int ps0 = decltype(PS0_)::value, pq = decltype(PQ_)::value;
+    constexpr int s0 = decltype(S0_)::value, q = decltype(Q_)::value;
     __syncthreads();
-#pragma unroll
-    for (int e = 0; e < EPT; ++e) fe_store(&lds[pos[e] * kCols + c], x[e]);
+    fe* wr = &lds[pos0 * kCols + c];
+#pragma unroll
+    for (int e = 0; e < EPT; ++e) fe_store(wr + phase_pos_c(ps0, pq, e) * kCols, x[e]);
     __syncthreads();
-    positions(S0_, Q_, pos);
-#pragma unroll
-    for (int e = 0; e < EPT; ++e) x[e] = fe_load(&lds[pos[e] * kCols + c]);
+    pos0 = pos_lane(S0_, Q_);
+    const fe* rd = &lds[pos0 * kCols + c];
+#pragma unroll
+    for (int e = 0; e < EPT; ++e) x[e] = fe_load(rd + phase_pos_c(s0, q, e) * kCols);
     run_phase(S0_, Q_);
   };
   constexpr int NTt = kCols * R / EPT;
   constexpr int kTbPerThread = TW == 0 ? R / NTt : 1;
   fe tbv[kTbPerThread][4];
-  const uint64_t jl = jrest & ((1ull << g.loga) - 1);
+  const fe* ta_tile = ta + (jcol0 & ((1ull << g.loga) - 1));
+  auto ta_lane_of = [&](uint32_t p0) -> Off { return (((Off)p0 << g.loga) + (Off)cB) << 4; };
+  auto ta_at = [&](int e, Off lane) -> fe {
+    return fe_load_at<Off>(ta_tile + ((uint64_t)pos_c(e) << g.loga), lane);
+  };
+  Off ta_lane = 0;
   fe ta_c0, ta_c1;
 #ifndef MLH_TB_COALESCED
 #define MLH_TB_COALESCED 1
 #endif
   auto load_tb = [&]() {
     if constexpr (TW == 0 && MLH_DIAG_TW == 0) {
-      const uint64_t jh = jrest >> g.loga;
+      const uint64_t jh = jcol0 >> g.loga;
       const uint32_t ltcols = g.lstride - g.loga;
+      const fe* tb_tile = tb + (jh << 2);
+#if MLH_TB_COALESCED
+      static_assert(NTt % 4 == 0, "a round of pieces is whole rows");
+      const Off tb_lane = ((((Off)(tid >> 2) << ltcols) << 2) + (Off)(tid & 3)) << 4;
+#else
+      const Off tb_lane = (((Off)tid << ltcols) << 2) << 4;
+#endif
 #pragma unroll
       for (int e = 0; e < kTbPerThread; ++e) {
+#pragma unroll
+        for (int k = 0; k < 4; ++k) {
 #if MLH_TB_COALESCED
-#pragma unroll
-        for (int k = 0; k < 4; ++k) {
-          const uint32_t i = (uint32_t)((e * 4 + k) * NTt + tid);
-          tbv[e][k] = fe_load(tb + ((((uint64_t)(i >> 2) << ltcols) + jh) << 2) + (i & 3));
+          tbv[e][k] = fe_load_at<Off>(tb_tile + (((uint64_t)((e * 4 + k) * (NTt / 4)) << ltcols) << 2), tb_lane);
+#else
+          tbv[e][k] = fe_load_at<Off>(tb_tile + (((uint64_t)(e * NTt) << ltcols) << 2) + k, tb_lane);
+#endif
         }
-#else
-        const fe* q = tb + ((((uint64_t)(e * NTt + tid) << ltcols) + jh) << 2);
-#pragma unroll
-        for (int k = 0; k < 4; ++k) tbv[e][k] = fe_load(q + k);
-#endif
       }
     }
   };
-  auto load_ta0 = [&](const uint32_t (&pf)[EPT]) {
+  auto load_ta0 = [&](uint32_t p0) {
     if constexpr (TW == 5) {
-      (void)pf;
+      (void)p0;
     } else if constexpr (!LAST && MLH_DIAG_TW == 2) {
-      ta_c0 = fe{{(uint32_t)jl | 1u, 7u, 9u, 3u}};
-      ta_c1 = fe{{(uint32_t)pf[1] | 1u, 5u, 9u, 3u}};
+      ta_c0 = fe{{(uint32_t)jrest | 1u, 7u, 9u, 3u}};
+      ta_c1 = fe{{(uint32_t)p0 | 1u, 5u, 9u, 3u}};
     } else if constexpr (!LAST) {
-      ta_c0 = fe_load(ta + ((uint64_t)pf[0] << g.loga) + jl);
-      ta_c1 = fe_load(ta + ((uint64_t)pf[1] << g.loga) + jl);
+      ta_lane = ta_lane_of(p0);
+      ta_c0 = ta_at(0, ta_lane);
+      ta_c1 = ta_at(1, ta_lane);
     }
   };
 #ifndef MLH_P0_EARLY_TB
@@ -316,41 +370,51 @@
   constexpr bool kEarly = MLH_P0_EARLY_TB && TW == 0 && LOGR > 2 * LQ;
   if constexpr (LOGR > LQ) {
     constexpr int Q2 = (LOGR - LQ) < LQ ? (LOGR - LQ) : LQ;
+    using IQ1 = std::integral_constant<int, Q1>;
+    using ILQ = std::integral_constant<int, LQ>;
+    using IQ2 = std::integral_constant<int, Q2>;
     if constexpr (kDirect) {
-      auto slot = [&](uint32_t row, int col) -> uint32_t {
-        return row * kCols + ((uint32_t)col ^ ((row >> (LOGR - 3)) & (kCols - 1)));
+      auto slot0 = [&](uint32_t p0, int col) -> uint32_t {
+        return p0 * kCols + ((uint32_t)col ^ ((p0 >> (LOGR - 3)) & (kCols - 1)));
       };
       __syncthreads();
-#pragma unroll
-      for (int e = 0; e < EPT; ++e) fe_store(&lds[slot(pos[e], c)], x[e]);
+      static_assert((phase_pos_c(0, Q1, EPT - 1) >> (LOGR - 3)) == 0, "phase 1: constant rows below the swizzle bits");
+      fe* wr = &lds[slot0(pos0, c)];
+#pragma unroll
+      for (int e = 0; e < EPT; ++e) fe_store(wr + phase_pos_c(0, Q1, e) * kCols, x[e]);
       __syncthreads();
       c = cB;
       t = tid / kCols;
-      positions(std::integral_constant<int, LQ>{}, std::integral_constant<int, Q2>{}, pos);
-#pragma unroll
-      for (int e = 0; e < EPT; ++e) x[e] = fe_load(&lds[slot(pos[e], c)]);
-      run_phase(std::integral_constant<int, LQ>{}, std::integral_constant<int, Q2>{});
+      pos0 = pos_lane(ILQ{}, IQ2{});
+      const uint32_t rd0 = slot0(pos0, c);
+#pragma unroll
+      for (int e = 0; e < EPT; ++e) {
+        const uint32_t pc = phase_pos_c(LQ, Q2, e);
+        const uint32_t sc = (pc >> (LOGR - 3)) & (kCols - 1);
+        x[e] = fe_load(&lds[(rd0 ^ sc) + pc * kCols]);
+      }
+      run_phase(ILQ{}, IQ2{});
     } else {
-      exchange_and_run(std::integral_constant<int, LQ>{}, std::integral_constant<int, Q2>{});
+      exchange_and_run(I0{}, IQ1{}, ILQ{}, IQ2{});
     }
     if constexpr (LOGR > 2 * LQ) {
       constexpr int Q3 = LOGR - 2 * LQ;
       static_assert(Q3 <= LQ, "LOGR <= 3 * LQ");
+      using I2LQ = std::integral_constant<int, 2 * LQ>;
+      using IQ3 = std::integral_constant<int, Q3>;
       if constexpr (kEarly) {
-        uint32_t pf[EPT];
-        positions(std::integral_constant<int, 2 * LQ>{}, std::integral_constant<int, Q3>{}, pf);
         load_tb();
-        if (MLH_P0_EARLY_TB == 1) load_ta0(pf);
-      }
-      exchange_and_run(std::integral_constant<int, 2 * LQ>{}, std::integral_constant<int, Q3>{});
+        if (MLH_P0_EARLY_TB == 1) load_ta0(pos_lane(I2LQ{}, IQ3{}));
+      }
+      exchange_and_run(ILQ{}, IQ2{}, I2LQ{}, IQ3{});
     }
   }
 
   if constexpr (!kEarly) {
-    load_ta0(pos);
+    load_ta0(pos0);
     load_tb();
   } else if (MLH_P0_EARLY_TB == 2) {
-    load_ta0(pos);
+    load_ta0(pos0);
   }
   if constexpr (TW == 0) {
     static_assert(4 * R <= R * kCols, "the expanded TB column fits the exchange tile");
@@ -363,20 +427,21 @@
         lds[MLH_TB_COALESCED ? (e * 4 + k) * NT + tid : 4 * (e * NT + tid) + k] = tbv[e][k];
     __syncthreads();
   }
-  uint64_t kbase = 0;
-  uint32_t kshift = 0;
-  if (LAST) {
-    kbase = k1 + (reverse_mid_digits(g, mid) << g.logr[0]);
-    kshift = g.log_n - LOGR;
-  }
+  Off st_lane = (((Off)pos0 << rshift) + ((Off)cB << cshift)) << 4;
+  auto store_row = [&](int e) {
+    fe_store_at<Off>(tile_out + ((uint64_t)pos_c(e) << rshift), st_lane, x[e]);
+  };
   if constexpr (TW == 5) {
     constexpr int Q3 = LOGR - 2 * LQ, NI = 1 << Q3, G = EPT / NI;
     static_assert(LOGR > 2 * LQ && G % 2 == 0, "progression twiddle: groups in pairs");
     fe tv[G];
 #pragma unroll
-    for (int gq = 0; gq < G; ++gq) tv[gq] = fe_load(ta + ((uint64_t)pos[gq * NI] << g.lstride) + jrest);
-    const fe* cp = tb + 4 * jrest;
-    const fe c0 = fe_load(cp), c1 = fe_load(cp + 1), c2 = fe_load(cp + 2), c3 = fe_load(cp + 3);
+    for (int gq = 0; gq < G; ++gq)
+      tv[gq] = fe_load_at<Off>(ta + jcol0 + ((uint64_t)pos_c(gq * NI) << g.lstride), st_lane);
+    const fe* cp = tb + 4 * jcol0;
+    const Off c_lane = (Off)cB << 6;
+    const fe c0 = fe_load_at<Off>(cp, c_lane), c1 = fe_load_at<Off>(cp + 1, c_lane),
+             c2 = fe_load_at<Off>(cp + 2, c_lane), c3 = fe_load_at<Off>(cp + 3, c_lane);
 #pragma unroll
     for (int i = 0; i < NI; ++i) {
       uint64_t rare;
@@ -384,8 +449,9 @@
       for (int gq = 0; gq < G; gq += 2) {
         const int e0 = gq * NI + i, e1 = (gq + 1) * NI + i;
         bfly_ff_v(x[e0], tv[gq], x[e1], tv[gq + 1], rare);
-        fe_store(dst + ((uint64_t)pos[e0] << rshift), x[e0]);
-        fe_store(dst + ((uint64_t)pos[e1] << rshift), x[e1]);
+        pin_lane_offset(st_lane);
+        store_row(e0);
+        store_row(e1);
       }
       if (i + 1 < NI) {
 #pragma unroll
@@ -393,38 +459,69 @@
       }
     }
   } else if constexpr (!LAST) {
+    const fe* tb_rows = lds + 4 * pos0;
 #pragma unroll
     for (int e = 0; e < EPT; e += 2) {
       uint64_t rare;
       const fe a0 = ta_c0, a1 = ta_c1;
       if (e + 2 < EPT && MLH_DIAG_TW < 2) {
-        ta_c0 = fe_load(ta + ((uint64_t)pos[e + 2] << g.loga) + jl);
-        ta_c1 = fe_load(ta + ((uint64_t)pos[e + 3] << g.loga) + jl);
+        pin_lane_offset(ta_lane);
+        ta_c0 = ta_at(e + 2, ta_lane);
+        ta_c1 = ta_at(e + 3, ta_lane);
       }
       bfly_ff_v(x[e], a0, x[e + 1], a1, rare);
       if constexpr (TW == 0 && MLH_DIAG_TW == 0) {
-        const fe* b0 = lds + 4 * pos[e];
-        const fe* b1 = lds + 4 * pos[e + 1];
+        const fe* b0 = tb_rows + 4 * pos_c(e);
+        const fe* b1 = tb_rows + 4 * pos_c(e + 1);
         bfly_pp_v(x[e], b0[0], b0[1], b0[2], b0[3], x[e + 1], b1[0], b1[1], b1[2], b1[3], rare);
       }
-      fe_store(dst + ((uint64_t)pos[e] << rshift), x[e]);
-      fe_store(dst + ((uint64_t)pos[e + 1] << rshift), x[e + 1]);
-    }
+      pin_lane_offset(st_lane);
+      store_row(e);
+      store_row(e + 1);
+    }
+    (void)tb_rows;
   } else {
     static_assert(EPT % 4 == 0, "canonicalisation in fours");
 #pragma unroll
     for (int e = 0; e < EPT; e += 4) bfly_cccc_v(x[e], x[e + 1], x[e + 2], x[e + 3]);
-#pragma unroll
-    for (int e = 0; e < EPT; ++e) {
-      uint64_t K = kbase + ((uint64_t)pos[e] << kshift);
-      if constexpr (SH) {
+    const uint32_t kshift = g.log_n - LOGR;
+    const uint64_t kbase_u = k1u + (reverse_mid_digits(g, mid) << g.logr[0]);
+    if constexpr (SH) {
+#pragma unroll
+      for (int e = 0; e < EPT; ++e) {
+        uint64_t K = kbase_u + cB + ((uint64_t)(pos0 + pos_c(e)) << kshift);
         const uint32_t lo = g.logr[0] - g.sh_p;
         K = ((K >> g.logr[0]) << lo) | (K & ((1ull << lo) - 1));
-      }
-      fe_store(out + K, x[e]);
-    }
-  }
+        fe_store(out + K, x[e]);
+      }
+    } else {
+      const Off k_lane = (((Off)pos0 << kshift) + (Off)cB) << 4;
+#pragma unroll
+      for (int e = 0; e < EPT; ++e)
+        fe_store_at<Off>(out + kbase_u + ((uint64_t)pos_c(e) << kshift), k_lane, x[e]);
+    }
+  }
+  (void)store_row;
+  (void)st_lane;
+  (void)ld_lane;
+  (void)jrest;
   (void)TPC;
+}
+
+template <int LOGR, int TW, int ZT, int EPT = kEPT>
+__global__ void __launch_bounds__(kCols * (1 << LOGR) / EPT,
+                                  (TW == 2 || TW == 4) ? 1 : pass_waves_per_simd(LOGR, EPT))
+ntt_pass_kernel(const fe* in, fe* out, const fe* __restrict__ tw,
+                const fe* __restrict__ ta, const fe* __restrict__ tb, PassGeom g) {
+  ntt_pass_body<LOGR, TW, ZT, EPT, false>(in, out, tw, ta, tb, g);
+}
+
+template <int LOGR, int TW, int ZT, int EPT = kEPT>
+__global__ void __launch_bounds__(kCols * (1 << LOGR) / EPT,
+                                  (TW == 2 || TW == 4) ? 1 : pass_waves_per_simd(LOGR, EPT))
+ntt_pass_wide_kernel(const fe* in, fe* out, const fe* __restrict__ tw,
+                     const fe* __restrict__ ta, const fe* __restrict__ tb, PassGeom g) {
+  ntt_pass_body<LOGR, TW, ZT, EPT, true>(in, out, tw, ta, tb, g);
 }
 
 __global__ void __launch_bounds__(512)
@@ -638,12 +735,18 @@
 template <int LOGR, int EPT>
 static hipError_t launch_pass_ept(bool last, int zero_top, const fe* in, fe* out, const fe* tw,
                                   const fe* ta, const fe* tb, const PassGeom& g, uint64_t tiles,
-                                  hipStream_t st, bool geo = false) {
+                                  hipStream_t st, bool geo, bool wide) {
   constexpr int threads = kCols * (1 << LOGR) / EPT;
   const dim3 grid((unsigned)tiles), blk(threads);
-#define MLH_PASS(TWV, ZTV)                                                                  \
-  hipLaunchKernelGGL((ntt_pass_kernel<LOGR, TWV, ZTV, EPT>), grid, blk, MLH_LDS_PAD, st, in, out, \
-                     tw, ta, tb, g)
+#define MLH_PASS(TWV, ZTV)                                                                        \
+  do {                                                                                            \
+    if (wide)                                                                                     \
+      hipLaunchKernelGGL((ntt_pass_wide_kernel<LOGR, TWV, ZTV, EPT>), grid, blk, MLH_LDS_PAD, st, \
+                         in, out, tw, ta, tb, g);                                                 \
+    else                                                                                          \
+      hipLaunchKernelGGL((ntt_pass_kernel<LOGR, TWV, ZTV, EPT>), grid, blk, MLH_LDS_PAD,          \
+                         st, in, out, tw, ta, tb, g);                                             \
+  } while (0)
   if (last) {
     if (zero_top) return hipErrorInvalidValue;
     MLH_PASS(2, 0);
@@ -674,8 +777,13 @@
 template <int LOGR>
 static hipError_t launch_pass(bool last, int zero_top, const fe* in, fe* out, const fe* tw,
                               const fe* ta, const fe* tb, const PassGeom& g, uint64_t tiles,
-                              hipStream_t st, bool geo = false) {
-  return launch_pass_ept<LOGR, kEPT>(last, zero_top, in, out, tw, ta, tb, g, tiles, st, geo);
+                              hipStream_t st, bool geo, bool wide) {
+  return launch_pass_ept<LOGR, kEPT>(last, zero_top, in, out, tw, ta, tb, g, tiles, st, geo, wide);
+}
+
+static bool pass_wide(const NttTables& tb, uint32_t log_n, uint32_t lr, uint32_t lstride, bool last) {
+  if (tb.wide_offsets) return true;
+  return (last ? log_n : lr + lstride) + 4 > 32;
 }
 
 void ntt_plan_radices(uint32_t log_n, uint32_t* nradix, uint32_t* logr, const uint32_t* forced,
@@ -748,13 +856,14 @@
     const bool geo = tb.gp[p] != nullptr;
     const fe* ta = geo ? tb.gp[p] : tb.ta[p];
     const fe* tbb = geo ? tb.gc[p] : tb.tb[p];
+    const bool wide = pass_wide(tb, log_n, lr, g.lstride, last);
     switch (lr) {
-      case 4: e = launch_pass<4>(last, zt, src, dst, tb.tw[p], ta, tbb, g, tiles, st, geo); break;
-      case 5: e = launch_pass<5>(last, zt, src, dst, tb.tw[p], ta, tbb, g, tiles, st, geo); break;
-      case 6: e = launch_pass<6>(last, zt, src, dst, tb.tw[p], ta, tbb, g, tiles, st, geo); break;
-      case 7: e = launch_pass<7>(last, zt, src, dst, tb.tw[p], ta, tbb, g, tiles, st, geo); break;
-      case 8: e = launch_pass<8>(last, zt, src, dst, tb.tw[p], ta, tbb, g, tiles, st, geo); break;
-      case 9: e = launch_pass<9>(last, zt, src, dst, tb.tw[p], ta, tbb, g, tiles, st, geo); break;
+      case 4: e = launch_pass<4>(last, zt, src, dst, tb.tw[p], ta, tbb, g, tiles, st, geo, wide); break;
+      case 5: e = launch_pass<5>(last, zt, src, dst, tb.tw[p], ta, tbb, g, tiles, st, geo, wide); break;
+      case 6: e = launch_pass<6>(last, zt, src, dst, tb.tw[p], ta, tbb, g, tiles, st, geo, wide); break;
+      case 7: e = launch_pass<7>(last, zt, src, dst, tb.tw[p], ta, tbb, g, tiles, st, geo, wide); break;
+      case 8: e = launch_pass<8>(last, zt, src, dst, tb.tw[p], ta, tbb, g, tiles, st, geo, wide); break;
+      case 9: e = launch_pass<9>(last, zt, src, dst, tb.tw[p], ta, tbb, g, tiles, st, geo, wide); break;
       default: return hipErrorInvalidValue;
     }
     if (e != hipSuccess) return e;
@@ -808,14 +917,15 @@
     g.lin_v = g.lout_v = log_n;
     const uint64_t tiles = N >> (kLogCols + lr);
     const fe* src = p == 0 ? in : out;
+    const bool wide = pass_wide(tb, log_n, lr, g.lstride, false);
     hipError_t e;
     switch (lr) {
-      case 4: e = launch_pass<4>(false, 0, src, out, tb.tw[p], tb.ta[p], tb.tb[p], g, tiles, st); break;
-      case 5: e = launch_pass<5>(false, 0, src, out, tb.tw[p], tb.ta[p], tb.tb[p], g, tiles, st); break;
-      case 6: e = launch_pass<6>(false, 0, src, out, tb.tw[p], tb.ta[p], tb.tb[p], g, tiles, st); break;
-      case 7: e = launch_pass<7>(false, 0, src, out, tb.tw[p], tb.ta[p], tb.tb[p], g, tiles, st); break;
-      case 8: e = launch_pass<8>(false, 0, src, out, tb.tw[p], tb.ta[p], tb.tb[p], g, tiles, st); break;
-      case 9: e = launch_pass<9>(false, 0, src, out, tb.tw[p], tb.ta[p], tb.tb[p], g, tiles, st); break;
+      case 4: e = launch_pass<4>(false, 0, src, out, tb.tw[p], tb.ta[p], tb.tb[p], g, tiles, st, false, wide); break;
+      case 5: e = launch_pass<5>(false, 0, src, out, tb.tw[p], tb.ta[p], tb.tb[p], g, tiles, st, false, wide); break;
+      case 6: e = launch_pass<6>(false, 0, src, out, tb.tw[p], tb.ta[p], tb.tb[p], g, tiles, st, false, wide); break;
+      case 7: e = launch_pass<7>(false, 0, src, out, tb.tw[p], tb.ta[p], tb.tb[p], g, tiles, st, false, wide); break;
+      case 8: e = launch_pass<8>(false, 0, src, out, tb.tw[p], tb.ta[p], tb.tb[p], g, tiles, st, false, wide); break;
+      case 9: e = launch_pass<9>(false, 0, src, out, tb.tw[p], tb.ta[p], tb.tb[p], g, tiles, st, false, wide); break;
       default: return hipErrorInvalidValue;
     }
     if (e != hipSuccess) return e;
diff --git a/multilinear_amd/csrc/ntt.hpp b/multilinear_amd/csrc/ntt.hpp
--- a/multilinear_amd/csrc/ntt.hpp
+++ b/multilinear_amd/csrc/ntt.hpp
@@ -27,6 +27,7 @@
   fe scale;
   bool inverse = false;
   bool debug_sync = false;
+  bool wide_offsets = false;
 };
 
 void ntt_plan_radices(uint32_t log_n, uint32_t* nradix, uint32_t* logr,
```

Result: faster. 40.05 billion (median of 6 runs) (+3.1%).
